# facebookresearch/gtn

Hardware: AMD Instinct MI355X
Metric: CTC forward+backward losses/sec (T=1000, C=256) (higher is better)
Workload: dtype f32; 1 GPU; BASELINE config C3: compose(ctc_target, emissions)+forwardScore CTC loss fwd+bwd, T=1000, C=256, U=100, batch=512 per GPU; global_batch=512, parallelism=dp1 (utterance sharding, all_gather of losses), rccl_ranks=0

## Files before the change

### gtn_amd/csrc/band.hip

```cpp
#include <hip/hip_runtime.h>

#include <algorithm>
#include <cstdlib>
#include <stdexcept>
#include <type_traits>

#include "kernels.h"

#ifdef GTNX_BAND_TIMING
__device__ long long g_band_timing[256];
#endif

namespace gtnx {
namespace {

constexpr float NEGF = -1.0e30f;
constexpr float DEADF = -1.0e29f;
constexpr float LOG2E = 1.44269504088896340736f;
constexpr double LN2 = 0.693147180559945309417;
constexpr int BW = 256;
constexpr int WG = 512;
constexpr int WGB = 768;
constexpr int NBE = 5;
constexpr int NBG = 7;
// ... 6 lines not shown
#endif
#ifndef GTNX_FWD_COPY_ROTATE
#define GTNX_FWD_COPY_ROTATE 1
#endif
#ifndef GTNX_FWD_DEPTH
#define GTNX_FWD_DEPTH 2
#endif

#ifdef GTNX_BAND_TIMING
#define GTNX_TM(slot)                 \
  do {                                \
    const long long now_ = clock64(); \
    tm_acc[slot] += now_ - tm_last;   \
    tm_last = now_;                   \
  } while (0)
#define GTNX_TM_INIT(base)                       \
  const int tm_base = base;                      \
  long long tm_acc[8] = {0, 0, 0, 0, 0, 0, 0, 0}; \
  long long tm_n = 0;                            \
  long long tm_last = clock64()
#define GTNX_TM_TICK() tm_n += 1
#define GTNX_TM_DUMP()                                                      \
  do {                                                                      \
    if (blockIdx.x == 0 && (threadIdx.x & 63) == 0) {                       \
      for (int i_ = 0; i_ < 7; ++i_) g_band_timing[tm_base + (threadIdx.x >> 6) * 7 + i_] += tm_acc[i_]; \
      if (threadIdx.x == 0) g_band_timing[tm_base + 127] += tm_n;           \
    }                                                                       \
  } while (0)
#else
#define GTNX_TM(slot) do { } while (0)
#define GTNX_TM_INIT(base) do { } while (0)
#define GTNX_TM_TICK() do { } while (0)
#define GTNX_TM_DUMP() do { } while (0)
#endif

__device__ __forceinline__ void lds_barrier() { asm volatile("s_waitcnt lgkmcnt(0)\n\ts_barrier" ::: "memory"); }
#ifdef GTNX_EXP_FAKE_MATH
__device__ __forceinline__ float ex2(float x) { return __builtin_fmaf(x, 0.001f, 1.0f); }
__device__ __forceinline__ float lg2(float x) { return __builtin_fmaf(x, 0.001f, -0.001f); }
#else
__device__ __forceinline__ float ex2(float x) { return __builtin_amdgcn_exp2f(x); }
__device__ __forceinline__ float lg2(float x) { return __builtin_amdgcn_logf(x); }
#endif

__device__ __forceinline__ void settle(float& x) { asm volatile("" : "+v"(x)); }
__device__ __forceinline__ void settle(int& x) { asm volatile("" : "+v"(x)); }
__device__ __forceinline__ float uniform(float x) {
  return __int_as_float(__builtin_amdgcn_readfirstlane(__float_as_int(x)));
}
__device__ __forceinline__ double uniform(double x) {
  const long long b = __double_as_longlong(x);
  const unsigned lo = __builtin_amdgcn_readfirstlane(unsigned(b)), hi = __builtin_amdgcn_readfirstlane(unsigned(b >> 32));
  return __longlong_as_double((long long)(((unsigned long long)hi << 32) | lo));
}

__device__ __forceinline__ float wave_shr1(float x, float fill) {
  return __int_as_float(__builtin_amdgcn_update_dpp(__float_as_int(fill), __float_as_int(x), 0x138, 0xf, 0xf, false));
}
__device__ __forceinline__ float wave_shl1(float x, float fill) {
  return __int_as_float(__builtin_amdgcn_update_dpp(__float_as_int(fill), __float_as_int(x), 0x130, 0xf, 0xf, false));
}
#define GTNX_DPP6(op)                                                         \
  "s_nop 1\n\t" op " %0, %0, %0 row_shr:1 row_mask:0xf bank_mask:0xf\n\t"     \
  "s_nop 1\n\t" op " %0, %0, %0 row_shr:2 row_mask:0xf bank_mask:0xf\n\t"     \
  "s_nop 1\n\t" op " %0, %0, %0 row_shr:4 row_mask:0xf bank_mask:0xf\n\t"     \
  "s_nop 1\n\t" op " %0, %0, %0 row_shr:8 row_mask:0xf bank_mask:0xf\n\t"     \
  "s_nop 1\n\t" op " %0, %0, %0 row_bcast:15 row_mask:0xa bank_mask:0xf\n\t"  \
  "s_nop 1\n\t" op " %0, %0, %0 row_bcast:31 row_mask:0xc bank_mask:0xf\n\t"  \
  "s_nop 1"
__device__ __forceinline__ float wave_max(float x) {
  asm volatile(GTNX_DPP6("v_max_f32_dpp") : "+v"(x));
  return __int_as_float(__builtin_amdgcn_readlane(__float_as_int(x), 63));
}
__device__ __forceinline__ float wave_sum63(float x) {
  asm volatile(GTNX_DPP6("v_add_f32_dpp") : "+v"(x));
  return x;
}
__device__ __forceinline__ float wave_sum(float x) {
  return __int_as_float(__builtin_amdgcn_readlane(__float_as_int(wave_sum63(x)), 63));
}
#define GTNX_DPP2(ctl)                                                  \
  "v_add_f32_dpp %0, %0, %0 " ctl "\n\tv_add_f32_dpp %1, %1, %1 " ctl "\n\ts_nop 0\n\t"
__device__ __forceinline__ void wave_sum63x2(float& a, float& b) {
  asm volatile("s_nop 1\n\t"
               GTNX_DPP2("row_shr:1 row_mask:0xf bank_mask:0xf")
               GTNX_DPP2("row_shr:2 row_mask:0xf bank_mask:0xf")
               GTNX_DPP2("row_shr:4 row_mask:0xf bank_mask:0xf")
               GTNX_DPP2("row_shr:8 row_mask:0xf bank_mask:0xf")
               GTNX_DPP2("row_bcast:15 row_mask:0xa bank_mask:0xf")
               GTNX_DPP2("row_bcast:31 row_mask:0xc bank_mask:0xf")
               : "+v"(a), "+v"(b));
}
__device__ __forceinline__ void row_sum15x2(float& a, float& b) {
  asm volatile("s_nop 1\n\t"
               GTNX_DPP2("row_shr:1 row_mask:0xf bank_mask:0xf")
               GTNX_DPP2("row_shr:2 row_mask:0xf bank_mask:0xf")
               GTNX_DPP2("row_shr:4 row_mask:0xf bank_mask:0xf")
               GTNX_DPP2("row_shr:8 row_mask:0xf bank_mask:0xf")
               : "+v"(a), "+v"(b));
}
#define GTNX_ROR4(op)                                                        \
  "s_nop 1\n\t" op " %0, %0, %0 row_ror:8 row_mask:0xf bank_mask:0xf\n\t"    \
  "s_nop 1\n\t" op " %0, %0, %0 row_ror:4 row_mask:0xf bank_mask:0xf\n\t"    \
  "s_nop 1\n\t" op " %0, %0, %0 row_ror:2 row_mask:0xf bank_mask:0xf\n\t"    \
  "s_nop 1\n\t" op " %0, %0, %0 row_ror:1 row_mask:0xf bank_mask:0xf\n\t"    \
  "s_nop 1"
__device__ __forceinline__ float row16_max(float x) {
  asm volatile(GTNX_ROR4("v_max_f32_dpp") : "+v"(x));
  return x;
}
__device__ __forceinline__ float row16_sum(float x) {
  asm volatile(GTNX_ROR4("v_add_f32_dpp") : "+v"(x));
  return x;
}
__device__ __forceinline__ float lse3(float x0, float x1, float x2) {
  const float mx = fmaxf(fmaxf(x0, x1), x2);
  const float md = __builtin_amdgcn_fmed3f(x0, x1, x2);
  const float mn = fminf(fminf(x0, x1), x2);
  return mx + lg2(1.0f + ex2(md - mx) + ex2(mn - mx));
}

template <int NPL>
struct NodeRegs {
  int lab[NPL];
  float wi[3][NPL];
  float wo[3][NPL];
  int ao[3][NPL];
  bool has_in[NPL];
  bool start[NPL], accept[NPL];
};
template <int NPL, bool WANT_OUT>
__device__ __forceinline__ void load_nodes(const BandPair& P, int m0, NodeRegs<NPL>& g) {
  const GTNX_G gtnx_i4* nodes = reinterpret_cast<const GTNX_G gtnx_i4*>(P.nodes);
#pragma unroll
  for (int j = 0; j < NPL; ++j) {
    const int m = m0 + j;
    g.lab[j] = 0;
    g.start[j] = g.accept[j] = g.has_in[j] = false;
#pragma unroll
    for (int k = 0; k < 3; ++k) {
      g.wi[k][j] = g.wo[k][j] = NEGF;
      g.ao[k][j] = -1;
    }
    if (m < P.N) {
      const gtnx_i4 q = nodes[m];
      g.lab[j] = q.x >= 0 ? q.x : 0;
      const uint8_t f = P.nflags[m];
      g.start[j] = (f & NF_START) != 0;
      g.accept[j] = (f & NF_ACCEPT) != 0;
      const int a[3] = {q.y, q.z, q.w};
#pragma unroll
      for (int k = 0; k < 3; ++k)
        if (a[k] >= 0) {
          g.has_in[j] = true;
          g.wi[k][j] = P.w ? fmaxf(P.w[a[k]] * LOG2E, NEGF) : 0.0f;
        }
    }
    if (WANT_OUT) {
#pragma unroll
      for (int k = 0; k < 3; ++k) {
        if (m + k < P.N) {
          const gtnx_i4 q = nodes[m + k];
          const int a = k == 0 ? q.y : (k == 1 ? q.z : q.w);
          if (a >= 0) {
            g.ao[k][j] = a;
            g.wo[k][j] = P.w ? fmaxf(P.w[a] * LOG2E, NEGF) : 0.0f;
          }
        }
      }
    }
  }
}

__device__ __forceinline__ float em2(float x) { return fmaxf(x * LOG2E, NEGF); }

__device__ __forceinline__ int row_of(int e, int W, float invW) {
  int r = int(float(e) * invW);
  if (r * W > e) --r;
  if ((r + 1) * W <= e) ++r;
  return r;
}

template <int NS, int LN = BW>
struct Stage {
  float v[NS];
  template <bool VEC>
  __device__ __forceinline__ void issue(const GTNX_G float* src, int cnt, int tid) {
    if (cnt <= 0) return;
#pragma unroll
    for (int i = 0; i < NS / 4; ++i) {
      if (i > 0 && 4 * i * LN >= cnt) break;
      const int e = min(4 * (i * LN + tid), cnt - 4);
      const gtnx_f4 q = *reinterpret_cast<const GTNX_G gtnx_f4*>(reinterpret_cast<const GTNX_G char*>(src) + unsigned(4 * e));
      v[4 * i] = q.x;
      v[4 * i + 1] = q.y;
      v[4 * i + 2] = q.z;
      v[4 * i + 3] = q.w;
    }
  }
  int off[NS / 4];
  __device__ __forceinline__ void init_offsets(int W, int stride, int K, int tid, bool reverse = true) {
    const float invW = 1.0f / float(W);
#pragma unroll
    for (int i = 0; i < NS / 4; ++i) {
      const int e = 4 * (i * LN + tid);
      const int r = row_of(min(e, 4096), W, invW);
      off[i] = (reverse ? K - 1 - r : r) * stride + (e - r * W);
    }
  }
  template <class F>
  __device__ __forceinline__ void each_vec(int cnt, int shift, int tid, F&& f) const {
#pragma unroll
    for (int i = 0; i < NS / 4; ++i) {
      if (i > 0 && 4 * i * LN >= cnt) break;
      if (4 * (i * LN + tid) < cnt) f(i, off[i] - shift, gtnx_f4{v[4 * i], v[4 * i + 1], v[4 * i + 2], v[4 * i + 3]});
    }
  }
  __device__ __forceinline__ void settle_all() {
#pragma unroll
    for (int i = 0; i < NS; ++i) asm volatile("" : "+v"(v[i]));
  }
  template <bool VEC, class F>
  __device__ __forceinline__ void each(int cnt, int W, int tid, F&& f) const {
    const float invW = 1.0f / float(W);
    if constexpr (VEC) {
#pragma unroll
      for (int i = 0; i < NS / 4; ++i) {
        if (i > 0 && 4 * i * LN >= cnt) break;
        const int e = 4 * (i * LN + tid);
        if (e < cnt) {
          const int r = row_of(e, W, invW);
          f(i, e, r, e - r * W, gtnx_f4{v[4 * i], v[4 * i + 1], v[4 * i + 2], v[4 * i + 3]});
        }
      }
    } else {
#pragma unroll
      for (int i = 0; i < NS / 4; ++i) {
        if (i > 0 && 4 * i * LN >= cnt) break;
        if (4 * (i * LN + tid) < cnt) {
          const int e = min(4 * (i * LN + tid), cnt - 4);
          const int r0 = row_of(e, W, invW), c0 = e - r0 * W;
#pragma unroll
          for (int k = 0; k < 4; ++k) {
            int r = r0, col = c0 + k;
            if (col >= W) {
              col -= W;
              ++r;
            }
            f(i, e + k, r, col, gtnx_f4{v[4 * i + k], 0.0f, 0.0f, 0.0f});
          }
        }
      }
    }
  }
};

struct BandLds {
  int CS;
  int o_ering, o_aring, o_oring, o_snode, o_misc, total;
};
__host__ __device__ inline BandLds band_lds(int C, int K, int NSmax, bool backward) {
  BandLds L;
  L.CS = C + 4;
  int o = 0;
  L.o_ering = o;
  o += (backward ? NBGE : NBE) * K * L.CS;
  o = (o + 3) & ~3;
  L.o_aring = o;
  o += backward ? NBE * K * NSmax : 0;
  o = (o + 3) & ~3;
  L.o_oring = o;
  o += backward ? max(NBG * K * NSmax, 2 * C) : 0;
  o = (o + 3) & ~3;
  L.o_snode = o;
  o += backward ? 512 : 0;
  L.o_misc = o;
  o += 160 + 32 + 8 + 2 * NBE * K * 4 + 40 * K + 8 + 512;
  L.total = o;
  return L;
}
struct BandMisc {
  double *offr, *red, *find, *aofr;
  float *bndr, *fin, *lsep;
};
template <int K>
__device__ __forceinline__ BandMisc band_misc(float* lds, const BandLds& L) {
  BandMisc m;
  m.offr = reinterpret_cast<double*>(lds + L.o_misc);
  m.red = m.offr + 80;
  m.find = m.red + 16;
  m.aofr = m.find + 4;
  m.bndr = lds + L.o_misc + 200 + 2 * NBE * K * 4;
  m.fin = m.bndr + 40 * K;
  m.lsep = m.fin + 8;
  return m;
}

__device__ __forceinline__ float wave_max_of(const float* v, int n) {
  float mx = v[0];
  for (int j = 1; j < n; ++j) mx = fmaxf(mx, v[j]);
  return wave_max(mx);
}

template <int NPL, bool UNIT, int K, bool VEC>
__global__ __launch_bounds__(WG) void band_forward_kernel(const BandPair* __restrict__ pairs, int NSmax) {
#define GTNX_BAND_PAIR pairs[blockIdx.x]
#include "band_forward_body.inc"
#undef GTNX_BAND_PAIR
}
template <int NPL, bool UNIT, int K, bool VEC>
__global__ __launch_bounds__(WG) void band_forward_one_kernel(BandPair one, int NSmax) {
#define GTNX_BAND_PAIR one
#include "band_forward_body.inc"
#undef GTNX_BAND_PAIR
}

__device__ __forceinline__ BandPair band_patched(BandPair P, const BandPatch& pt) {
  if (pt.on) {
    const int b = P.bidx;
    P.delta = pt.delta + b;
    P.delta_norm = pt.delta_norm ? pt.delta_norm + b : nullptr;
    P.rowlse = pt.rowlse ? pt.rowlse + int64_t(b) * pt.M : nullptr;
    P.norm = nullptr;
    P.em_copy = nullptr;
    P.grad_em = pt.grad_em ? pt.grad_em + int64_t(b) * pt.A : nullptr;
    P.grad_fixed = pt.grad_fixed ? pt.grad_fixed + P.goff : nullptr;
  }
  return P;
}
template <int NPL, bool UNIT, bool GRADG, int K, bool VEC, bool BIG>
__global__ __launch_bounds__(WGB, BIG ? 3 : 6) void band_backward_kernel(const BandPair* __restrict__ pairs, int NSmax, BandPatch patch) {
#define GTNX_BAND_PAIR band_patched(pairs[blockIdx.x], patch)
#include "band_backward_body.inc"
#undef GTNX_BAND_PAIR
}
template <int NPL, bool UNIT, bool GRADG, int K, bool VEC, bool BIG>
__global__ __launch_bounds__(WGB, BIG ? 3 : 6) void band_backward_one_kernel(BandPair one, int NSmax) {
#define GTNX_BAND_PAIR one
#include "band_backward_body.inc"
#undef GTNX_BAND_PAIR
}


__global__ __launch_bounds__(512) void ctc_targets_kernel(const CtcTargetArgs* __restrict__ args, int blank) {
  const CtcTargetArgs a = args[blockIdx.x];
  __shared__ __attribute__((aligned(16))) int tl[256 + 4];
  __shared__ __attribute__((aligned(16))) int tk[256 + 4];
  const int N = a.N, U = (N - 1) >> 1, m = threadIdx.x;
  if (m < 260) {
    const int v = m < U ? a.labels[m] : 0x7fffffff;
    tl[m] = v;
    tk[m] = (m > 0 && m < U && v != a.labels[m - 1]) ? 1 : 0;
  }
  __syncthreads();
  if (m >= N) return;
  const bool odd = (m & 1) != 0;
  const int my = odd ? tl[(m - 1) >> 1] : blank;
  const int skip = odd ? tk[(m - 1) >> 1] : 0;
  const int mi = (m - 1) >> 1;
  const int before = odd ? mi : (m >> 1);
  int rank = 0, skips = 0;
  for (int o = 0; o < U; o += 4) {
    const gtnx_i4 l4 = *reinterpret_cast<const gtnx_i4*>(tl + o), k4 = *reinterpret_cast<const gtnx_i4*>(tk + o);
    const int lo[4] = {l4.x, l4.y, l4.z, l4.w}, ko[4] = {k4.x, k4.y, k4.z, k4.w};
#pragma unroll
    for (int k = 0; k < 4; ++k) {
      const bool front = o + k < before;
      rank += (lo[k] < my || (lo[k] == my && front)) ? 1 : 0;
      skips += front ? ko[k] : 0;
    }
  }
  rank += blank < my ? U + 1 : (blank == my ? (m + 1) >> 1 : 0);
  const int base = (m > 0 ? 2 * m - 1 : 0) + skips;
  GTNX_G BandNode* nd = const_cast<GTNX_G BandNode*>(a.nodes);
  nd[m].lab = my;
  nd[m].aid[0] = base;
  nd[m].aid[1] = m > 0 ? base + 1 : -1;
  nd[m].aid[2] = skip ? base + 2 : -1;
  a.nflags[m] = uint8_t((m == 0 ? NF_START : 0) | (m + 2 >= N ? NF_ACCEPT : 0));
  a.snode[rank] = m;
  a.slab[rank] = my;
  if (m == N - 1 && a.n_arcs) a.n_arcs[0] = base + 1 + (m > 0 ? 1 : 0) + skip;
}

__global__ __launch_bounds__(512) void band_viterbi_kernel(const BandDecode* __restrict__ pairs) {
  const BandDecode P = pairs[blockIdx.x];
  const int T = P.T, C = P.C, N = P.N, NS = P.NS;
  extern __shared__ float lds[];
  const float NINF = -__builtin_inff();
  float* a0 = lds;
  float* a1 = lds + 516;
  float* stage = lds + 1032;
  const int m = threadIdx.x;
  const GTNX_G gtnx_i4* nodes = reinterpret_cast<const GTNX_G gtnx_i4*>(P.nodes);
  int lab = 0;
  float wi[3] = {NINF, NINF, NINF};
  bool accept = false, start = false;
  if (m < N) {
    const gtnx_i4 q = nodes[m];
    lab = q.x >= 0 ? q.x : 0;
    const int a[3] = {q.y, q.z, q.w};
#pragma unroll
    for (int k = 0; k < 3; ++k)
      if (a[k] >= 0) wi[k] = P.w ? P.w[a[k]] : 0.0f;
    const uint8_t f = P.nflags[m];
    start = (f & NF_START) != 0;
    accept = (f & NF_ACCEPT) != 0;
  }
  if (m < 2) a0[m] = a1[m] = NINF;
  a0[2 + m] = start ? 0.0f : NINF;
  a1[2 + m] = NINF;
  int tie = 0;
  const int R = max(1, min(64, P.stage_floats / C));
  float* cur = a0;
  float* nxt = a1;
  __syncthreads();
  for (int t0 = 0; t0 < T; t0 += R) {
    const int rows = min(R, T - t0);
    for (int e = threadIdx.x; e < rows * C; e += blockDim.x) stage[e] = P.em[int64_t(t0) * C + e];
    __syncthreads();
    for (int i = 0; i < rows; ++i) {
      const float e = stage[i * C + lab];
      const float c0 = cur[2 + m] + (wi[0] + e), c1 = cur[1 + m] + (wi[1] + e), c2 = cur[m] + (wi[2] + e);
      float best = c0;
      int k = 0;
      if (c1 > best) best = c1, k = 1;
      if (c2 > best) best = c2, k = 2;
      if (best > NINF && ((k != 0 && c0 == best) || (k != 1 && c1 == best) || (k != 2 && c2 == best))) tie = 1;
      if (m < NS) P.bp[int64_t(t0 + i) * NS + m] = uint8_t(best > NINF ? k : 3);
      nxt[2 + m] = m < N ? best : NINF;
      __syncthreads();
      float* sw = cur;
      cur = nxt;
      nxt = sw;
    }
  }
  __shared__ float red_v[8];
  __shared__ int red_m[8], s_best, s_tie;
  float v = accept ? cur[2 + m] : NINF;
  int bm = (m < N && accept && v > NINF) ? m : 1 << 30;
  const float wmx = wave_max(v);
  if (!(v == wmx)) bm = 1 << 30;
  int cnt = (bm != (1 << 30)) ? 1 : 0;
  for (int o = 32; o > 0; o >>= 1) {
    bm = min(bm, __shfl_xor(bm, o));
    cnt += __shfl_xor(cnt, o);
  }
  if ((threadIdx.x & 63) == 0) {
    red_v[threadIdx.x >> 6] = wmx;
    red_m[threadIdx.x >> 6] = bm;
  }
  if (cnt > 1) tie = 1;
  if (threadIdx.x == 0) s_tie = 0;
  __syncthreads();
  if (threadIdx.x == 0) {
    float bv = NINF;
    int bn = -1;
    for (int w = 0; w < 8; ++w) {
      if (red_m[w] == (1 << 30)) continue;
      if (red_v[w] > bv) bv = red_v[w], bn = red_m[w];
      else if (red_v[w] == bv && bv > NINF) s_tie = 1;
    }
    s_best = bn;
    P.score[0] = bv;
  }
  if (tie) atomicOr(&s_tie, 1);
  __syncthreads();
  const int best = s_best;
  if (threadIdx.x == 0) {
    P.tie[0] = s_tie;
    P.path_len[0] = best >= 0 ? T : -1;
  }
  if (best < 0 || T == 0) return;
  uint8_t* bst = reinterpret_cast<uint8_t*>(stage);
  const int RB = max(1, min(T, P.stage_floats * 4 / NS));
  __shared__ int s_node;
  if (threadIdx.x == 0) {
    s_node = best;
    P.pnode[T] = best;
  }
  for (int hi = T; hi > 0; hi -= RB) {
    const int lo = max(0, hi - RB);
    __syncthreads();
    for (int e = threadIdx.x; e < (hi - lo) * NS; e += blockDim.x) bst[e] = P.bp[int64_t(lo) * NS + e];
    __syncthreads();
    if (threadIdx.x == 0) {
      int node = s_node;
      for (int t = hi - 1; t >= lo; --t) {
        node -= bst[(t - lo) * NS + node] & 3;
        P.pnode[t] = node;
      }
      s_node = node;
    }
  }
  __threadfence_block();
  __syncthreads();
  for (int t = threadIdx.x; t < T; t += blockDim.x) {
    const int m1 = P.pnode[t + 1], k = m1 - P.pnode[t];
    const gtnx_i4 q = nodes[m1];
    const int arc = k == 0 ? q.y : (k == 1 ? q.z : q.w);
    P.path_arc[t] = arc;
    P.path_lab[t] = q.x;
    P.path_w[t] = (P.w ? P.w[arc] : 0.0f) + P.em[int64_t(t) * C + q.x];
  }
}

constexpr int VBLK = 2048;

template <int NPL, bool RANKED>
__global__ __launch_bounds__(64) void band_viterbi_wave_kernel(const BandDecode* __restrict__ pairs) {
  const BandDecode P = pairs[blockIdx.x];
  const int T = P.T, C = P.C, N = P.N;
  const int lane = threadIdx.x;
  constexpr int SPW = 16 / NPL;
  constexpr int NLD = VBLK / 256;
  __shared__ __attribute__((aligned(16))) float ring[3 * VBLK];
  const float NINF = -__builtin_inff();
  const GTNX_G gtnx_i4* nodes = reinterpret_cast<const GTNX_G gtnx_i4*>(P.nodes);
  int loff[NPL];
  float w0[NPL], w1[NPL], w2[NPL], alpha[NPL];
  bool acc[NPL];
#pragma unroll
  for (int j = 0; j < NPL; ++j) {
    const int m = lane * NPL + j;
    loff[j] = 0;
    w0[j] = w1[j] = w2[j] = NINF;
    alpha[j] = NINF;
    acc[j] = false;
    if (m < N) {
      const gtnx_i4 q = nodes[m];
      loff[j] = 4 * (q.x >= 0 ? q.x : 0);
      if (q.y >= 0) w0[j] = P.w ? P.w[q.y] : 0.0f;
      if (q.z >= 0) w1[j] = P.w ? P.w[q.z] : 0.0f;
      if (q.w >= 0) w2[j] = P.w ? P.w[q.w] : 0.0f;
      const uint8_t f = P.nflags[m];
      if (f & NF_START) alpha[j] = 0.0f;
      acc[j] = (f & NF_ACCEPT) != 0;
    }
  }
#pragma unroll
  for (int j = 0; j < NPL; ++j) {
    settle(w0[j]);
    settle(w1[j]);
    settle(w2[j]);
    settle(loff[j]);
  }
  int r0[NPL], r1[NPL], r2[NPL];
  if (RANKED) {
#pragma unroll
    for (int j = 0; j < NPL; ++j) {
      const int m = lane * NPL + j;
      r0[j] = m < N ? P.rank_in[m] : 0x7ffffffe;
      r1[j] = (m >= 1 && m - 1 < N) ? P.rank_in[m - 1] : 0x7ffffffe;
      r2[j] = (m >= 2 && m - 2 < N) ? P.rank_in[m - 2] : 0x7ffffffe;
    }
  }
  const int R = max(1, VBLK / C);
  const int NB = (T + R - 1) / R;
  const int64_t total = int64_t(T) * C;
  auto issue = [&](int b) {
    const int64_t f0 = int64_t(b) * R * C;
    float* dst = ring + (b % 3) * VBLK;
#pragma unroll
    for (int i = 0; i < NLD; ++i) {
      int64_t f = f0 + i * 256 + lane * 4;
      f = f + 4 <= total ? f : total - 4;
      __builtin_amdgcn_global_load_lds((const __attribute__((address_space(1))) void*)(P.em + f),
                                       (__attribute__((address_space(3))) void*)(dst + i * 256), 16, 0, 0);
    }
  };
  GTNX_G unsigned* bp32 = reinterpret_cast<GTNX_G unsigned*>(P.bp);
  unsigned word = 0;
  if (NB > 0) issue(0);
  if (NB > 1) issue(1);
#ifdef GTNX_VIT_NO_SWEEP
#define GTNX_VIT_ROWS 0
#else
#define GTNX_VIT_ROWS rows
#endif
  for (int b = 0; b < NB; ++b) {
    if (b + 2 < NB) {
      issue(b + 2);
      asm volatile("s_waitcnt vmcnt(16)" ::: "memory");
    } else if (b + 1 < NB) {
      asm volatile("s_waitcnt vmcnt(8)" ::: "memory");
    } else {
      asm volatile("s_waitcnt vmcnt(0)" ::: "memory");
    }
    const char* buf = reinterpret_cast<const char*>(ring + (b % 3) * VBLK);
    const int t0 = b * R, rows = min(R, T - t0);
    float e[NPL];
#pragma unroll
    for (int j = 0; j < NPL; ++j) e[j] = *reinterpret_cast<const float*>(buf + loff[j]);
    for (int i = 0; i < GTNX_VIT_ROWS; ++i) {
      const int t = t0 + i;
      const char* nrow = buf + (i + 1 < rows ? i + 1 : i) * (C * 4);
      float en[NPL];
#pragma unroll
      for (int j = 0; j < NPL; ++j) en[j] = *reinterpret_cast<const float*>(nrow + loff[j]);
      float s1, s2;
      if (NPL >= 2) {
        s1 = wave_shr1(alpha[NPL - 1], NINF);
        s2 = wave_shr1(alpha[NPL >= 2 ? NPL - 2 : 0], NINF);
      } else {
        s1 = wave_shr1(alpha[0], NINF);
        s2 = wave_shr1(s1, NINF);
      }
      float na[NPL];
      const int sh = (t % SPW) * 2 * NPL;
      unsigned codes = 0;
#pragma unroll
      for (int j = 0; j < NPL; ++j) {
        const float p1 = j > 0 ? alpha[j > 0 ? j - 1 : 0] : s1;
        const float p2 = j > 1 ? alpha[j > 1 ? j - 2 : 0] : (j == 1 ? s1 : s2);
        const float c0 = alpha[j] + (w0[j] + e[j]), c1 = p1 + (w1[j] + e[j]), c2 = p2 + (w2[j] + e[j]);
        const float best = fmaxf(fmaxf(c0, c1), c2);
        const float med = __builtin_amdgcn_fmed3f(c0, c1, c2);
        unsigned k;
        if (RANKED) {
          const int q0 = c0 == best ? r0[j] : 0x7fffffff, q1 = c1 == best ? r1[j] : 0x7fffffff,
                    q2 = c2 == best ? r2[j] : 0x7fffffff;
          k = (q0 <= q1 && q0 <= q2) ? 0u : (q1 <= q2 ? 1u : 2u);
          k = best == NINF ? 3u : k;
          (void)med;
        } else {
          k = c0 == best ? 0u : (c1 == best ? 1u : 2u);
          k = med == best ? 3u : k;
        }
        codes |= k << (2 * j);
        na[j] = best;
      }
      word |= codes << sh;
#pragma unroll
      for (int j = 0; j < NPL; ++j) {
        alpha[j] = na[j];
        e[j] = en[j];
      }
      if ((t % SPW) == SPW - 1 || t == T - 1) {
        bp32[int64_t(t / SPW) * 64 + lane] = word;
        word = 0;
      }
    }
  }
  float lv = NINF;
#pragma unroll
  for (int j = 0; j < NPL; ++j) lv = fmaxf(lv, acc[j] ? alpha[j] : NINF);
  const float wmx = wave_max(lv);
  int bm = 1 << 30, cnt = 0;
#pragma unroll
  for (int j = NPL - 1; j >= 0; --j)
    if (acc[j] && alpha[j] == wmx && wmx > NINF) {
      const int m = lane * NPL + j;
      bm = RANKED ? min(bm, (P.rank_acc[m] << 16) | m) : m;
      ++cnt;
    }
  for (int o = 32; o > 0; o >>= 1) {
    bm = min(bm, __shfl_xor(bm, o));
    cnt += __shfl_xor(cnt, o);
  }
  int tie = (cnt > 1 && !RANKED) ? 1 : 0;
  const int best = bm == (1 << 30) ? -1 : (RANKED ? (bm & 0xffff) : bm);
  if (lane == 0) {
    P.score[0] = best >= 0 ? wmx : NINF;
    P.path_len[0] = best >= 0 ? T : -1;
  }
  if (best < 0 || T == 0) {
    if (lane == 0) P.tie[0] = tie;
    return;
  }
#ifdef GTNX_VIT_NO_CHASE
  if (lane == 0) P.tie[0] = tie;
  return;
#endif
  __builtin_amdgcn_fence(__ATOMIC_SEQ_CST, "workgroup");
  unsigned node = unsigned(__builtin_amdgcn_readfirstlane(best));
  int* lpn = reinterpret_cast<int*>(ring);
  constexpr int LPN = 3 * VBLK;
  if (lane == 0) {
    P.pnode[T] = int(node);
    if (T < LPN) lpn[T] = int(node);
  }
  const int NW = (T + SPW - 1) / SPW;
  constexpr int RB = 16;
  unsigned cur[RB], nxt[RB];
  const int nbatch = (NW + RB - 1) / RB;
  auto fetch = [&](unsigned (&dst)[RB], int q) {
#pragma unroll
    for (int r = 0; r < RB; ++r) dst[r] = bp32[int64_t(min(q * RB + r, NW - 1)) * 64 + lane];
  };
  fetch(cur, nbatch - 1);
  int pn = 0;
  for (int q = nbatch - 1; q >= 0; --q) {
    if (q > 0) fetch(nxt, q - 1);
#pragma unroll
    for (int r = RB - 1; r >= 0; --r) {
      const int wi = q * RB + r;
      if (wi < NW) {
#pragma unroll
        for (int u = SPW - 1; u >= 0; --u) {
          const int t = wi * SPW + u;
          if (t < T) {
            const unsigned wv = unsigned(__builtin_amdgcn_readlane(int(cur[r]), int(node / NPL)));
            unsigned k = (wv >> (u * 2 * NPL + 2 * (node % NPL))) & 3u;
            if (k == 3u) {
              tie = 1;
              k = 0;
            }
            node -= min(k, node);
            if (lane == (t & 63)) pn = int(node);
            if ((t & 63) == 0) {
              if (t + lane < T) {
                P.pnode[t + lane] = pn;
                if (t + lane < LPN) lpn[t + lane] = pn;
              }
            }
          }
        }
      }
    }
#pragma unroll
    for (int r = 0; r < RB; ++r) cur[r] = nxt[r];
  }
  if (lane == 0) P.tie[0] = tie;
  if (T >= LPN) __builtin_amdgcn_fence(__ATOMIC_SEQ_CST, "workgroup");
  for (int t = lane; t < T; t += 64) {
    const int m1 = T < LPN ? lpn[t + 1] : P.pnode[t + 1], k = m1 - (T < LPN ? lpn[t] : P.pnode[t]);
    const gtnx_i4 q = nodes[m1];
    const int arc = k == 0 ? q.y : (k == 1 ? q.z : q.w);
    P.path_arc[t] = arc;
    P.path_lab[t] = q.x;
    P.path_w[t] = (arc >= 0 && P.w ? P.w[arc] : 0.0f) + P.em[int64_t(t) * C + (q.x >= 0 ? q.x : 0)];
  }
}

__global__ __launch_bounds__(512) void asg_fal_targets_kernel(const AsgFalArgs* __restrict__ args, int NL) {
  const AsgFalArgs a = args[blockIdx.x];
  __shared__ int lab[512];
  const int U = a.U, m = threadIdx.x;
  int my = -1;
  if (m >= 1 && m <= U) my = a.labels[m - 1];
  lab[m] = my;
  __syncthreads();
  if (m > U) return;
  GTNX_G BandNode* nd = const_cast<GTNX_G BandNode*>(a.nodes);
  nd[m].lab = my;
  nd[m].aid[0] = m >= 1 ? 2 * m - 1 : -1;
  nd[m].aid[1] = m >= 1 ? 2 * m - 2 : -1;
  nd[m].aid[2] = -1;
  a.nflags[m] = uint8_t((m == 0 ? NF_START : 0) | (m == U ? NF_ACCEPT : 0));
  if (m >= 1) {
    int rank = 0;
    for (int o = 1; o <= U; ++o) {
      const int lo = lab[o];
      rank += (lo < my || (lo == my && o < m)) ? 1 : 0;
    }
    a.snode[rank] = m;
    a.slab[rank] = my;
    const int step = m == 1 ? my : NL + my * NL + lab[m - 1];
    const int self = NL + my * NL + my;
    a.arc_map[2 * m - 2] = step;
    a.arc_map[2 * m - 1] = self;
    a.w[2 * m - 2] = a.trans_w[step];
    a.w[2 * m - 1] = a.trans_w[self];
  }
}
__global__ void asg_fal_scatter_kernel(const float* __restrict__ g, const int* __restrict__ maps,
                                       const int64_t* __restrict__ tab, float* __restrict__ trans_grad) {
  const int64_t* e = tab + int64_t(blockIdx.y) * 3;
  const int64_t n = e[2];
  const float* gb = g + e[0];
  const int* mb = maps + e[1];
  for (int64_t i = int64_t(blockIdx.x) * blockDim.x + threadIdx.x; i < n; i += int64_t(gridDim.x) * blockDim.x)
    if (mb[i] >= 0 && gb[i] != 0.0f) atomicAdd(trans_grad + mb[i], gb[i]);
}

template <class K>
void big_lds(K kern) {
  (void)hipFuncSetAttribute(reinterpret_cast<const void*>(kern), hipFuncAttributeMaxDynamicSharedMemorySize, 160 * 1024 - 512);
}

template <int NPL, int K, bool VEC>
void launch_fwd2(const BandPair* d, const BandPair* one, int n, int ns, size_t lds, bool unit, hipStream_t st) {
  static std::atomic<uint64_t> done{0};
  if (gtnx_first_on_device first{done}) {
    big_lds(band_forward_kernel<NPL, true, K, VEC>);
    big_lds(band_forward_kernel<NPL, false, K, VEC>);
    if constexpr (NPL == 1 && VEC) {
      big_lds(band_forward_one_kernel<NPL, true, K, VEC>);
      big_lds(band_forward_one_kernel<NPL, false, K, VEC>);
    }
  }
  if constexpr (NPL == 1 && VEC) {
    if (one) {
      if (unit) hipLaunchKernelGGL((band_forward_one_kernel<NPL, true, K, VEC>), dim3(1), dim3(WG), lds, st, *one, ns);
      else hipLaunchKernelGGL((band_forward_one_kernel<NPL, false, K, VEC>), dim3(1), dim3(WG), lds, st, *one, ns);
      return;
    }
  }
  if (unit) hipLaunchKernelGGL((band_forward_kernel<NPL, true, K, VEC>), dim3(n), dim3(WG), lds, st, d, ns);
  else hipLaunchKernelGGL((band_forward_kernel<NPL, false, K, VEC>), dim3(n), dim3(WG), lds, st, d, ns);
}
template <int NPL, int K>
void launch_fwd(const BandPair* d, const BandPair* one, int n, int ns, size_t lds, bool unit, bool vec, hipStream_t st) {
  if (vec) launch_fwd2<NPL, K, true>(d, one, n, ns, lds, unit, st);
  else launch_fwd2<NPL, K, false>(d, one, n, ns, lds, unit, st);
}
template <int NPL, int K, bool VEC, bool BIG>
void launch_bwd3(const BandPair* d, const BandPair* one, int n, int ns, size_t lds, bool unit, bool gradg, hipStream_t st,
                 const BandPatch& pt) {
  constexpr bool ONE = NPL == 1 && VEC && !BIG;
  static std::atomic<uint64_t> done{0};
  if (gtnx_first_on_device first{done}) {
    big_lds(band_backward_kernel<NPL, true, true, K, VEC, BIG>);
    big_lds(band_backward_kernel<NPL, true, false, K, VEC, BIG>);
    big_lds(band_backward_kernel<NPL, false, true, K, VEC, BIG>);
    big_lds(band_backward_kernel<NPL, false, false, K, VEC, BIG>);
    if constexpr (ONE) {
      big_lds(band_backward_one_kernel<NPL, true, true, K, VEC, BIG>);
      big_lds(band_backward_one_kernel<NPL, true, false, K, VEC, BIG>);
      big_lds(band_backward_one_kernel<NPL, false, true, K, VEC, BIG>);
      big_lds(band_backward_one_kernel<NPL, false, false, K, VEC, BIG>);
    }
  }
  if constexpr (ONE) {
    if (one) {
      if (unit) {
        if (gradg) hipLaunchKernelGGL((band_backward_one_kernel<NPL, true, true, K, VEC, BIG>), dim3(1), dim3(WGB), lds, st, *one, ns);
        else hipLaunchKernelGGL((band_backward_one_kernel<NPL, true, false, K, VEC, BIG>), dim3(1), dim3(WGB), lds, st, *one, ns);
      } else {
        if (gradg) hipLaunchKernelGGL((band_backward_one_kernel<NPL, false, true, K, VEC, BIG>), dim3(1), dim3(WGB), lds, st, *one, ns);
        else hipLaunchKernelGGL((band_backward_one_kernel<NPL, false, false, K, VEC, BIG>), dim3(1), dim3(WGB), lds, st, *one, ns);
      }
      return;
    }
  }
  if (unit) {
    if (gradg) hipLaunchKernelGGL((band_backward_kernel<NPL, true, true, K, VEC, BIG>), dim3(n), dim3(WGB), lds, st, d, ns, pt);
    else hipLaunchKernelGGL((band_backward_kernel<NPL, true, false, K, VEC, BIG>), dim3(n), dim3(WGB), lds, st, d, ns, pt);
  } else {
    if (gradg) hipLaunchKernelGGL((band_backward_kernel<NPL, false, true, K, VEC, BIG>), dim3(n), dim3(WGB), lds, st, d, ns, pt);
    else hipLaunchKernelGGL((band_backward_kernel<NPL, false, false, K, VEC, BIG>), dim3(n), dim3(WGB), lds, st, d, ns, pt);
  }
}
template <int NPL, int K>
void launch_bwd(const BandPair* d, const BandPair* one, int n, int ns, size_t lds, bool unit, bool gradg, bool vec, bool big,
                hipStream_t st, const BandPatch& pt) {
  if constexpr (K == 2) {
    if (big) {
      if (vec) launch_bwd3<NPL, K, true, true>(d, one, n, ns, lds, unit, gradg, st, pt);
      else launch_bwd3<NPL, K, false, true>(d, one, n, ns, lds, unit, gradg, st, pt);
      return;
    }
  }
  if (vec) launch_bwd3<NPL, K, true, false>(d, one, n, ns, lds, unit, gradg, st, pt);
  else launch_bwd3<NPL, K, false, false>(d, one, n, ns, lds, unit, gradg, st, pt);
}

constexpr size_t LDS_TWO = 78 * 1024;
constexpr size_t LDS_ONE = 156 * 1024;

}

int band_block_rows(int C, int max_NS, bool backward);
static int band_backward_lds_stride(int K, int max_NS) { return K == 4 ? (max_NS + 15) / 16 * 16 : max_NS; }
int band_max_nodes() { return 512; }
int band_max_labels() { return 1024; }
int band_min_labels() { return 4; }
int band_npl(int max_nodes) { return max_nodes <= 256 ? 1 : 2; }
int band_row_stride(int N, int) { return (N + 3) / 4 * 4; }
#ifndef GTNX_FWD_SHIFT_ROWS
#define GTNX_FWD_SHIFT_ROWS 4
#endif
int band_forward_lgrn(int C) {
  const int K = band_block_rows(C, 0, false);
  return K >= GTNX_FWD_SHIFT_ROWS ? (GTNX_FWD_SHIFT_ROWS == 8 ? 3 : 2) : (K >= 4 ? 2 : 1);
}
int band_block_rows(int C, int max_NS, bool backward) {
  for (int k = backward ? 4 : 8; k >= 2; k /= 2) {
    if (k * C > 2048 || k * max_NS > 2048) continue;
    if (backward && k > 2 && (k * C > 1024 || k * max_NS > 1024)) continue;
    const int ns_lds = backward ? band_backward_lds_stride(k, max_NS) : max_NS;
    if (4 * size_t(band_lds(C, k, ns_lds, backward).total) + 64 <= LDS_TWO) return k;
  }
  if (4 * size_t(band_lds(C, 2, max_NS, backward).total) + 64 <= LDS_ONE) return 2;
  return 0;
}

bool band_one_ok(int npl, int C, int max_NS, bool vec, bool backward) {
  if (npl != 1 || !vec) return false;
  if (!backward) return true;
  const int K = band_block_rows(C, max_NS, true);
  return !(K * C > 1024 || K * max_NS > 1024);
}
void launch_band_forward(const BandPair* d_pairs, int n, int npl, int C, int max_NS, bool unit, bool vec, hipStream_t st,
                         const BandPair* one) {
  if (n <= 0) return;
  if (one && (n != 1 || !band_one_ok(npl, C, max_NS, vec, false))) throw std::logic_error("band.hip: not a single-pair launch");
  const int K = band_block_rows(C, 0, false);
  const size_t lds = 4 * size_t(band_lds(C, K, max_NS, false).total) + 64;
  if (npl == 1) {
    if (K == 8) launch_fwd<1, 8>(d_pairs, one, n, max_NS, lds, unit, vec, st);
    else if (K == 4) launch_fwd<1, 4>(d_pairs, one, n, max_NS, lds, unit, vec, st);
    else launch_fwd<1, 2>(d_pairs, one, n, max_NS, lds, unit, vec, st);
  } else {
    if (K == 8) launch_fwd<2, 8>(d_pairs, one, n, max_NS, lds, unit, vec, st);
    else if (K == 4) launch_fwd<2, 4>(d_pairs, one, n, max_NS, lds, unit, vec, st);
    else launch_fwd<2, 2>(d_pairs, one, n, max_NS, lds, unit, vec, st);
  }
}

void launch_band_backward(const BandPair* d_pairs, int n, int npl, int C, int max_NS, bool unit, bool gradg, bool vec,
                          hipStream_t st, const BandPair* one, const BandPatch* patch) {
  if (n <= 0) return;
  if (one && patch) throw std::logic_error("band.hip: a patched launch reads a device table");
  BandPatch pt{};
  if (patch) pt = *patch;
  if (one && (n != 1 || !band_one_ok(npl, C, max_NS, vec, true))) throw std::logic_error("band.hip: not a single-pair launch");
  const int K = band_block_rows(C, max_NS, true);
  const bool big = K * C > 1024 || K * max_NS > 1024;
  const int ns_lds = band_backward_lds_stride(K, max_NS);
  const size_t lds = 4 * size_t(band_lds(C, K, ns_lds, true).total) + 64;
  if (npl == 1) {
    if (K == 4) launch_bwd<1, 4>(d_pairs, one, n, ns_lds, lds, unit, gradg, vec, big, st, pt);
    else launch_bwd<1, 2>(d_pairs, one, n, ns_lds, lds, unit, gradg, vec, big, st, pt);
  } else {
    if (K == 4) throw std::logic_error("band.hip: four rows per block with two nodes per lane");
    launch_bwd<2, 2>(d_pairs, one, n, ns_lds, lds, unit, gradg, vec, big, st, pt);
  }
}

template <int NPL>
static void launch_viterbi_wave(const BandDecode* d_pairs, int n, int ranked, hipStream_t st) {
  if (ranked) hipLaunchKernelGGL((band_viterbi_wave_kernel<NPL, true>), dim3(n), dim3(64), 0, st, d_pairs);
  else hipLaunchKernelGGL((band_viterbi_wave_kernel<NPL, false>), dim3(n), dim3(64), 0, st, d_pairs);
}
bool band_viterbi_wave_ok(int max_nodes, int max_labels, int vec) {
  static const bool force_wg = std::getenv("GTNX_VITERBI_WG") != nullptr;
  return !force_wg && vec && max_nodes <= 512 && max_labels <= VBLK;
}
void launch_band_viterbi(const BandDecode* d_pairs, int n, int stage_floats, int max_nodes, int max_labels, int vec,
                         hipStream_t st, int ranked) {
  if (n <= 0) return;
  if (band_viterbi_wave_ok(max_nodes, max_labels, vec)) {
    if (max_nodes <= 64) launch_viterbi_wave<1>(d_pairs, n, ranked, st);
    else if (max_nodes <= 128) launch_viterbi_wave<2>(d_pairs, n, ranked, st);
    else if (max_nodes <= 256) launch_viterbi_wave<4>(d_pairs, n, ranked, st);
    else launch_viterbi_wave<8>(d_pairs, n, ranked, st);
    return;
  }
  if (ranked) return;
  static std::atomic<uint64_t> done{0};
  if (gtnx_first_on_device first{done}) big_lds(band_viterbi_kernel);
  hipLaunchKernelGGL(band_viterbi_kernel, dim3(n), dim3(512), 4 * size_t(1032 + stage_floats) + 64, st, d_pairs);
}

void launch_asg_fal_targets(const AsgFalArgs* d_args, int n, int n_labels, hipStream_t st) {
  if (n > 0) hipLaunchKernelGGL(asg_fal_targets_kernel, dim3(n), dim3(512), 0, st, d_args, n_labels);
}
void launch_asg_fal_scatter(const float* g, const int* maps, const int64_t* tab, int n_seq, int64_t longest, float* trans_grad,
                            hipStream_t st) {
  if (n_seq > 0 && longest > 0)
    hipLaunchKernelGGL(asg_fal_scatter_kernel, dim3(unsigned(std::min<int64_t>((longest + 255) / 256, 64)), unsigned(n_seq)),
                       dim3(256), 0, st, g, maps, tab, trans_grad);
}
void launch_ctc_targets(const CtcTargetArgs* d_args, int n, int blank, hipStream_t st) {
  if (n > 0) hipLaunchKernelGGL(ctc_targets_kernel, dim3(n), dim3(512), 0, st, d_args, blank);
}

}
```

### gtn_amd/csrc/band_backward_body.inc

```
  constexpr int RNk = K >= 4 ? 4 : K;
  constexpr int NP = K / RNk;
  const BandPair P = GTNX_BAND_PAIR;
  const int T = P.T, C = P.C, NS = P.NS;
  extern __shared__ float lds[];
  const BandLds L = band_lds(C, K, NSmax, true);
  float* ering = lds + L.o_ering;
  float* aring = lds + L.o_aring;
  float* oring = lds + L.o_oring;
  int* snode = reinterpret_cast<int*>(lds + L.o_snode);
  const BandMisc M = band_misc<K>(lds, L);
  float* lser = M.lsep;
  const int CS = L.CS;
  const int wv = __builtin_amdgcn_readfirstlane(threadIdx.x >> 6);
  const bool sweeper = wv < 4;
  const int l = threadIdx.x & 63;
  const int nblocks = (T + K - 1) / K;
  const int nticks = nblocks + 5;
  const GTNX_G double* ao = P.aoff;
  const double z2 = uniform(ao[0]);
  const bool dead = !(z2 > double(DEADF));
  const float ds = uniform(P.delta[0]);
  const bool want_em = P.grad_em != nullptr;
  GTNX_TM_INIT(128);
  constexpr bool SPLIT = !BIG && K >= 2 && GTNX_BWD_SPLIT;
  const float dn_k = P.delta_norm ? uniform(P.delta_norm[0]) : 0.0f;
  float* const rnorm_k = lser + NBG * K;
  auto rows_of_k = [&](int c) { return c < nblocks ? min(K, T - c * K) : 0; };
  auto ring_start = [](int c, int M) { return ((c % M) + M) % M; };
  static_assert((NBGE & (NBGE - 1)) == 0, "the emission ring's position is a mask");
  auto ge_of = [](int c) { return int(unsigned(c) & unsigned(NBGE - 1)); };
  auto ring_step = [](int& v, int M) { v = v + 1 == M ? 0 : v + 1; };
  struct RowSumRegs {
    float in[NPL];
    gtnx_f4 hot[NPL];
  };
  auto rowsum_init = [&](RowSumRegs& R) {
#pragma unroll
    for (int q = 0; q < NPL; ++q) {
      const int mb = 256 * q + 4 * l;
      R.in[q] = mb < NSmax ? 1.0f : 0.0f;
      float hm[4];
#pragma unroll
      for (int k = 0; k < 4; ++k) {
        const int m = mb + k;
        int lab = -1;
        if (m < P.N) lab = P.nodes[m].lab;
        settle(lab);
        hm[k] = (P.hot >= 0 && lab == P.hot) ? 1.0f : 0.0f;
      }
      R.hot[q] = gtnx_f4{hm[0], hm[1], hm[2], hm[3]};
    }
  };
  auto rowsum_do = [&](const RowSumRegs& R, int c, int cg , int r, auto steady_tag) -> float {
    constexpr bool STEADY = decltype(steady_tag)::value;
    if (!want_em || (K < 4 && r >= K)) return 0.0f;
    if constexpr (!STEADY) {
      if (r >= rows_of_k(c)) return 0.0f;
    }
    const bool dead_r = STEADY ? false : dead;
    const float* ob = oring + (cg * K + r) * NSmax;
    gtnx_f4 v[NPL];
#pragma unroll
    for (int q = 0; q < NPL; ++q) v[q] = *reinterpret_cast<const gtnx_f4*>(ob + min(256 * q + 4 * l, NSmax - 4));
    const float em_hot = ering[(ge_of(c) * K + r) * CS + max(P.hot, 0)];
    const float ls_hot = lser[cg * K + r];
    float all = (v[0].x * R.in[0] + v[0].y * R.in[0]) + (v[0].z * R.in[0] + v[0].w * R.in[0]);
    float hotp = (v[0].x * R.hot[0].x + v[0].y * R.hot[0].y) + (v[0].z * R.hot[0].z + v[0].w * R.hot[0].w);
#pragma unroll
    for (int q = 1; q < NPL; ++q) {
      all += (v[q].x * R.in[q] + v[q].y * R.in[q]) + (v[q].z * R.in[q] + v[q].w * R.in[q]);
      hotp += (v[q].x * R.hot[q].x + v[q].y * R.hot[q].y) + (v[q].z * R.hot[q].z + v[q].w * R.hot[q].w);
    }
    if (dead_r) all = hotp = 0.0f;
    wave_sum63x2(all, hotp);
    all = __int_as_float(__builtin_amdgcn_readlane(__float_as_int(all), 63));
    const bool have = all != 0.0f && !dead_r;
    const float f = have ? ds * __builtin_amdgcn_rcpf(all) : 1.0f;
    if (l == 63 && P.hot >= 0) {
      const float sm = dn_k * ex2(em_hot - ls_hot);
      P.grad_em[int64_t(T - 1 - c * K - r) * C + P.hot] = (dead_r ? 0.0f : hotp * f) + sm;
    }
    if (l == 0) rnorm_k[cg * K + r] = f;
    return have ? f : 0.0f;
  };
#ifndef GTNX_BWD_ROWSUM4
#define GTNX_BWD_ROWSUM4 1
#endif
  constexpr bool RS4 = !BIG && !SPLIT && K == 4 && NPL == 1 && GTNX_BWD_ROWSUM4;
  struct RowSum4Regs {
    float in;
    gtnx_f4 hot[4];
    int po;
    int eo, go;
  };
  auto rowsum4_init = [&](RowSum4Regs& R) {
    const int r = l >> 4, nb = 16 * (l & 15);
    R.in = nb < NSmax ? 1.0f : 0.0f;
    R.po = r * NSmax + min(nb, NSmax - 16);
#pragma unroll
    for (int k = 0; k < 4; ++k) {
      float hm[4];
#pragma unroll
      for (int e = 0; e < 4; ++e) {
        const int m = nb + 4 * k + e;
        int lab = -1;
        if (m < P.N) lab = P.nodes[m].lab;
        settle(lab);
        hm[e] = (P.hot >= 0 && lab == P.hot) ? 1.0f : 0.0f;
      }
      R.hot[k] = gtnx_f4{hm[0], hm[1], hm[2], hm[3]};
    }
    R.eo = r * CS + max(P.hot, 0);
    R.go = (K - 1 - r) * C + max(P.hot, 0);
  };
  auto rowsum4_do = [&](const RowSum4Regs& R, int c, int cg , auto steady_tag) {
    constexpr bool STEADY = decltype(steady_tag)::value;
    const int rows = STEADY ? K : rows_of_k(c);
    if (!want_em || rows <= 0) return;
    const bool dead_r = STEADY ? false : dead;
    typedef float f2v __attribute__((ext_vector_type(2)));
    const float* ob = oring + cg * K * NSmax + R.po;
    gtnx_f4 v[4];
#pragma unroll
    for (int k = 0; k < 4; ++k) v[k] = *reinterpret_cast<const gtnx_f4*>(ob + 4 * k);
    const float em_hot = ering[ge_of(c) * K * CS + R.eo];
    const float ls_hot = lser[cg * K + (l >> 4)];
    f2v a2 = f2v{v[0].x, v[0].y} + f2v{v[0].z, v[0].w};
    f2v h2 = f2v{v[0].x, v[0].y} * f2v{R.hot[0].x, R.hot[0].y};
    h2 = __builtin_elementwise_fma(f2v{v[0].z, v[0].w}, f2v{R.hot[0].z, R.hot[0].w}, h2);
#pragma unroll
    for (int k = 1; k < 4; ++k) {
      a2 += f2v{v[k].x, v[k].y} + f2v{v[k].z, v[k].w};
      h2 = __builtin_elementwise_fma(f2v{v[k].x, v[k].y}, f2v{R.hot[k].x, R.hot[k].y}, h2);
      h2 = __builtin_elementwise_fma(f2v{v[k].z, v[k].w}, f2v{R.hot[k].z, R.hot[k].w}, h2);
    }
    float all = (a2.x + a2.y) * R.in, hotp = h2.x + h2.y;
    if (dead_r) all = hotp = 0.0f;
    row_sum15x2(all, hotp);
    const bool have = all != 0.0f && !dead_r;
    const float f = have ? ds * __builtin_amdgcn_rcpf(all) : 1.0f;
    if ((l & 15) == 15 && (STEADY || (l >> 4) < rows)) {
      if (P.hot >= 0) {
        const float sm = dn_k * ex2(em_hot - ls_hot);
        const GTNX_G char* gb = reinterpret_cast<const GTNX_G char*>(P.grad_em + int64_t(T - c * K - K) * C);
        *reinterpret_cast<GTNX_G float*>(const_cast<GTNX_G char*>(gb) + unsigned(4 * R.go)) = (dead_r ? 0.0f : hotp * f) + sm;
      }
      rnorm_k[cg * K + (l >> 4)] = f;
    }
  };
  constexpr int NCS = 8 / K;
  struct DrainRegs {
    int s[NCS], e[NCS], n0[NCS], n1[NCS];
    float m0[NCS], m1[NCS];
    bool more_any;
  };
  auto drain_init = [&](DrainRegs& D, int hid) {
    const int* cls = reinterpret_cast<const int*>(oring);
#pragma unroll
    for (int q = 0; q < NCS; ++q) {
      const int cc = hid + q * BW;
      D.s[q] = D.e[q] = 0;
      if (cc < C && cc != P.hot) {
        D.s[q] = cls[cc];
        D.e[q] = cls[C + cc];
      }
      const int cnt = D.e[q] - D.s[q];
      D.n0[q] = cnt > 0 ? snode[D.s[q]] : 0;
      D.n1[q] = cnt > 1 ? snode[D.s[q] + 1] : 0;
      D.m0[q] = cnt > 0 ? 1.0f : 0.0f;
      D.m1[q] = cnt > 1 ? 1.0f : 0.0f;
    }
    D.more_any = false;
#pragma unroll
    for (int q = 0; q < NCS; ++q) D.more_any = D.more_any || __builtin_amdgcn_ballot_w64(D.e[q] - D.s[q] > 2) != 0;
  };
  auto drain_rows = [&](const DrainRegs& D, int hid, int c, int cg , auto full_tag, auto dead_tag, auto r0_tag, auto r1_tag) {
    constexpr bool FULL = decltype(full_tag)::value;
    constexpr bool DEADU = decltype(dead_tag)::value;
    constexpr int R0 = decltype(r0_tag)::value, R1 = decltype(r1_tag)::value;
    const int rows = FULL ? K : rows_of_k(c);
    const float* ob = oring + cg * K * NSmax;
    const float* eb = ering + ge_of(c) * K * CS;
    const float* lb = lser + cg * K;
    const float* fb = rnorm_k + cg * K;
    GTNX_G float* dst = P.grad_em + int64_t(T - 1 - c * K) * C;
#pragma unroll
    for (int q = 0; q < NCS; ++q) {
      if (q > 0 && q * BW >= C) break;
      const int cc = hid + q * BW;
      const bool mine = cc < C && cc != P.hot;
      float p0[K], p1[K], e[K], ls[K], f[K];
#pragma unroll
      for (int r = R0; r < R1; ++r) {
        if constexpr (!DEADU) {
          p0[r] = ob[r * NSmax + D.n0[q]];
          p1[r] = ob[r * NSmax + D.n1[q]];
        }
        e[r] = eb[r * CS + min(cc, C - 1)];
      }
      if constexpr (K == 4) {
        const gtnx_f4 l4 = *reinterpret_cast<const gtnx_f4*>(lb), f4 = *reinterpret_cast<const gtnx_f4*>(fb);
        ls[0] = l4.x, ls[1] = l4.y, ls[2] = l4.z, ls[3] = l4.w;
        f[0] = f4.x, f[1] = f4.y, f[2] = f4.z, f[3] = f4.w;
      } else {
#pragma unroll
        for (int r = R0; r < R1; ++r) {
          ls[r] = lb[r];
          f[r] = fb[r];
        }
      }
      float sum[K];
      if constexpr (!DEADU) {
#pragma unroll
      for (int r = R0; r < R1; ++r) sum[r] = p0[r] * D.m0[q] + p1[r] * D.m1[q];
      }
      if (!DEADU && D.more_any) {
        for (int i = D.s[q] + 2; i < D.e[q]; ++i) {
          const float* o = ob + snode[i];
#pragma unroll
          for (int r = R0; r < R1; ++r) sum[r] += o[r * NSmax];
        }
      }
      float val[K];
#pragma unroll
      for (int r = R0; r < R1; ++r) {
        const float sm = dn_k * ex2(e[r] - ls[r]);
        val[r] = DEADU ? sm : sum[r] * f[r] + sm;
      }
      if (mine) {
#pragma unroll
        for (int r = R0; r < R1; ++r) {
          if (FULL || r < rows) {
            GTNX_G float* row = dst - int64_t(r) * C;
            row[cc] = val[r];
          }
        }
      }
    }
  };
  auto drain_block = [&](const DrainRegs& D, int hid, int c, int cg, auto r0_tag, auto r1_tag) {
    if (!want_em || c >= nblocks) return;
    if (dead) drain_rows(D, hid, c, cg, std::false_type{}, std::true_type{}, r0_tag, r1_tag);
    else if (c * K + K <= T) drain_rows(D, hid, c, cg, std::true_type{}, std::false_type{}, r0_tag, r1_tag);
    else drain_rows(D, hid, c, cg, std::false_type{}, std::false_type{}, r0_tag, r1_tag);
  };
  constexpr int KH = SPLIT ? K / 2 : K;

  if (sweeper) {
#ifndef GTNX_BWD_SWEEP_PRIO
#define GTNX_BWD_SWEEP_PRIO 1
#endif
    __builtin_amdgcn_s_setprio(GTNX_BWD_SWEEP_PRIO);
    const int w = wv;
    const int lag = 3 - w;
    const int m0 = threadIdx.x * NPL;
    NodeRegs<NPL> g;
    load_nodes<NPL, true>(P, m0, g);
    float b[NPL], post[NPL], acc[3][NPL];
    const double Ahi = uniform(ao[1 + (T >> P.lgrn) * 4 + w]);
    double bsum = 0.0;
#pragma unroll
    for (int j = 0; j < NPL; ++j) {
      b[j] = g.accept[j] ? 0.0f : NEGF;
      float ahi = m0 < NS ? P.alpha[int64_t(T) * NS + m0 + j] : NEGF;
      settle(ahi);
      post[j] = dead ? 0.0f : ex2(ahi + b[j] + float(Ahi - z2));
      acc[0][j] = acc[1][j] = acc[2][j] = 0.0f;
      settle(g.lab[j]);
#pragma unroll
      for (int k = 0; k < 3; ++k) {
        settle(g.wo[k][j]);
        settle(g.ao[k][j]);
      }
    }
    float* bnd_own = M.bndr + (4 - w) * 4 * K * 2;
    const float* bnd_prev = M.bndr + (3 - w) * 4 * K * 2;
    double* off_own = M.offr + (4 - w) * 16;
    const double* off_prev = M.offr + (3 - w) * 16;
    if (threadIdx.x < 8 * K) M.bndr[threadIdx.x] = NEGF;
    if (threadIdx.x < 16) M.offr[threadIdx.x] = 0.0;
    if (l == 0) off_own[0] = 0.0;
    lds_barrier();
    lds_barrier();
    RowSumRegs rsr;
    if constexpr (!SPLIT && !RS4) rowsum_init(rsr);
    float gscale = ds;
    int bm5 = ring_start(-lag, NBE), bm7 = ring_start(-lag, NBG), rm7 = ring_start(RS4 ? -5 : -4, NBG);
    lds_barrier();
    auto tick = [&](int tau, auto steady_tag) {
      constexpr bool STEADY = decltype(steady_tag)::value;
      GTNX_TM(0);
      if constexpr (RS4) {
#ifndef GTNX_EXP_NO_GSCALE
        if (GRADG && want_em && (STEADY || (tau >= 5 && (tau - 5) * K + K <= T))) gscale = rnorm_k[rm7 * K + w];
#endif
      } else if constexpr (!SPLIT) {
#ifndef GTNX_EXP_NO_ROWSUM
        if (STEADY || tau >= 4) {
          const float fr = rowsum_do(rsr, tau - 4, rm7, w, steady_tag);
#ifndef GTNX_EXP_NO_GSCALE
          if (fr != 0.0f) gscale = fr;
#endif
        }
#endif
      }
      GTNX_TM(3);
      const int beta = tau - lag;
      auto block = [&](auto full_tag) {
        constexpr bool FULL = decltype(full_tag)::value;
        const int v0 = beta * K, rows = FULL ? K : min(K, T - v0);
        const float* eb = ering + ge_of(beta) * K * CS;
        const float* ab = aring + bm5 * K * NSmax;
        const double* Ab = M.aofr + (bm5 * K) * 4 + w;
        float* ob = oring + bm7 * K * NSmax + m0;
        float ev[K][NPL], alov[K][NPL], bq1[K], bq2[K];
        double Acur[K], offp[NP + 1];
#pragma unroll
        for (int i = 0; i < K; ++i) {
#pragma unroll
          for (int j = 0; j < NPL; ++j) {
            ev[i][j] = eb[i * CS + g.lab[j]];
            alov[i][j] = ab[i * NSmax + min(m0 + j, NS - 1)];
          }
          Acur[i] = Ab[i * 4];
        }
#pragma unroll
        for (int q = 0; q <= NP; ++q) offp[q] = off_prev[(beta * NP + q) & 15];
        {
// ... 400 lines not shown
```

### gtn_amd/csrc/band_forward_body.inc

```
#ifndef GTNX_FWD_SHIFT_ROWS
#define GTNX_FWD_SHIFT_ROWS 4
#endif
  constexpr int RNk = K >= GTNX_FWD_SHIFT_ROWS ? GTNX_FWD_SHIFT_ROWS : (K >= 4 ? 4 : K);
  constexpr int NP = K / RNk;
  constexpr int D = 8 / K > GTNX_FWD_DEPTH ? 8 / K : GTNX_FWD_DEPTH;
  const BandPair P = GTNX_BAND_PAIR;
  const int T = P.T, C = P.C, NS = P.NS;
  extern __shared__ float lds[];
  const BandLds L = band_lds(C, K, NSmax, false);
  float* ering = lds + L.o_ering;
  const BandMisc M = band_misc<K>(lds, L);
  const int CS = L.CS;
  const int wv = __builtin_amdgcn_readfirstlane(threadIdx.x >> 6);
  const bool sweeper = wv < 4;
  const int l = threadIdx.x & 63;
  const int nblocks = (T + K - 1) / K;
  const int nticks = nblocks + 3;
  GTNX_TM_INIT(0);

  if (sweeper) {
    __builtin_amdgcn_s_setprio(1);
    const int w = wv;
    const int m0 = threadIdx.x * NPL;
    NodeRegs<NPL> g;
    load_nodes<NPL, false>(P, m0, g);
    const bool writer = m0 < NS;
    float a[NPL];
#pragma unroll
    for (int j = 0; j < NPL; ++j) a[j] = g.start[j] ? 0.0f : NEGF;
    double off = 0.0;
    const GTNX_G char* arow = reinterpret_cast<const GTNX_G char*>(P.alpha);
    const unsigned aoffb = unsigned(m0) * 4u;
    auto store_row = [&](const float* v) {
#pragma unroll
      for (int j = 0; j < NPL; ++j) *reinterpret_cast<GTNX_G float*>(const_cast<GTNX_G char*>(arow) + (aoffb + 4u * j)) = v[j];
    };
    if (writer) store_row(a);
    float* bnd_own = M.bndr + (w + 1) * 4 * K * 2;
    const float* bnd_prev = M.bndr + w * 4 * K * 2;
    double* off_own = M.offr + (w + 1) * 16;
    const double* off_prev = M.offr + w * 16;
    if (threadIdx.x < 8 * K) M.bndr[threadIdx.x] = NEGF;
    if (threadIdx.x < 16) M.offr[threadIdx.x] = 0.0;
    if (l == 0) {
      P.aoff[1 + w] = 0.0;
      off_own[0] = 0.0;
    }
    if (NPL == 1) {
      if (l >= 62) bnd_own[63 - l] = a[0];
    } else if (l == 63) {
      bnd_own[0] = a[NPL - 1];
      bnd_own[1] = a[0];
    }
    lds_barrier();
    int bm5 = ((-w % NBE) + NBE) % NBE;
    for (int tau = 0; tau < nticks; ++tau, bm5 = bm5 + 1 == NBE ? 0 : bm5 + 1) {
      GTNX_TM(0);
      const int beta = tau - w;
      auto block = [&](auto full_tag) {
        constexpr bool FULL = decltype(full_tag)::value;
        const int t0 = beta * K, rows = FULL ? K : min(K, T - t0);
        const float* eb = ering + bm5 * K * CS;
        float ev[K][NPL], bv1[K], bv2[K];
        double offp[NP + 1];
#pragma unroll
        for (int i = 0; i < K; ++i) {
#pragma unroll
#ifdef GTNX_EXP_NOCONFLICT
          for (int j = 0; j < NPL; ++j) ev[i][j] = eb[i * CS + l * NPL + j];
#else
          for (int j = 0; j < NPL; ++j) ev[i][j] = eb[i * CS + g.lab[j]];
#endif
        }
        {
          const float* bp = bnd_prev + (beta & 3) * K * 2;
          if constexpr (K % 2 == 0) {
#pragma unroll
            for (int i = 0; i < K; i += 2) {
              const gtnx_f4 q4 = *reinterpret_cast<const gtnx_f4*>(bp + 2 * i);
              bv1[i] = q4.x, bv2[i] = q4.y, bv1[i + 1] = q4.z, bv2[i + 1] = q4.w;
            }
          } else {
#pragma unroll
            for (int i = 0; i < K; ++i) bv1[i] = bp[2 * i], bv2[i] = bp[2 * i + 1];
          }
        }
#pragma unroll
        for (int q = 0; q <= NP; ++q) offp[q] = off_prev[(beta * NP + q) & 15];
        float hist[K][NPL];
#pragma unroll
        for (int i = 0; i < K; ++i) {
          if (FULL || i < rows) {
            if (i % RNk == 0) {
              typedef float f2v __attribute__((ext_vector_type(2)));
              const float dconv = float(offp[i / RNk] - off);
              const f2v d2 = {dconv, dconv};
#pragma unroll
              for (int r = i; r < i + RNk && r < K; ++r) {
                const f2v c = f2v{bv1[r], bv2[r]} + d2;
                bv1[r] = c.x, bv2[r] = c.y;
              }
            }
            const float b1 = bv1[i], b2 = bv2[i];
            const float p1 = wave_shr1(a[NPL - 1], b1);
            const float p2 = NPL == 2 ? wave_shr1(a[0], b2) : wave_shr1(p1, b2);
            float nw[NPL];
#pragma unroll
            for (int j = 0; j < NPL; ++j) {
              const float s1 = j == 0 ? p1 : a[0];
              const float s2 = j == 0 ? p2 : p1;
              float x0, x1, x2;
              if (UNIT) {
                x0 = a[j];
                x1 = s1;
                x2 = s2 + g.wi[2][j];
              } else {
                x0 = a[j] + g.wi[0][j];
                x1 = s1 + g.wi[1][j];
                x2 = s2 + g.wi[2][j];
              }
              nw[j] = lse3(x0, x1, x2) + ev[i][j];
            }
            if ((i + 1) % RNk == 0) {
              const float mx = wave_max_of(nw, NPL);
              if (mx > DEADF) {
#pragma unroll
                for (int j = 0; j < NPL; ++j) nw[j] -= mx;
                off += double(mx);
              } else if (w > 0) {
                off = offp[(i + 1) / RNk];
              }
              if (l == 0) {
                const int p = (t0 + i + 1) / RNk;
                off_own[p & 15] = off;
                P.aoff[1 + p * 4 + w] = off;
              }
            }
#pragma unroll
            for (int j = 0; j < NPL; ++j) hist[i][j] = a[j] = nw[j];
          }
        }
        {
          const GTNX_G char* const brow = arow;
          arow += int64_t(NS) * 4 * rows;
#ifdef GTNX_EXP_NO_ALPHA_STORE
          if (writer && beta < 0) {
#else
          if (writer) {
#endif
#pragma unroll
            for (int i = 0; i < K; ++i)
              if (FULL || i < rows) {
                const GTNX_G char* ri = brow + int64_t(NS) * 4 * (i + 1);
#pragma unroll
                for (int j = 0; j < NPL; ++j) *reinterpret_cast<GTNX_G float*>(const_cast<GTNX_G char*>(ri) + (aoffb + 4u * j)) = hist[i][j];
              }
          }
        }
        if (NPL == 1 ? l >= 62 : l == 63) {
#pragma unroll
          for (int i = 0; i < K; ++i)
            if (FULL || i < rows) {
              float* bp = bnd_own + ((((beta & 3) * K + i + 1) & (4 * K - 1))) * 2;
              if (NPL == 1) {
                bp[63 - l] = hist[i][0];
              } else {
                bp[0] = hist[i][NPL - 1];
                bp[1] = hist[i][0];
              }
            }
        }
      };
      if (beta >= 0 && beta < nblocks) {
        if (beta * K + K <= T) block(std::true_type{});
        else block(std::false_type{});
      }
      GTNX_TM(5);
      lds_barrier();
      GTNX_TM(6);
      GTNX_TM_TICK();
    }
    float f = NEGF;
#pragma unroll
    for (int j = 0; j < NPL; ++j) f = fmaxf(f, g.accept[j] ? a[j] : NEGF);
    const float mx = wave_max(f);
    float s = 0.0f;
#pragma unroll
    for (int j = 0; j < NPL; ++j) s += g.accept[j] ? ex2(a[j] - mx) : 0.0f;
    s = wave_sum(s);
    if (l == 0) {
      M.fin[2 * w] = mx;
      M.fin[2 * w + 1] = s;
      M.find[w] = off;
    }
  } else {
    const int hid = threadIdx.x - BW;
    constexpr bool vec = VEC;
    const bool want_lse = P.norm != nullptr || P.rowlse != nullptr;
    Stage<8> st[D];
    auto rows_of = [&](int c) { return c < nblocks ? min(K, T - c * K) : 0; };
    auto issue = [&](Stage<8>& s, int c) { s.template issue<VEC>(P.em + int64_t(c) * K * C, rows_of(c) * C, hid); };
    GTNX_G float* const em_copy = P.em_copy;
    auto land = [&](const Stage<8>& s, int c, int c5 , auto copy_tag) {
      constexpr bool COPY = decltype(copy_tag)::value;
      float* base = ering + c5 * K * CS;
      GTNX_G float* cdst = em_copy + int64_t(c) * K * C;
      s.template each<VEC>(rows_of(c) * C, C, hid, [&](int, int e, int r, int col, gtnx_f4 q) {
        float* d = base + r * CS + col;
        if (vec) *reinterpret_cast<gtnx_f4*>(d) = gtnx_f4{em2(q.x), em2(q.y), em2(q.z), em2(q.w)};
        else d[0] = em2(q.x);
        if (COPY) {
          if (vec) __builtin_nontemporal_store(q, reinterpret_cast<GTNX_G gtnx_f4*>(cdst + e));
          else __builtin_nontemporal_store(q.x, cdst + e);
        }
      });
    };
    constexpr int LPR = BW / K, G16 = LPR / 16;
    const int EPL = (C + LPR - 1) / LPR;
    double normacc = 0.0;
    auto lse_a_n = [&](int c, int c5 , auto nconst) {
      constexpr int NE = decltype(nconst)::value;
      const int rows = rows_of(c), rr = hid / LPR, sub = hid - rr * LPR;
      if (rows <= 0) return;
      const float* e = ering + (c5 * K + min(rr, rows - 1)) * CS + sub * EPL;
      float x[NE];
      float m = NEGF;
      if (VEC && (EPL & 3) == 0) {
#pragma unroll
        for (int i = 0; i < NE; i += 4) {
          const bool in = i < EPL && sub * EPL + i < C;
          const gtnx_f4 q = in ? *reinterpret_cast<const gtnx_f4*>(e + i) : gtnx_f4{NEGF, NEGF, NEGF, NEGF};
          x[i] = q.x, x[i + 1] = q.y, x[i + 2] = q.z, x[i + 3] = q.w;
          m = fmaxf(fmaxf(m, fmaxf(q.x, q.y)), fmaxf(q.z, q.w));
        }
      } else {
#pragma unroll
        for (int i = 0; i < NE; ++i) {
          x[i] = (i < EPL && sub * EPL + i < C) ? e[i] : NEGF;
          m = fmaxf(m, x[i]);
        }
      }
      m = row16_max(m);
      float sum = 0.0f;
#pragma unroll
      for (int i = 0; i < NE; ++i) sum += (i < EPL) ? ex2(x[i] - m) : 0.0f;
      sum = row16_sum(sum);
      if ((hid & 15) == 0 && rr < rows) {
        float* p = M.lsep + (c & 1) * 256 + (rr * 8 + (sub >> 4)) * 2;
        p[0] = m;
        p[1] = sum;
      }
    };
    auto lse_a = [&](int c, int c5) {
      if (EPL <= 4) lse_a_n(c, c5, std::integral_constant<int, 4>{});
      else if (EPL <= 8) lse_a_n(c, c5, std::integral_constant<int, 8>{});
      else lse_a_n(c, c5, std::integral_constant<int, 16>{});
    };
    auto lse_b = [&](int c) {
      const int rows = rows_of(c);
      if (hid < rows) {
        const float* p = M.lsep + (c & 1) * 256 + hid * 16;
        float Mx = p[0];
#pragma unroll
        for (int k = 1; k < G16; ++k) Mx = fmaxf(Mx, p[2 * k]);
        float S = 0.0f;
#pragma unroll
        for (int k = 0; k < G16; ++k) S += p[2 * k + 1] * ex2(p[2 * k] - Mx);
        const float l2 = Mx + lg2(S);
        if (P.rowlse) P.rowlse[c * K + hid] = l2;
        normacc += double(l2);
      }
    };
    auto run = [&](auto copy_tag) {
      issue(st[0], 0);
      land(st[0], 0, 0, copy_tag);
#pragma unroll
      for (int c = 1; c <= D; ++c) issue(st[c % D], c);
      lds_barrier();
      int t5 = 0;
      for (int tau0 = 0; tau0 < nticks; tau0 += D) {
#pragma unroll
        for (int d = 0; d < D; ++d) {
          const int tau = tau0 + d;
          if (tau >= nticks) break;
          GTNX_TM(0);
          const int n5 = t5 + 1 == NBE ? 0 : t5 + 1;
          land(st[(d + 1) % D], tau + 1, n5, copy_tag);
          GTNX_TM(1);
          issue(st[(d + 1) % D], tau + 1 + D);
          GTNX_TM(2);
          if (want_lse) {
            if (tau >= 1 && tau - 1 < nblocks) lse_b(tau - 1);
            if (tau < nblocks) lse_a(tau, t5);
          }
          t5 = n5;
          GTNX_TM(4);
          lds_barrier();
          GTNX_TM(6);
          GTNX_TM_TICK();
        }
      }
    };
    auto run_copy = [&]() {
      constexpr int DC = GTNX_FWD_COPY_DEPTH < 8 / K ? 8 / K : GTNX_FWD_COPY_DEPTH;
      constexpr int R = DC + 1;
      Stage<8> sc[R];
      issue(sc[0], 0);
      land(sc[0], 0, 0, std::true_type{});
#pragma unroll
      for (int c = 1; c <= DC; ++c) issue(sc[c % R], c);
      lds_barrier();
      int t5 = 0;
      for (int tau0 = 0; tau0 < nticks; tau0 += R) {
#pragma unroll
        for (int d = 0; d < R; ++d) {
          const int tau = tau0 + d;
          if (tau >= nticks) break;
          GTNX_TM(0);
          const int n5 = t5 + 1 == NBE ? 0 : t5 + 1;
          sc[(d + 1) % R].settle_all();
          issue(sc[d % R], tau + 1 + DC);
          GTNX_TM(2);
          land(sc[(d + 1) % R], tau + 1, n5, std::true_type{});
          GTNX_TM(1);
          if (want_lse) {
            if (tau >= 1 && tau - 1 < nblocks) lse_b(tau - 1);
            if (tau < nblocks) lse_a(tau, t5);
// ... 37 lines not shown
```

### gtn_amd/csrc/batch.cpp

```cpp
#include "batch.h"

#include <algorithm>
#include <atomic>
#include <unordered_map>
#include <unordered_set>

namespace gtnx {

namespace {

std::atomic<uint64_t> g_batch_seq{1};

struct CompMode {
  int old;
  CompMode() : old(compose_mode_hint(2)) {}
  ~CompMode() { compose_mode_hint(old); }
};

BatchP make_batch(Batch::Kind k, int n, bool cg) {
  auto b = std::make_shared<Batch>();
  b->kind = k;
  b->n = n;
  b->calc_grad = cg;
  return b;
}

BatchP result(Batch::Kind k, int n, std::shared_ptr<BatchOp> op) {
  bool cg = false;
  for (auto& i : op->inputs) cg |= i->calc_grad;
  BatchP r = make_batch(k, n, cg);
  op->seq = g_batch_seq.fetch_add(1);
  r->op = std::move(op);
  return r;
}

bool native(const Batch& b, Batch::Kind k) { return b.kind == k; }

void alloc_grad(Batch& b, bool zero) {
  Runtime& rt = Runtime::get();
  b.g_off.resize(size_t(b.n) + 1);
  b.g_off[0] = 0;
  for (int i = 0; i < b.n; ++i) b.g_off[size_t(i) + 1] = b.g_off[size_t(i)] + b.elem_size(i);
  const size_t bytes = sizeof(float) * size_t(b.g_off[size_t(b.n)]);
  if (b.dest) {
    b.g_mem = b.dest_mem;
    b.g_dev = b.dest;
    b.dest = nullptr;
    if (zero && bytes) HIP_CHECK(hipMemsetAsync(b.g_dev, 0, bytes, rt.stream()));
  } else {
    b.g_mem = zero ? rt.alloc_zero(bytes ? bytes : 4) : rt.alloc(bytes ? bytes : 4);
    b.g_dev = b.g_mem->as<float>();
  }
}

struct GradTarget {
  float* ptr = nullptr;
  DevMemP scratch;
};
GradTarget grad_target(Batch& b, bool zero) {
  GradTarget t;
  if (!b.g_dev) {
    alloc_grad(b, zero);
    t.ptr = b.g_dev;
    return t;
  }
  Runtime& rt = Runtime::get();
  const size_t bytes = sizeof(float) * size_t(b.g_off[size_t(b.n)]);
  t.scratch = zero ? rt.alloc_zero(bytes ? bytes : 4) : rt.alloc(bytes ? bytes : 4);
  t.ptr = t.scratch->as<float>();
  return t;
}
void add_scratch(Batch& b, const GradTarget& t) {
  if (!t.scratch) return;
  launch_vec_axpby(b.g_dev, t.ptr, nullptr, size_t(b.g_off[size_t(b.n)]), 1.0f, 0.0f, 1, Runtime::get().stream());
}

struct BScalarOp : BatchOp {
  ScalarKind kind;
  void backward(Batch& out) override {
    Runtime& rt = Runtime::get();
    for (size_t i = 0; i < inputs.size(); ++i) {
      Batch& in = *inputs[i];
      if (!in.calc_grad) continue;
      const float s = (kind == SK_NEGATE || (kind == SK_SUBTRACT && i == 1)) ? -1.0f : 1.0f;
      const bool have = in.g_dev != nullptr;
      if (!have) alloc_grad(in, false);
      launch_vec_axpby(in.g_dev, out.g_dev, nullptr, size_t(in.n), s, 0.0f, have ? 1 : 0, rt.stream());
    }
  }
};

struct BackwardPlan {
  std::unordered_map<Batch*, Batch*> lin;
  std::unordered_set<Batch*> fused;
};
thread_local BackwardPlan* t_plan = nullptr;
thread_local bool t_batch_retain = false;

struct BFsLinearOp : BatchOp {
  void backward(Batch& out) override {
    Batch& e = *inputs[0];
    if (!e.calc_grad) return;
    if (t_plan && e.nc_rowlse && !t_plan->lin.count(&e)) {
      t_plan->lin[&e] = &out;
      return;
    }
    run(out);
  }
  void run(Batch& out) {
    Batch& e = *inputs[0];
    Runtime& rt = Runtime::get();
    if (e.w_pend) e.w_pend->settle();
    const bool have = e.g_dev != nullptr;
    if (!have) alloc_grad(e, false);
    std::vector<LinArgs> args;
    args.resize(size_t(e.n));
    const size_t A = size_t(e.M) * size_t(e.C);
    for (int b = 0; b < e.n; ++b) {
      LinArgs& a = args[size_t(b)];
      a.w = e.w_dev + size_t(b) * A;
      a.M = e.M;
      a.C = e.C;
      a.out_score = nullptr;
      a.partial = nullptr;
      a.delta = out.g_dev + b;
      a.grad = e.g_dev + size_t(b) * A;
      a.accumulate = have ? 1 : 0;
    }
    DevMemP d = upload_vec(args);
    const bool vec_rows = e.C % 4 == 0 && e.C <= 1024 && (reinterpret_cast<uintptr_t>(e.w_dev) & 15) == 0 &&
                          (reinterpret_cast<uintptr_t>(e.g_dev) & 15) == 0;
    GTNX_PROF("linear_forward_grad", (have ? 12.0 : 8.0) * double(A) * e.n);
    launch_linear_backward(d->as<LinArgs>(), e.n, 0, vec_rows ? 1 : 0, rt.stream());
  }
};

struct BFsBandOp : BatchOp {
  std::vector<BandPair> pairs;
  DevMemP arena;
  DevMemP fwd_table;
  DevMemP through_acc;
  void backward(Batch& out) override {
    Batch& prod = *inputs[0];
    Batch& fx = *prod.fixed;
    Batch& ch = *prod.chain;
    Runtime& rt = Runtime::get();
    const float* delta = out.g_dev;
    if (through_acc || t_batch_retain) {
      const size_t n = size_t(prod.n);
      if (!through_acc) through_acc = rt.alloc_zero(sizeof(float) * (n ? n : 1));
      launch_vec_axpby(through_acc->as<float>(), out.g_dev, nullptr, n, 1.0f, 0.0f, 1, rt.stream());
      delta = through_acc->as<float>();
    }
    GradTarget ge, gf;
    if (ch.calc_grad) ge = grad_target(ch, false);
    if (fx.calc_grad) gf = grad_target(fx, fx.fal);
    Batch* lin_out = nullptr;
    if (t_plan && ch.calc_grad && !ge.scratch) {
      auto it = t_plan->lin.find(&ch);
      if (it != t_plan->lin.end() && !t_plan->fused.count(&ch)) {
        lin_out = it->second;
        t_plan->fused.insert(&ch);
      }
    }
    std::vector<std::pair<BandLaunchKey, BandPair>> tab;
    tab.reserve(pairs.size());
    double bytes = 0;
    const size_t A = size_t(ch.M) * size_t(ch.C);
    bool one_key = true;
    int max_ns = 0;
    for (int b = 0; b < prod.n; ++b) {
      BandPair p = pairs[size_t(b)];
      p.delta = delta + b;
      p.delta_norm = lin_out ? lin_out->g_dev + b : nullptr;
      p.rowlse = lin_out ? ch.nc_rowlse + size_t(b) * size_t(ch.M) : nullptr;
      p.norm = nullptr;
      p.grad_em = ge.ptr ? ge.ptr + size_t(b) * A : nullptr;
      p.grad_fixed = gf.ptr ? gf.ptr + fx.g_off[size_t(b)] : nullptr;
      tab.push_back({BandLaunchKey{p.C, band_npl(p.N), fx.fal ? 0 : 1, p.grad_fixed ? 1 : 0, band_vec_ok(p)}, p});
      one_key = one_key && tab.back().first == tab.front().first;
      max_ns = std::max(max_ns, p.NS);
      bytes += 4.0 * p.T * p.C * (p.grad_em ? 2 : 1) + 4.0 * double(p.T + 1) * p.NS +
               (p.grad_fixed ? 4.0 * double(fx.elem_size(b)) : 0.0);
    }
    static const bool no_patch = std::getenv("GTNX_NO_BAND_PATCH") != nullptr;
    if (fwd_table && one_key && prod.n > 1 && !no_patch) {
      BandPatch pt{};
      pt.on = 1;
      pt.M = ch.M;
      pt.delta = delta;
      pt.delta_norm = lin_out ? lin_out->g_dev : nullptr;
      pt.rowlse = lin_out ? ch.nc_rowlse : nullptr;
      pt.grad_em = ge.ptr;
      pt.grad_fixed = gf.ptr;
      pt.A = int64_t(A);
      band_launch_patched(fwd_table, prod.n, tab.front().first, max_ns, pt, "band_forward_score_grad", bytes);
    } else {
      band_launch(tab, true, "band_forward_score_grad", bytes);
    }
    if (ch.calc_grad) add_scratch(ch, ge);
    if (fx.calc_grad) add_scratch(fx, gf);
    (void)rt;
  }
};


struct BFalOp : BatchOp {
  void backward(Batch& out) override {
    Graph& tr = out.trans;
    if (!tr.calc_grad() || !out.g_dev) return;
    Runtime& rt = Runtime::get();
    const int64_t A = tr.num_arcs();
    DevMemP gm = rt.alloc_zero(sizeof(float) * size_t(A ? A : 1));
    std::vector<int64_t> tab(size_t(out.n) * 3);
    int64_t longest = 0;
    for (int b = 0; b < out.n; ++b) {
      const int64_t len = out.g_off[size_t(b) + 1] - out.g_off[size_t(b)];
      tab[size_t(b) * 3 + 0] = out.g_off[size_t(b)];
      tab[size_t(b) * 3 + 1] = int64_t(out.map_off[size_t(b)] / sizeof(int));
      tab[size_t(b) * 3 + 2] = len;
      longest = std::max(longest, len);
    }
    DevMemP dt = upload_vec(tab);
    launch_asg_fal_scatter(out.g_dev, out.rec_mem->as<int>(), dt->as<int64_t>(), out.n, longest, gm->as<float>(), rt.stream());
    tr.add_grad_device(gm, gm->as<float>(), true);
  }
};

struct BFromGraphsOp : BatchOp {
  DevMemP passed;
  void backward(Batch& out) override {
    Batch& src = *inputs[0];
    Runtime& rt = Runtime::get();
    const size_t n = size_t(src.n);
    DevMemP delta = rt.alloc(sizeof(float) * (n ? n : 1));
    if (passed)
      launch_vec_axpby(delta->as<float>(), out.g_dev, passed->as<float>(), n, 1.0f, -1.0f, 0, rt.stream());
    else
      rt.d2d(delta->ptr, out.g_dev, sizeof(float) * n);
    if (retain) {
      if (!passed) passed = rt.alloc(sizeof(float) * (n ? n : 1));
      rt.d2d(passed->ptr, out.g_dev, sizeof(float) * n);
    }
    std::vector<Graph> roots;
    for (int b = 0; b < src.n; ++b) {
      Graph& r = src.graphs[size_t(b)];
      if (!r.calc_grad()) continue;
      r.add_grad_device(delta, delta->as<float>() + b, true);
      roots.push_back(r);
    }
    if (!roots.empty()) op_backward(roots, nullptr, retain, false);
  }
  bool retain = false;
};

}

Batch::~Batch() {
  if (host_ev) (void)hipEventDestroy(static_cast<hipEvent_t>(host_ev));
  if (give_back && !origins.empty()) {
    for (const Origin& o : origins) {
      auto* part = new std::vector<Graph>();
      part->reserve(o.end - o.begin);
      for (size_t i = o.begin; i < o.end && i < graphs.size(); ++i) part->push_back(std::move(graphs[i]));
      give_back(o.home, part);
    }
    graphs.clear();
    return;
  }
  if (graphs.size() < 64 || !Runtime::initialized()) return;
  Runtime& rt = Runtime::get();
  for (size_t i = 0; i < graphs.size(); i += 32) {
    auto* part = new std::vector<Graph>();
    const size_t e = std::min(graphs.size(), i + 32);
    part->reserve(e - i);
    for (size_t k = i; k < e; ++k) part->push_back(std::move(graphs[k]));
    rt.defer_delete(part, [](void* q) { delete static_cast<std::vector<Graph>*>(q); }, e - i);
  }
  graphs.clear();
}

int64_t Batch::elem_size(int b) const {
  switch (kind) {
    case SCALAR: return 1;
    case LINEAR: return int64_t(M) * C;
    case CTC_TARGETS:
      if (fal) return 2 * int64_t(lab_off[size_t(b) + 1] - lab_off[size_t(b)]);
      return 3 * int64_t(2 * (lab_off[size_t(b) + 1] - lab_off[size_t(b)]) + 1);
    default: return 0;
  }
}

BatchP batch_from_graphs(std::vector<Graph> gs) {
  bool cg = false;
  for (auto& g : gs) cg |= g.calc_grad();
  BatchP b = make_batch(Batch::GRAPHS, int(gs.size()), cg);
  b->graphs = std::move(gs);
  b->materialised = true;
  return b;
}

namespace {
Graph ctc_target_graph_host(const int* t, int U, int blank, bool cg) {
  const int L = 2 * U + 1;
  std::vector<uint8_t> st(size_t(L), 0), ac(size_t(L), 0);
  std::vector<int> src, dst, lab;
  src.reserve(size_t(3 * L));
  dst.reserve(size_t(3 * L));
  lab.reserve(size_t(3 * L));
  for (int l = 0; l < L; ++l) {
    const int idx = (l - 1) / 2;
    st[size_t(l)] = l == 0;
    ac[size_t(l)] = l == L - 1 || l + 2 == L;
    const int label = l % 2 ? t[idx] : blank;
    src.push_back(l), dst.push_back(l), lab.push_back(label);
    if (l > 0) src.push_back(l - 1), dst.push_back(l), lab.push_back(label);
    if (l % 2 && l > 1 && label != t[idx - 1]) src.push_back(l - 2), dst.push_back(l), lab.push_back(label);
  }
  Graph g(cg);
  g.add_nodes(L, st.data(), ac.data());
  g.add_arcs(int(src.size()), src.data(), dst.data(), lab.data(), lab.data(), nullptr);
  g.arc_sort(false);
  return g;
}
}

BatchP batch_ctc_targets(const int* labels, const int* lengths, int n, int blank, bool calc_grad) {
  GTNX_HOST_T("batch.ctc_targets");
  if (n < 0) throw_invalid("[gtnx_batch_ctc_targets] negative batch size");
  BatchP b = make_batch(Batch::CTC_TARGETS, n, calc_grad);
  b->blank = blank;
  b->lab_off.resize(size_t(n) + 1);
  b->lab_off[0] = 0;
  for (int i = 0; i < n; ++i) {
    if (lengths[i] < 0) throw_invalid("[gtnx_batch_ctc_targets] negative length");
    b->lab_off[size_t(i) + 1] = b->lab_off[size_t(i)] + lengths[i];
    b->max_nodes = std::max(b->max_nodes, 2 * lengths[i] + 1);
  }
  const size_t total = size_t(b->lab_off[size_t(n)]);
  b->labels.assign(labels, labels + total);
  int mn = blank;
  b->max_label = blank;
  for (size_t i = 0; i < total; ++i) {
    b->max_label = std::max(b->max_label, labels[i]);
    mn = std::min(mn, labels[i]);
  }
  if (mn < 0 || b->max_nodes > band_max_nodes() || n == 0) {
    std::vector<Graph> gs;
    gs.reserve(size_t(n));
    for (int i = 0; i < n; ++i)
      gs.push_back(ctc_target_graph_host(labels + b->lab_off[size_t(i)], lengths[i], blank, calc_grad));
    return batch_from_graphs(std::move(gs));
  }
  Runtime& rt = Runtime::get();
  const size_t lab_bytes = align_up(sizeof(int) * (total ? total : 1), 256);
  const size_t arg_bytes = align_up(sizeof(CtcTargetArgs) * size_t(n), 256);
  size_t bytes = lab_bytes + arg_bytes;
  b->rec_off.resize(size_t(n));
  for (int i = 0; i < n; ++i) {
    const size_t N = size_t(2 * lengths[i] + 1);
    b->rec_off[size_t(i)] = bytes;
    bytes += align_up(sizeof(BandNode) * N, 64) + align_up(N, 64) + 2 * align_up(4 * N, 64) + 64;
  }
  b->rec_mem = rt.alloc(bytes);
  PinnedMemP pin = rt.alloc_pinned(lab_bytes + arg_bytes);
  std::memcpy(pin->ptr, labels, sizeof(int) * total);
  CtcTargetArgs* args = reinterpret_cast<CtcTargetArgs*>(static_cast<char*>(pin->ptr) + lab_bytes);
  for (int i = 0; i < n; ++i) {
    const size_t N = size_t(2 * lengths[i] + 1);
    char* base = b->rec_mem->as<char>(b->rec_off[size_t(i)]);
    CtcTargetArgs& a = args[size_t(i)];
    a.labels = b->rec_mem->as<int>() + b->lab_off[size_t(i)];
    a.nodes = reinterpret_cast<BandNode*>(base);
    base += align_up(sizeof(BandNode) * N, 64);
    a.nflags = reinterpret_cast<uint8_t*>(base);
    base += align_up(N, 64);
    a.snode = reinterpret_cast<int*>(base);
    base += align_up(4 * N, 64);
    a.slab = reinterpret_cast<int*>(base);
    base += align_up(4 * N, 64);
    a.n_arcs = reinterpret_cast<int*>(base);
    a.N = int(N);
    a.pad = 0;
  }
  rt.h2d_pinned(b->rec_mem->ptr, pin->ptr, lab_bytes + arg_bytes);
  launch_ctc_targets(reinterpret_cast<const CtcTargetArgs*>(b->rec_mem->as<char>(lab_bytes)), n, blank, rt.stream());
  return b;
}


BatchP batch_asg_force_align(const int* labels, const int* lengths, int n, Graph& transitions, int n_labels) {
  if (n < 0) throw_invalid("[gtnx_batch_asg_force_align] negative batch size");
  if (transitions.num_nodes() != int64_t(n_labels) + 1 || transitions.num_arcs() != int64_t(n_labels) * (n_labels + 1))
    throw_invalid("[gtnx_batch_asg_force_align] the transitions graph must have the asgTransitions(N) layout");
  BatchP b = make_batch(Batch::CTC_TARGETS, n, transitions.calc_grad());
  b->fal = true;
  b->trans = transitions;
  b->trans_labels = n_labels;
  b->lab_off.resize(size_t(n) + 1);
  b->lab_off[0] = 0;
  int max_u = 0;
  for (int i = 0; i < n; ++i) {
    if (lengths[i] < 0) throw_invalid("[gtnx_batch_asg_force_align] negative length");
    b->lab_off[size_t(i) + 1] = b->lab_off[size_t(i)] + lengths[i];
    max_u = std::max(max_u, lengths[i]);
  }
  b->max_nodes = max_u + 1;
  const size_t total = size_t(b->lab_off[size_t(n)]);
  b->labels.assign(labels, labels + total);
  int mn = 0;
  for (size_t i = 0; i < total; ++i) {
    b->max_label = std::max(b->max_label, labels[i]);
    mn = std::min(mn, labels[i]);
  }
  if (mn < 0 || b->max_label >= n_labels || b->max_nodes > band_max_nodes() || n == 0) {
    b->kind = Batch::GRAPHS;
    batch_materialise(*b);
    return b;
  }
  Runtime& rt = Runtime::get();
  std::vector<Weights*> ws{transitions.w.get()};
  ensure_weights_device_batch(ws);
  size_t bytes = align_up(sizeof(int) * (total ? total : 1), 256);
  b->rec_off.resize(size_t(n));
  b->w_off.resize(size_t(n));
  b->map_off.resize(size_t(n));
  for (int i = 0; i < n; ++i) {
    const size_t N = size_t(lengths[i]) + 1, A = 2 * size_t(lengths[i]);
    b->rec_off[size_t(i)] = bytes;
    bytes += align_up(sizeof(BandNode) * N, 64) + align_up(N, 64) + 2 * align_up(4 * N, 64);
    b->w_off[size_t(i)] = bytes;
    bytes += align_up(4 * (A ? A : 1), 64);
    b->map_off[size_t(i)] = bytes;
    bytes += align_up(4 * (A ? A : 1), 64);
  }
  b->rec_mem = rt.alloc(bytes);
  {
    PinnedMemP pin = rt.alloc_pinned(sizeof(int) * (total ? total : 1));
    std::memcpy(pin->ptr, labels, sizeof(int) * total);
    rt.h2d_pinned(b->rec_mem->ptr, pin->ptr, sizeof(int) * total);
  }
  std::vector<AsgFalArgs> args;
  args.resize(size_t(n));
  for (int i = 0; i < n; ++i) {
    const size_t N = size_t(lengths[i]) + 1;
    char* base = b->rec_mem->as<char>(b->rec_off[size_t(i)]);
    AsgFalArgs& a = args[size_t(i)];
    a.labels = b->rec_mem->as<int>() + b->lab_off[size_t(i)];
    a.trans_w = transitions.w->dev;
    a.nodes = reinterpret_cast<BandNode*>(base);
    base += align_up(sizeof(BandNode) * N, 64);
    a.nflags = reinterpret_cast<uint8_t*>(base);
    base += align_up(N, 64);
    a.snode = reinterpret_cast<int*>(base);
    base += align_up(4 * N, 64);
    a.slab = reinterpret_cast<int*>(base);
    a.w = b->rec_mem->as<float>(b->w_off[size_t(i)]);
    a.arc_map = b->rec_mem->as<int>(b->map_off[size_t(i)]);
    a.U = lengths[i];
    a.pad = 0;
  }
  DevMemP d = upload_vec(args);
  launch_asg_fal_targets(d->as<AsgFalArgs>(), n, n_labels, rt.stream());
  auto op = std::make_shared<BFalOp>();
  op->seq = g_batch_seq.fetch_add(1);
  b->op = op;
  return b;
}

BatchP batch_linear(int n, int M, int C, bool calc_grad, const void* dev, bool borrow) {
  if (n < 0 || M < 0 || C < 0) throw_invalid("[gtnx_batch_linear] negative size");
  Runtime& rt = Runtime::get();
  BatchP b = make_batch(Batch::LINEAR, n, calc_grad);
  b->M = M;
  b->C = C;
  const size_t bytes = sizeof(float) * size_t(n) * size_t(M) * size_t(C);
  if (borrow && dev) {
    b->w_mem = std::make_shared<DevMem>();
    b->w_mem->ptr = const_cast<void*>(dev);
    b->w_mem->bytes = bytes;
    b->w_mem->borrowed = true;
  } else {
    b->w_mem = dev ? rt.alloc(bytes ? bytes : 4) : rt.alloc_zero(bytes ? bytes : 4);
    if (dev && bytes) rt.d2d(b->w_mem->ptr, dev, bytes);
  }
  b->w_dev = b->w_mem->as<float>();
  return b;
}

BatchP batch_ctc_targets_from_graphs(const std::vector<Graph>& gs) {
  GTNX_HOST_T("batch.ctc_targets_from_graphs");
  const int n = int(gs.size());
  if (n == 0) return nullptr;
  detect_ctc_shape(*gs[0].s);
  const Structure& s0 = *gs[0].s;
  if (!s0.ctc_labels) return nullptr;
  const bool cg = gs[0].calc_grad();
  std::vector<int> flat, len;
  len.reserve(size_t(n));
  flat.reserve(size_t(n) * s0.ctc_labels->size());
  for (auto& g : gs) {
    detect_ctc_shape(*g.s);
    const Structure& s = *g.s;
    if (!s.ctc_labels || s.ctc_blank != s0.ctc_blank || g.calc_grad() != cg || s.N > band_max_nodes() ||
        !g.w->is_all_zero())
      return nullptr;
    flat.insert(flat.end(), s.ctc_labels->begin(), s.ctc_labels->end());
    len.push_back(int(s.ctc_labels->size()));
  }
  BatchP b = batch_ctc_targets(flat.data(), len.data(), n, s0.ctc_blank, cg);
  if (b->kind != Batch::CTC_TARGETS) return nullptr;
  b->graphs = gs;
  b->leaf = true;
  for (auto& g : gs) g.s->leaf_batch = b;
  return b;
}

BatchP batch_linear_from_graphs(const std::vector<Graph>& gs) {
  GTNX_HOST_T("batch.linear_from_graphs");
  const int n = int(gs.size());
  if (n == 0) return nullptr;
  const Structure& s0 = *gs[0].s;
  if (s0.kind != KIND_LINEAR || s0.M < 1 || s0.C < 1) return nullptr;
  const bool cg = gs[0].calc_grad();
  std::vector<Weights*> ws;
  ws.reserve(size_t(n));
  std::unordered_set<Weights*> distinct;
  for (auto& g : gs) {
    const Structure& s = *g.s;
    if (s.kind != KIND_LINEAR || s.M != s0.M || s.C != s0.C || g.calc_grad() != cg || g.w->host_escaped ||
        !distinct.insert(g.w.get()).second)
      return nullptr;
    ws.push_back(g.w.get());
  }
  ensure_weights_device_batch(ws);
  Runtime& rt = Runtime::get();
  const size_t A = size_t(s0.M) * size_t(s0.C);
  BatchP b = make_batch(Batch::LINEAR, n, cg);
  b->M = s0.M;
  b->C = s0.C;
  bool contiguous = true;
  for (int i = 0; i < n && contiguous; ++i)
    contiguous = ws[size_t(i)]->dev == ws[0]->dev + size_t(i) * A && ws[size_t(i)]->dev_mem == ws[0]->dev_mem;
  if (contiguous) {
    b->w_mem = ws[0]->dev_mem;
    b->w_dev = ws[0]->dev;
  } else {
    b->w_mem = rt.alloc(sizeof(float) * A * size_t(n));
    b->w_dev = b->w_mem->as<float>();
    std::vector<CopySeg> segs;
    segs.resize(size_t(n));
    for (int i = 0; i < n; ++i) segs[size_t(i)] = {b->w_dev + size_t(i) * A, ws[size_t(i)]->dev, int64_t(4 * A)};
    DevMemP d = upload_vec(segs);
    launch_copy_segments(d->as<CopySeg>(), n, int64_t(4 * A), rt.stream());
    for (int i = 0; i < n; ++i) {
      ws[size_t(i)]->dev_mem = b->w_mem;
      ws[size_t(i)]->dev = b->w_dev + size_t(i) * A;
    }
  }
  b->graphs = gs;
  b->leaf = true;
  for (auto& g : gs) {
    g.w->leaf_batch = b;
    g.w->leaf_version = g.w->version;
  }
  if (cg && gs[0].g->grad_dest && !gs[0].is_grad_available()) {
    bool block = true;
    for (int i = 0; i < n && block; ++i)
      block = gs[size_t(i)].g->grad_dest == gs[0].g->grad_dest + size_t(i) * A && !gs[size_t(i)].is_grad_available();
    if (block) {
      b->dest_mem = gs[0].g->grad_dest_mem;
      b->dest = gs[0].g->grad_dest;
    }
  }
  return b;
}

namespace {
void push_grads_to_graphs(Batch& x) {
  if (!x.g_dev) return;
  GTNX_HOST_T("batch.push_grads_to_graphs");
  GradSink sink;
  const size_t n = size_t(x.n);
  for (size_t i = 0; i < n; ++i) {
    if (i + 6 < n) __builtin_prefetch(x.graphs[i + 6].g.get(), 1);
    if (i + 3 < n) __builtin_prefetch(x.graphs[i + 3].s.get(), 1);
    Graph& g = x.graphs[i];
    if (!g.calc_grad()) continue;
    float* ptr = x.g_dev + x.g_off[i];
    if (!g.s->deferred) {
      std::lock_guard<std::mutex> lk(g.s->grad_lock);
      if (!g.is_grad_available()) {
        g.g->lazy_owner = x.g_mem;
        g.g->lazy_ptr = ptr;
        continue;
      }
    }
    sink.add(g, x.g_mem, ptr);
  }
  sink.flush();
  x.g_dev = nullptr;
  x.g_mem.reset();
}
}

void batch_materialise(Batch& x) {
  if (x.materialised) return;
  if (x.leaf) {
    x.materialised = true;
    push_grads_to_graphs(x);
    return;
  }
  GraphSlabScope slab_scope(size_t(x.n > 0 ? x.n : 0));
  std::vector<Graph> gs;
  switch (x.fal && x.kind == Batch::GRAPHS ? Batch::CTC_TARGETS : x.kind) {
    case Batch::GRAPHS: break;
    case Batch::CTC_TARGETS:
      gs.reserve(size_t(x.n));
      if (x.fal) {
        std::vector<Graph> fals;
        for (int i = 0; i < x.n; ++i) {
          const int* t = x.labels.data() + x.lab_off[size_t(i)];
          const int U = x.lab_off[size_t(i) + 1] - x.lab_off[size_t(i)];
          Graph f(false);
          f.add_node(true, U == 0);
          for (int l = 1; l <= U; ++l) {
            f.add_node(false, l == U);
            f.add_arc(l - 1, l, t[l - 1], t[l - 1], 0.0f);
            f.add_arc(l, l, t[l - 1], t[l - 1], 0.0f);
          }
          fals.push_back(std::move(f));
        }
        std::vector<Graph> tr{x.trans};
        gs = op_compose(fals, tr, false);
        break;
      }
      for (int i = 0; i < x.n; ++i)
        gs.push_back(ctc_target_graph_host(x.labels.data() + x.lab_off[size_t(i)],
                                           x.lab_off[size_t(i) + 1] - x.lab_off[size_t(i)], x.blank, x.calc_grad));
      break;
    case Batch::LINEAR: {
      gs.reserve(size_t(x.n));
      const int64_t A = int64_t(x.M) * x.C;
      for (int i = 0; i < x.n; ++i) {
        Graph g = Graph::make_result(x.calc_grad);
        Structure& s = *g.s;
        s.kind = KIND_LINEAR;
        s.M = x.M;
        s.C = x.C;
        s.N = int64_t(x.M) + 1;
        s.A = A;
        s.ilabel_sorted = s.olabel_sorted = true;
        Weights& w = *g.w;
        w.n = A;
        if (x.w_pend) x.w_pend->settle();
        w.dev_mem = x.w_mem;
        w.dev = x.w_dev + size_t(i) * size_t(A);
        w.dev_valid = true;
        w.host_valid = false;
        w.version++;
        gs.push_back(std::move(g));
      }
      break;
    }
    case Batch::PRODUCT: {
      batch_materialise(*x.fixed);
      batch_materialise(*x.chain);
      CompMode symbolic;
      gs = x.chain_first ? op_compose(x.chain->graphs, x.fixed->graphs, x.intersect)
                         : op_compose(x.fixed->graphs, x.chain->graphs, x.intersect);
      break;
    }
    case Batch::SCALAR: {
      if (!x.v_mem && x.v_dev) {
        Runtime& rt = Runtime::get();
        x.v_mem = rt.alloc(sizeof(float) * size_t(x.n ? x.n : 1));
        rt.d2d(x.v_mem->ptr, x.v_dev, sizeof(float) * size_t(x.n));
        x.v_dev = x.v_mem->as<float>();
      }
      if (!x.op) {
        gs.reserve(size_t(x.n));
        for (int i = 0; i < x.n; ++i) {
          Graph g(false);
          Structure& s = *g.s;
          s.kind = KIND_LINEAR;
          s.M = s.C = 1;
          s.N = 2;
          s.A = 1;
          Weights& w = *g.w;
          w.n = 1;
          w.dev_mem = x.v_mem;
          w.dev = x.v_dev + i;
          w.dev_valid = true;
          w.host_valid = false;
          w.version++;
          gs.push_back(std::move(g));
        }
        break;
      }
      for (auto& in : x.op->inputs) batch_materialise(*in);
      if (auto* so = dynamic_cast<BScalarOp*>(x.op.get())) {
        std::vector<Graph> none;
        gs = op_scalar(so->kind, so->inputs[0]->graphs, so->inputs.size() > 1 ? so->inputs[1]->graphs : none);
      } else {
        gs = op_shortest_distance(x.op->inputs[0]->graphs, false);
      }
      break;
    }
  }
  if (x.kind != Batch::GRAPHS || x.fal) x.graphs = std::move(gs);
  x.materialised = true;
  if (x.g_dev && ((x.kind == Batch::CTC_TARGETS && !x.fal) || x.kind == Batch::LINEAR)) {
    for (int i = 0; i < x.n; ++i) x.graphs[size_t(i)].add_grad_device(x.g_mem, x.g_dev + x.g_off[size_t(i)], true);
    x.g_dev = nullptr;
    x.g_mem.reset();
  }
}

Graph batch_get(const BatchP& x, int i) {
  if (i < 0 || i >= x->n) throw_range("[gtnx_batch_get] element index out of range");
  batch_materialise(*x);
  return x->graphs[size_t(i)];
}

BatchP batch_compose(const BatchP& a, const BatchP& b, bool intersect) {
  const Batch *fx = nullptr, *ch = nullptr;
  bool chain_first = false;
  if (native(*a, Batch::CTC_TARGETS) && native(*b, Batch::LINEAR)) fx = a.get(), ch = b.get();
  if (native(*a, Batch::LINEAR) && native(*b, Batch::CTC_TARGETS)) fx = b.get(), ch = a.get(), chain_first = true;
  if (fx && a->n == b->n && ch->C >= band_min_labels() && ch->C <= band_max_labels() && fx->max_label < ch->C && ch->M <= (1 << 20)) {
    struct Op : BatchOp {
      void backward(Batch&) override {}
    };
    auto op = std::make_shared<Op>();
    op->inputs = {a, b};
    BatchP r = result(Batch::PRODUCT, a->n, op);
    r->fixed = chain_first ? b : a;
    r->chain = chain_first ? a : b;
    r->chain_first = chain_first;
    r->intersect = intersect;
    return r;
  }
  batch_materialise(*a);
  batch_materialise(*b);
  return batch_from_graphs(op_compose(a->graphs, b->graphs, intersect));
}

BatchP batch_shortest_distance(const BatchP& x, bool tropical) {
  GTNX_HOST_T("batch.shortest_distance");
  Runtime& rt = Runtime::get();
  if (!tropical && native(*x, Batch::PRODUCT) && !x->materialised) {
    Batch& fx = *x->fixed;
    Batch& ch = *x->chain;
    const int n = x->n, T = ch.M, C = ch.C;
    auto op = std::make_shared<BFsBandOp>();
    op->inputs = {x};
    const bool want_norm = ch.nc_norm == nullptr;
    size_t bytes = align_up(4 * size_t(n), 256);
    const size_t o_norm = bytes;
    bytes = align_up(bytes + 4 * size_t(n), 256);
    const size_t o_lse = bytes;
    bytes = align_up(bytes + 4 * size_t(n) * size_t(T > 0 ? T : 1), 256);
    std::vector<size_t> oo, ao;
    oo.resize(size_t(n));
    ao.resize(size_t(n));
    for (int b = 0; b < n; ++b) {
      const int Ub = fx.lab_off[size_t(b) + 1] - fx.lab_off[size_t(b)];
      const int N = fx.fal ? Ub + 1 : 2 * Ub + 1;
      const int ns = band_row_stride(N, band_npl(N));
      oo[size_t(b)] = bytes;
      bytes = align_up(bytes + 8 * (4 * size_t(T) + 16), 256);
      ao[size_t(b)] = bytes;
      bytes = align_up(bytes + 4 * size_t(T + 1) * size_t(ns), 256);
    }
    op->arena = rt.alloc(bytes);
    op->pairs.resize(size_t(n));
    std::vector<std::pair<BandLaunchKey, BandPair>> tab;
    tab.reserve(size_t(n));
    double abytes = 0;
    std::shared_ptr<PendingCopy> pend = ch.w_pend;
    std::unique_lock<std::mutex> pend_lock;
    bool fuse_copy = false;
    if (pend && !pend->done.load(std::memory_order_acquire)) {
      pend_lock = std::unique_lock<std::mutex>(pend->mu);
      fuse_copy = !pend->done.load(std::memory_order_relaxed) && pend->device == rt.device();
      const size_t A = size_t(T) * size_t(C);
      for (int b = 0; b < n && fuse_copy; ++b) fuse_copy = pend->src_of(ch.w_dev + size_t(b) * A) != nullptr;
      fuse_copy = fuse_copy && pend->segs.size() == size_t(n);
      if (!fuse_copy) {
        pend_lock.unlock();
        pend->settle();
      }
    }
    int64_t goff_run = 0;
    for (int b = 0; b < n; ++b) {
      BandPair& p = op->pairs[size_t(b)];
      p = BandPair{};
      const int U = fx.lab_off[size_t(b) + 1] - fx.lab_off[size_t(b)];
      const size_t N = fx.fal ? size_t(U) + 1 : size_t(2 * U + 1);
      char* base = fx.rec_mem->as<char>(fx.rec_off[size_t(b)]);
      p.nodes = reinterpret_cast<BandNode*>(base);
      base += align_up(sizeof(BandNode) * N, 64);
      p.nflags = reinterpret_cast<uint8_t*>(base);
      base += align_up(N, 64);
      p.snode = reinterpret_cast<int*>(base);
      base += align_up(4 * N, 64);
      p.slab = reinterpret_cast<int*>(base);
      p.n_lab = fx.fal ? U : int(N);
      p.w = fx.fal ? fx.rec_mem->as<float>(fx.w_off[size_t(b)]) : nullptr;
      p.em = ch.w_dev + size_t(b) * size_t(T) * size_t(C);
      p.N = int(N);
      p.T = T;
      p.C = C;
      p.NS = band_row_stride(p.N, band_npl(p.N));
      p.alpha = op->arena->as<float>(ao[size_t(b)]);
      p.aoff = op->arena->as<double>(oo[size_t(b)]);
      p.score = op->arena->as<float>(4 * size_t(b));
      if (want_norm) {
        p.norm = op->arena->as<float>(o_norm + 4 * size_t(b));
        p.rowlse = op->arena->as<float>(o_lse + 4 * size_t(b) * size_t(T));
      }
      p.hot = (!fx.fal && U + 1 >= 8) ? fx.blank : -1;
      p.lgrn = band_forward_lgrn(C);
      p.bidx = b;
      p.goff = goff_run;
      goff_run += int64_t(fx.elem_size(b));
      BandPair q = p;
      if (fuse_copy) {
        q.em = static_cast<const float*>(pend->src_of(p.em));
        q.em_copy = const_cast<float*>(p.em);
      }
      tab.push_back({BandLaunchKey{C, band_npl(q.N), fx.fal ? 0 : 1, 0, band_vec_ok(q)}, q});
      abytes += 4.0 * T * C + 4.0 * double(T + 1) * p.NS + (fuse_copy ? 4.0 * T * C : 0.0);
    }
    band_launch(tab, false, "band_forward_score", abytes, fuse_copy ? nullptr : &op->fwd_table);
    if (fuse_copy) pend->done.store(true, std::memory_order_release);
    if (want_norm) {
      ch.nc_mem = op->arena;
      ch.nc_norm = op->arena->as<float>(o_norm);
      ch.nc_rowlse = op->arena->as<float>(o_lse);
    }
    DevMemP arena = op->arena;
    BatchP r = result(Batch::SCALAR, n, op);
    r->v_mem = arena;
    r->v_dev = arena->as<float>();
    return r;
  }
  if (!tropical && native(*x, Batch::LINEAR) && !x->materialised && x->nc_norm) {
    auto op = std::make_shared<BFsLinearOp>();
    op->inputs = {x};
    BatchP r = result(Batch::SCALAR, x->n, op);
    r->v_mem = x->nc_mem;
    r->v_dev = x->nc_norm;
    return r;
  }
  if (!tropical && native(*x, Batch::LINEAR) && !x->materialised && x->n > 0 && x->M > 0) {
    if (x->w_pend) x->w_pend->settle();
    auto op = std::make_shared<BFsLinearOp>();
    op->inputs = {x};
    const int n = x->n;
    DevMemP res = rt.alloc(sizeof(float) * size_t(n) * 9);
    float* scal = res->as<float>();
    float* partial = scal + n;
    std::vector<LinArgs> args;
    args.resize(size_t(n));
    const size_t A = size_t(x->M) * size_t(x->C);
    for (int b = 0; b < n; ++b) {
      LinArgs& a = args[size_t(b)];
      a.w = x->w_dev + size_t(b) * A;
      a.M = x->M;
      a.C = x->C;
      a.out_score = scal + b;
      a.partial = partial + size_t(b) * 8;
      a.delta = nullptr;
      a.grad = nullptr;
      a.accumulate = 0;
    }
    DevMemP d = upload_vec(args);
    const bool vec_rows = x->C % 4 == 0 && x->C <= 1024 && (reinterpret_cast<uintptr_t>(x->w_dev) & 15) == 0 && (A % 4) == 0;
    {
      GTNX_PROF("linear_forward", 4.0 * double(A) * n);
      launch_linear_forward(d->as<LinArgs>(), n, 0, vec_rows ? 1 : 0, rt.stream());
    }
    BatchP r = result(Batch::SCALAR, n, op);
    r->v_mem = res;
    r->v_dev = scal;
    return r;
  }
  batch_materialise(*x);
  return batch_from_graphs(op_shortest_distance(x->graphs, tropical));
}

BatchP batch_viterbi_path(const BatchP& x) {
  batch_materialise(*x);
  return batch_from_graphs(op_viterbi_path(x->graphs));
}


namespace {
BatchP scalars_from_graphs(const BatchP& gsb) {
  Runtime& rt = Runtime::get();
  for (auto& g : gsb->graphs)
    if (g.num_arcs() != 1) return nullptr;
  auto op = std::make_shared<BFromGraphsOp>();
  op->inputs = {gsb};
  BatchP r = result(Batch::SCALAR, gsb->n, op);
  r->v_mem = rt.alloc(sizeof(float) * size_t(gsb->n ? gsb->n : 1));
  r->v_dev = r->v_mem->as<float>();
  items_device(gsb->graphs, r->v_dev);
  return r;
}
}

BatchP batch_scalar(ScalarKind k, const BatchP& a0, const BatchP& b0, void* items_dev) {
  BatchP a = a0, b = b0;
  const bool binary = k != SK_NEGATE;
  if (binary && a->n == b->n) {
    const bool an = a->kind == Batch::SCALAR && !a->materialised, bn = b->kind == Batch::SCALAR && !b->materialised;
    if (an && !bn && b->kind == Batch::GRAPHS) {
      if (BatchP w = scalars_from_graphs(b)) b = w;
    } else if (bn && !an && a->kind == Batch::GRAPHS) {
      if (BatchP w = scalars_from_graphs(a)) a = w;
    }
  }

  if (native(*a, Batch::SCALAR) && !a->materialised &&
      (!binary || (native(*b, Batch::SCALAR) && !b->materialised && b->n == a->n))) {
    Runtime& rt = Runtime::get();
    auto op = std::make_shared<BScalarOp>();
    op->kind = k;
    op->inputs = binary ? std::vector<BatchP>{a, b} : std::vector<BatchP>{a};
    BatchP r = result(Batch::SCALAR, a->n, op);
    if (items_dev) {
      r->v_dev = static_cast<float*>(items_dev);
    } else {
      r->v_mem = rt.alloc(sizeof(float) * size_t(a->n ? a->n : 1));
      r->v_dev = r->v_mem->as<float>();
    }
    launch_vec_axpby(r->v_dev, a->v_dev, binary ? b->v_dev : nullptr, size_t(a->n), k == SK_NEGATE ? -1.0f : 1.0f,
                     k == SK_SUBTRACT ? -1.0f : 1.0f, 0, rt.stream());
    return r;
  }
  batch_materialise(*a);
  std::vector<Graph> none;
  if (binary) batch_materialise(*b);
  BatchP r = batch_from_graphs(op_scalar(k, a->graphs, binary ? b->graphs : none));
  if (items_dev) batch_items_device(r, items_dev);
  return r;
}

void batch_backward(const BatchP& root, bool retain) {
  GTNX_HOST_T("batch.backward");
  if (root->tape_cleared)
    throw_invalid("[autograd::backward] Cannot Backward twice without retaining the graph.");
  if (root->materialised || !root->op || root->kind != Batch::SCALAR) {
    batch_materialise(*root);
    op_backward(root->graphs, nullptr, retain);
    return;
  }
  Runtime& rt = Runtime::get();
  std::vector<Batch*> order;
  std::unordered_set<Batch*> seen;
  std::vector<BatchP> hold;
  std::vector<BatchP> stack{root};
  while (!stack.empty()) {
    BatchP b = stack.back();
    stack.pop_back();
    if (!b->calc_grad || !seen.insert(b.get()).second) continue;
    hold.push_back(b);
    if (b->op) {
      order.push_back(b.get());
      for (auto& in : b->op->inputs) stack.push_back(in);
    }
  }
  std::sort(order.begin(), order.end(), [](Batch* a, Batch* b) { return a->op->seq > b->op->seq; });
  bool root_done = false;
  if (!root->g_dev) {
    alloc_grad(*root, false);
    auto* sop = dynamic_cast<BScalarOp*>(root->op.get());
    bool plain = sop != nullptr && !sop->inputs.empty() && sop->inputs.size() <= 2;
    if (plain)
      for (auto& in : sop->inputs) plain = plain && in->kind == Batch::SCALAR && !in->materialised && in->n == root->n;
    if (plain && sop->inputs.size() == 2 && sop->inputs[0].get() == sop->inputs[1].get()) plain = false;
    if (plain) {
      float* g[2] = {nullptr, nullptr};
      float sc[2] = {0.0f, 0.0f};
      int acc[2] = {0, 0};
      for (size_t i = 0; i < sop->inputs.size(); ++i) {
        Batch& in = *sop->inputs[i];
        if (!in.calc_grad) continue;
        sc[i] = (sop->kind == SK_NEGATE || (sop->kind == SK_SUBTRACT && i == 1)) ? -1.0f : 1.0f;
        acc[i] = in.g_dev != nullptr;
        if (!in.g_dev) alloc_grad(in, false);
        g[i] = in.g_dev;
      }
      launch_scalar_seed(root->g_dev, g[0], sc[0], acc[0], g[1], sc[1], acc[1], size_t(root->n), rt.stream());
      root_done = true;
    } else {
      launch_fill_f32(root->g_dev, 1.0f, size_t(root->n), rt.stream());
    }
  } else {
    DevMemP ones = rt.alloc(sizeof(float) * size_t(root->n ? root->n : 1));
    launch_fill_f32(ones->as<float>(), 1.0f, size_t(root->n), rt.stream());
    launch_vec_axpby(root->g_dev, ones->as<float>(), nullptr, size_t(root->n), 1.0f, 0.0f, 1, rt.stream());
  }
  std::vector<Batch*> from_graphs;
  BackwardPlan plan;
  t_plan = &plan;
  struct RetainScope {
    bool prev;
    explicit RetainScope(bool r) : prev(t_batch_retain) { t_batch_retain = r; }
    ~RetainScope() { t_batch_retain = prev; }
  } retain_scope(retain);
  try {
    for (Batch* b : order) {
      if (!b->g_dev) continue;
      if (root_done && b == root.get()) continue;
      if (auto* f = dynamic_cast<BFromGraphsOp*>(b->op.get())) {
        f->retain = retain;
        from_graphs.push_back(b);
        continue;
      }
      b->op->backward(*b);
    }
    for (auto& kv : plan.lin)
      if (!plan.fused.count(kv.first)) static_cast<BFsLinearOp*>(kv.second->op.get())->run(*kv.second);
  } catch (...) {
    t_plan = nullptr;
    throw;
  }
  t_plan = nullptr;
  for (Batch* b : seen)
    if ((b->materialised || b->leaf) && b->g_dev && !b->op) push_grads_to_graphs(*b);
  for (Batch* b : from_graphs) b->op->backward(*b);
  if (!retain)
    for (Batch* b : order) {
      if (b != root.get()) {
        b->g_dev = nullptr;
        b->g_mem.reset();
      }
      b->op.reset();
      b->tape_cleared = true;
    }
}

void batch_items_device(const BatchP& x, void* dev_out) {
  if (x->kind == Batch::SCALAR && !x->materialised) {
    if (static_cast<const void*>(x->v_dev) == dev_out) return;
    Runtime::get().d2d(dev_out, x->v_dev, sizeof(float) * size_t(x->n));
    return;
  }
  batch_materialise(*x);
  items_device(x->graphs, dev_out);
}
float batch_item_host(const BatchP& x, int i) {
  if (i < 0 || i >= x->n) throw_range("[gtnx_batch_get] element index out of range");
  if (!x->host_vals_valid) {
    x->host_vals.resize(size_t(x->n));
    if (x->host_ev) {
      Runtime::get().drain_until(x->host_ev);
      std::memcpy(x->host_vals.data(), x->host_pin->ptr, sizeof(float) * size_t(x->n));
      (void)hipEventDestroy(static_cast<hipEvent_t>(x->host_ev));
      x->host_ev = nullptr;
      x->host_pin.reset();
    } else {
      Runtime::get().d2h_sync(x->host_vals.data(), x->v_dev, sizeof(float) * size_t(x->n));
    }
    x->host_vals_valid = true;
  }
  return x->host_vals[size_t(i)];
}
void batch_prefetch_items(const BatchP& x) {
  if (!x || x->kind != Batch::SCALAR || x->materialised || x->host_vals_valid || x->host_ev || x->n <= 0 || !x->v_dev) return;
  Runtime& rt = Runtime::get();
  hipEvent_t ev;
  if (hipEventCreateWithFlags(&ev, hipEventDisableTiming) != hipSuccess) {
    (void)hipGetLastError();
    return;
  }
  x->host_pin = rt.alloc_pinned(sizeof(float) * size_t(x->n));
  rt.d2h_pinned_async(x->host_pin->ptr, x->v_dev, sizeof(float) * size_t(x->n));
  HIP_CHECK(hipEventRecord(ev, rt.stream()));
  x->host_ev = ev;
}
void batch_items_host(const BatchP& x, float* out) {
  if (x->kind == Batch::SCALAR && !x->materialised) {
    Runtime::get().d2h_sync(out, x->v_dev, sizeof(float) * size_t(x->n));
    return;
  }
  batch_materialise(*x);
  items_host(x->graphs, out);
}
void batch_grads_bind(const BatchP& x, void* dev_out, const int64_t* offsets) {
  if (x->materialised) {
    grads_bind_device(x->graphs, dev_out, offsets);
    return;
  }
  if (x->kind != Batch::LINEAR && x->kind != Batch::SCALAR) return;
  int64_t o = 0;
  for (int i = 0; i < x->n; ++i) {
    if (offsets[i] != offsets[0] + o) return;
    o += x->elem_size(i);
  }
  if (x->n == 0) return;
  x->dest_mem = std::make_shared<DevMem>();
  x->dest_mem->ptr = dev_out;
  x->dest_mem->borrowed = true;
  x->dest = static_cast<float*>(dev_out) + offsets[0];
}
void batch_grads_device(const BatchP& x, void* dev_out, const int64_t* offsets) {
  if (x->kind == Batch::CTC_TARGETS) batch_materialise(*x);
  if (x->materialised) {
    grads_device(x->graphs, dev_out, offsets);
    return;
  }
  if (!x->g_dev) throw_logic("[gtn::Graph::grad] Gradient not calculated yet.");
  Runtime& rt = Runtime::get();
  std::vector<AxpyArgs> ax;
  int64_t maxn = 0;
  for (int i = 0; i < x->n; ++i) {
    float* dst = static_cast<float*>(dev_out) + offsets[i];
    float* src = x->g_dev + x->g_off[size_t(i)];
    if (dst == src) continue;
    const int64_t len = x->g_off[size_t(i) + 1] - x->g_off[size_t(i)];
    ax.push_back({dst, src, len, 1.0f});
    maxn = std::max(maxn, len);
  }
  if (ax.empty()) return;
  DevMemP d = upload_vec(ax);
  launch_axpy_batch(d->as<AxpyArgs>(), int(ax.size()), maxn,  2, rt.stream());
}

}
```

### gtn_amd/csrc/batch.h

```cpp
#pragma once

#include <memory>
#include <vector>

#include "ops.h"

namespace gtnx {

struct Batch;
using BatchP = std::shared_ptr<Batch>;

struct BatchOp {
  uint64_t seq = 0;
  std::vector<BatchP> inputs;
  virtual void backward(Batch& out) = 0;
  virtual ~BatchOp() {}
};

struct Batch {
  enum Kind { GRAPHS, CTC_TARGETS, LINEAR, PRODUCT, SCALAR };
  Kind kind = GRAPHS;
  int n = 0;
  bool calc_grad = false;

  bool materialised = false;
  std::vector<Graph> graphs;
  bool leaf = false;
  struct Origin {
    std::shared_ptr<void> home;
    size_t begin, end;
  };
  std::vector<Origin> origins;
  void (*give_back)(const std::shared_ptr<void>& home, std::vector<Graph>* part) = nullptr;
  std::vector<float> host_vals;
  bool host_vals_valid = false;
  PinnedMemP host_pin;
  void* host_ev = nullptr;

  std::vector<int> labels, lab_off;
  int blank = 0;
  int max_label = -1, max_nodes = 0;
  DevMemP rec_mem;
  std::vector<size_t> rec_off;
  bool fal = false;
  Graph trans;
  int trans_labels = 0;
  std::vector<size_t> w_off, map_off;
  int M = 0, C = 0;
  DevMemP w_mem;
  float* w_dev = nullptr;
  std::shared_ptr<PendingCopy> w_pend;
  DevMemP nc_mem;
  float* nc_norm = nullptr;
  float* nc_rowlse = nullptr;
  BatchP fixed, chain;
  bool chain_first = false, intersect = false;
  DevMemP v_mem;
  float* v_dev = nullptr;

  std::shared_ptr<BatchOp> op;
  bool tape_cleared = false;
  DevMemP g_mem;
  float* g_dev = nullptr;
  std::vector<int64_t> g_off;
  DevMemP dest_mem;
  float* dest = nullptr;

  int64_t elem_size(int b) const;
  ~Batch();
};

BatchP batch_from_graphs(std::vector<Graph> gs);
BatchP batch_ctc_targets(const int* labels, const int* lengths, int n, int blank, bool calc_grad);
BatchP batch_asg_force_align(const int* labels, const int* lengths, int n, Graph& transitions, int n_labels);
BatchP batch_linear(int n, int M, int C, bool calc_grad, const void* dev, bool borrow);
BatchP batch_compose(const BatchP& a, const BatchP& b, bool intersect);
BatchP batch_shortest_distance(const BatchP& x, bool tropical);
BatchP batch_viterbi_path(const BatchP& x);
BatchP batch_scalar(ScalarKind k, const BatchP& a, const BatchP& b, void* items_dev = nullptr);
void batch_backward(const BatchP& root, bool retain);
void batch_items_host(const BatchP& x, float* out);
void batch_items_device(const BatchP& x, void* dev_out);
void batch_grads_device(const BatchP& x, void* dev_out, const int64_t* offsets);
void batch_grads_bind(const BatchP& x, void* dev_out, const int64_t* offsets);
Graph batch_get(const BatchP& x, int i);
float batch_item_host(const BatchP& x, int i);
void batch_prefetch_items(const BatchP& x);
BatchP batch_ctc_targets_from_graphs(const std::vector<Graph>& gs);
BatchP batch_linear_from_graphs(const std::vector<Graph>& gs);
void batch_materialise(Batch& x);

}
```

### gtn_amd/csrc/capi.cpp

```cpp
#include <atomic>
#include <chrono>
#include <condition_variable>
#include <cstdlib>
#include <cstring>
#include <mutex>
#include <string>
#include <vector>

#include "batch.h"
#include "ops.h"
#include "ops_internal.h"
#include "region.h"

#define GTNX_API extern "C" __attribute__((visibility("default")))

using namespace gtnx;

namespace {
thread_local std::string g_err;

gtnx_status_t fail(gtnx_status_t s, const std::string& m) {
  g_err = m;
  return s;
}

template <class F>
gtnx_status_t guard(F&& f) {
  try {
    f();
    return GTNX_OK;
  } catch (const Error& e) {
    return fail(e.status, e.what());
  } catch (const std::bad_alloc&) {
    return fail(GTNX_RUNTIME_ERROR, "out of host memory");
  } catch (const std::exception& e) {
    return fail(GTNX_RUNTIME_ERROR, e.what());
  }
}

inline Graph& RAW(gtnx_graph_t h) {
  if (!h) throw_invalid("null graph handle");
  return *reinterpret_cast<Graph*>(h);
}
inline Graph& GL(gtnx_graph_t h) {
  Graph& g = RAW(h);
  if (g.s->pending) return region_value(g);
  if (g.s->device >= 0 && g.s->device != Runtime::current_device()) {
    const bool host_only = !g.s->dev_valid && !g.s->lazy && !g.s->deferred && (!g.w || (!g.w->dev_valid && !g.w->staged)) &&
                           (!g.g || !g.is_grad_available());
    if (host_only) {
      g.s->device = Runtime::current_device();
      return g;
    }
    throw_invalid("[gtn_amd] this graph lives on device " + std::to_string(g.s->device) + ", the calling thread is on device " +
                  std::to_string(Runtime::current_device()) + " (gtnx_set_device)");
  }
  return g;
}
inline Graph& G(gtnx_graph_t h) {
  Graph& g = GL(h);
  if (g.s->lazy) realize(g);
  if (g.s->deferred) g.s->resolve_sizes();
  return g;
}
struct HandleSlab {
  std::atomic<int> live;
};
struct HandleEntry {
  Graph g;
  HandleSlab* slab;
};
HandleEntry* new_handles(size_t n) {
  const size_t head = (sizeof(HandleSlab) + alignof(HandleEntry) - 1) / alignof(HandleEntry) * alignof(HandleEntry);
  char* raw = static_cast<char*>(::operator new(head + sizeof(HandleEntry) * (n ? n : 1)));
  HandleSlab* s = new (raw) HandleSlab();
  s->live.store(int(n), std::memory_order_relaxed);
  HandleEntry* e = reinterpret_cast<HandleEntry*>(raw + head);
  for (size_t i = 0; i < n; ++i) {
    new (&e[i].g) Graph(Graph::Empty{});
    e[i].slab = s;
  }
  return e;
}
inline gtnx_graph_t H(Graph g) {
  HandleEntry* e = new_handles(1);
  e->g = std::move(g);
  return reinterpret_cast<gtnx_graph_t>(&e->g);
}

std::vector<Graph> vec(const gtnx_graph_t* a, int n, bool lazy_ok = false) {
  std::vector<Graph> v;
  v.reserve(n > 0 ? n : 0);
  for (int i = 0; i < n; ++i) v.push_back(lazy_ok ? GL(a[i]) : G(a[i]));
  return v;
}
void put(std::vector<Graph>& r, gtnx_graph_t* out) {
  if (r.empty()) return;
  HandleEntry* e = new_handles(r.size());
  for (size_t i = 0; i < r.size(); ++i) {
    e[i].g = std::move(r[i]);
    out[i] = reinterpret_cast<gtnx_graph_t>(&e[i].g);
  }
}
bool is_device_pointer(const void* p) {
  static const bool have_gpu = Runtime::device_count() > 0;
  if (!have_gpu || !p) return false;
  hipPointerAttribute_t attr;
  if (hipPointerGetAttributes(&attr, p) != hipSuccess) {
    (void)hipGetLastError();
    return false;
  }
  return attr.type == hipMemoryTypeDevice;
}
void check_node(Graph& g, int n) {
  if (n < 0 || n >= g.num_nodes()) throw_range("node index out of range");
}
void check_arc(Graph& g, int a) {
  if (a < 0 || a >= g.num_arcs()) throw_range("arc index out of range");
}
}

namespace gtnx {
void destroy_handle(Graph* g) {
  HandleEntry* e = reinterpret_cast<HandleEntry*>(g);
  HandleSlab* s = e->slab;
  e->g.~Graph();
  if (s->live.fetch_sub(1, std::memory_order_acq_rel) == 1) {
    s->~HandleSlab();
    ::operator delete(static_cast<void*>(s));
  }
}
}

GTNX_API gtnx_status_t gtnx_parallel_enter(void) {
  return guard([&] { region_enter(); });
}
GTNX_API gtnx_status_t gtnx_parallel_leave(void) {
  return guard([&] { region_leave(); });
}
GTNX_API gtnx_status_t gtnx_parallel_flush(void) {
  return guard([&] { region_flush(); });
}

GTNX_API const char* gtnx_last_error(void) { return g_err.c_str(); }
namespace gtnx {
void set_last_error(const std::string& m) { g_err = m; }
}
GTNX_API const char* gtnx_version(void) { return "0.1.0"; }
GTNX_API const char* gtnx_backend(void) { return "hip:gfx950"; }
GTNX_API int gtnx_device_count(void) { return Runtime::device_count(); }
GTNX_API gtnx_status_t gtnx_set_device(int d) {
  return guard([&] { Runtime::set_current_device(d); });
}
GTNX_API gtnx_status_t gtnx_get_device(int* d) {
  return guard([&] { *d = Runtime::current_device(); });
}
GTNX_API gtnx_status_t gtnx_compose_mode(int mode, int* previous) {
  return guard([&] {
    if (mode < -1 || mode > 2) throw_invalid("[gtnx_compose_mode] mode must be -1, 0, 1 or 2");
    const int old = compose_mode_hint(mode);
    if (previous) *previous = old;
  });
}
GTNX_API gtnx_status_t gtnx_set_stream(void* s) {
  return guard([&] { Runtime::get().set_stream(static_cast<hipStream_t>(s)); });
}
GTNX_API gtnx_status_t gtnx_synchronize(void) {
  return guard([&] {
    if (Runtime::initialized()) {
      Runtime::get().sync();
      deferred_resolve_all();
    }
  });
}
GTNX_API gtnx_status_t gtnx_memory_stats(uint64_t* r, uint64_t* u) {
  return guard([&] {
    if (r) *r = 0;
    if (u) *u = 0;
    if (Runtime::initialized()) Runtime::get().stats(r, u);
  });
}
GTNX_API gtnx_status_t gtnx_reclaim(void) {
  return guard([&] {
    region_reclaim_thread();
  });
}
GTNX_API gtnx_status_t gtnx_debug_viterbi_ties(int64_t* seen, int64_t* unresolved) {
  return guard([&] {
    if (seen) *seen = g_viterbi_ties_seen.load();
    if (unresolved) *unresolved = g_viterbi_ties_unresolved.load();
  });
}
GTNX_API gtnx_status_t gtnx_debug_tie_ranks(gtnx_graph_t g, int* queue_rank, int* creation_rank, int* applies) {
  return guard([&] {
    Graph& x = GL(g);
    const std::vector<int>*k = nullptr, *c = nullptr;
    const bool ok = x.s->kind == KIND_EXPLICIT && !x.s->lazy && ctc_tie_ranks(*x.s, true, &k, &c);
    if (applies) *applies = ok ? 1 : 0;
    if (!ok) return;
    if (queue_rank) std::copy(k->begin(), k->end(), queue_rank);
    if (creation_rank) std::copy(c->begin(), c->end(), creation_rank);
  });
}
GTNX_API gtnx_status_t gtnx_empty_cache(void) {
  return guard([&] {
    if (Runtime::initialized()) Runtime::get().empty_cache();
  });
}

GTNX_API gtnx_status_t gtnx_graph_create(int calc_grad, gtnx_graph_t* out) {
  return guard([&] { *out = H(Graph(calc_grad != 0)); });
}
GTNX_API gtnx_status_t gtnx_graph_copy(gtnx_graph_t g, gtnx_graph_t* out) {
  return guard([&] { *out = H(RAW(g)); });
}
GTNX_API gtnx_status_t gtnx_graph_deep_copy(gtnx_graph_t g, gtnx_graph_t* out) {
  return guard([&] { *out = H(Graph::deep_copy(G(g))); });
}
GTNX_API gtnx_status_t gtnx_graph_destroy(gtnx_graph_t g) {
  return guard([&] {
    Graph* p = reinterpret_cast<Graph*>(g);
    if (!p) return;
    if (region_active())
      region_trash(p);
    else if (p->s && p->s->pending)
      destroy_handle(p);
    else if (Runtime::initialized())
      Runtime::send(p->s && p->s->home ? p->s->home : Runtime::home(), p, [](void* q) { destroy_handle(static_cast<Graph*>(q)); });
    else
      destroy_handle(p);
  });
}
GTNX_API gtnx_status_t gtnx_graph_add_node(gtnx_graph_t g, int s, int a, int* id) {
  return guard([&] {
    Graph& gr = G(g);
    region_before_mutation(gr);
    int i = gr.add_node(s != 0, a != 0);
    if (id) *id = i;
  });
}
GTNX_API gtnx_status_t gtnx_graph_add_arc(gtnx_graph_t g, int src, int dst, int il, int ol, float w, int* id) {
  return guard([&] {
    Graph& gr = G(g);
    region_before_mutation(gr);
    int i = gr.add_arc(src, dst, il, ol, w);
    if (id) *id = i;
  });
}
GTNX_API gtnx_status_t gtnx_graph_add_nodes(gtnx_graph_t g, int n, const uint8_t* s, const uint8_t* a) {
  return guard([&] {
    Graph& gr = G(g);
    region_before_mutation(gr);
    gr.add_nodes(n, s, a);
  });
}
GTNX_API gtnx_status_t gtnx_graph_add_arcs(gtnx_graph_t g, int n, const int* src, const int* dst, const int* il,
                                           const int* ol, const float* w) {
  return guard([&] {
    Graph& gr = G(g);
    region_before_mutation(gr);
    gr.add_arcs(n, src, dst, il, ol, w);
  });
}
GTNX_API gtnx_status_t gtnx_graph_num_nodes(gtnx_graph_t g, int64_t* out) {
  return guard([&] { *out = G(g).num_nodes(); });
}
GTNX_API gtnx_status_t gtnx_graph_num_arcs(gtnx_graph_t g, int64_t* out) {
  return guard([&] { *out = G(g).num_arcs(); });
}
GTNX_API gtnx_status_t gtnx_graph_num_start(gtnx_graph_t g, int64_t* out) {
  return guard([&] { *out = G(g).num_start(); });
}
GTNX_API gtnx_status_t gtnx_graph_num_accept(gtnx_graph_t g, int64_t* out) {
  return guard([&] { *out = G(g).num_accept(); });
}
GTNX_API gtnx_status_t gtnx_graph_num_inputs(gtnx_graph_t g, int64_t* out) {
  return guard([&] { *out = int64_t(GL(g).g->inputs.size()); });
}
GTNX_API gtnx_status_t gtnx_graph_item(gtnx_graph_t g, float* out) {
  return guard([&] {
    Graph& raw = RAW(g);
    if (raw.s->pending && region_item(raw, out)) return;
    *out = G(g).item();
  });
}
GTNX_API gtnx_status_t gtnx_graph_arc_sort(gtnx_graph_t g, int ol) {
  return guard([&] {
    Graph& gr = G(g);
    region_before_mutation(gr);
    gr.arc_sort(ol != 0);
  });
}
GTNX_API gtnx_status_t gtnx_graph_mark_arc_sorted(gtnx_graph_t g, int ol) {
  return guard([&] {
    region_before_mutation(G(g));
    Structure& s = *G(g).s;
    bool& flag = ol ? s.olabel_sorted : s.ilabel_sorted;
    if (!flag) {
      flag = true;
      s.dev_valid = s.kind == KIND_LINEAR ? s.dev_valid : false;
    }
  });
}
GTNX_API gtnx_status_t gtnx_graph_ilabel_sorted(gtnx_graph_t g, int* out) {
  return guard([&] { *out = G(g).s->ilabel_sorted; });
}
GTNX_API gtnx_status_t gtnx_graph_olabel_sorted(gtnx_graph_t g, int* out) {
  return guard([&] { *out = G(g).s->olabel_sorted; });
}
GTNX_API gtnx_status_t gtnx_graph_weights(gtnx_graph_t g, int mut, float** out) {
  return guard([&] {
    Graph& gr = G(g);
    if (mut) region_before_mutation(gr);
    *out = const_cast<float*>(gr.weights_host(mut != 0));
  });
}
GTNX_API gtnx_status_t gtnx_graph_get_weights(gtnx_graph_t g, float* out) {
  return guard([&] {
    Graph& gr = G(g);
    const float* p = gr.weights_host(false);
    std::memcpy(out, p, sizeof(float) * size_t(gr.num_arcs()));
  });
}
GTNX_API gtnx_status_t gtnx_graph_set_weights(gtnx_graph_t g, const float* w) {
  return guard([&] {
    Graph& gr = G(g);
    region_before_mutation(gr);
    const bool dev = is_device_pointer(w);
    if (region_stage_weights(gr, w, dev)) return;
    if (dev)
      gr.set_weights_device(w);
    else
      gr.set_weights_host(w);
  });
}
GTNX_API gtnx_status_t gtnx_graph_set_weights_device(gtnx_graph_t g, const void* w) {
  return guard([&] {
    Graph& gr = G(g);
    region_before_mutation(gr);
    if (region_stage_weights(gr, static_cast<const float*>(w), true)) return;
    gr.set_weights_device(w);
  });
}
GTNX_API gtnx_status_t gtnx_graph_weights_device(gtnx_graph_t g, void** out) {
  return guard([&] {
    Graph& gr = G(g);
    std::vector<Weights*> v{gr.w.get()};
    ensure_weights_device_batch(v);
    *out = gr.w->dev;
  });
}
GTNX_API gtnx_status_t gtnx_graph_labels_to_array(gtnx_graph_t g, int* out, int il) {
  return guard([&] {
    Structure& s = *G(g).s;
    if (s.kind == KIND_LINEAR) {
      for (int64_t a = 0; a < s.A; ++a) out[a] = int(a % s.C);
      return;
    }
    s.ensure_host();
    std::memcpy(out, (il ? s.il : s.ol).data(), sizeof(int) * size_t(s.A));
  });
}
GTNX_API gtnx_status_t gtnx_graph_get_start(gtnx_graph_t g, int* out) {
  return guard([&] {
    Structure& s = *G(g).s;
    if (s.kind == KIND_LINEAR) {
      out[0] = 0;
      return;
    }
    s.ensure_host();
    std::memcpy(out, s.start.data(), sizeof(int) * s.start.size());
  });
}
GTNX_API gtnx_status_t gtnx_graph_get_accept(gtnx_graph_t g, int* out) {
  return guard([&] {
    Structure& s = *G(g).s;
    if (s.kind == KIND_LINEAR) {
      if (s.M > 0) out[0] = s.M;
      return;
    }
    s.ensure_host();
    std::memcpy(out, s.accept.data(), sizeof(int) * s.accept.size());
  });
}
GTNX_API gtnx_status_t gtnx_graph_is_start(gtnx_graph_t g, int n, int* out) {
  return guard([&] {
    Graph& gr = G(g);
    check_node(gr, n);
    Structure& s = *gr.s;
    if (s.kind == KIND_LINEAR) {
      *out = n == 0;
      return;
    }
    s.ensure_host();
    *out = (s.nflags[n] & NF_START) != 0;
  });
}
GTNX_API gtnx_status_t gtnx_graph_is_accept(gtnx_graph_t g, int n, int* out) {
  return guard([&] {
    Graph& gr = G(g);
    check_node(gr, n);
    Structure& s = *gr.s;
    if (s.kind == KIND_LINEAR) {
      *out = s.M > 0 && n == s.M;
      return;
    }
    s.ensure_host();
    *out = (s.nflags[n] & NF_ACCEPT) != 0;
  });
}
GTNX_API gtnx_status_t gtnx_graph_make_accept(gtnx_graph_t g, int n) {
  return guard([&] {
    Graph& gr = G(g);
    check_node(gr, n);
    region_before_mutation(gr);
    Structure& s = *gr.s;
    s.materialize();
    s.ensure_host();
    if (!(s.nflags[n] & NF_ACCEPT)) {
      s.accept.push_back(n);
      s.nflags[n] |= NF_ACCEPT;
      s.dev_valid = false;
      s.dev_mem.reset();
      s.rec_mem.reset();
      s.sched.reset();
      s.ctc_labels.reset();
      s.ctc_checked = false;
      s.leaf_batch.reset();
      s.band[0].reset();
      s.band[1].reset();
      s.dense[0].reset();
      s.dense[1].reset();
    }
  });
}
GTNX_API gtnx_status_t gtnx_graph_num_out(gtnx_graph_t g, int n, int64_t* out) {
  return guard([&] {
    check_node(G(g), n);
    *out = G(g).s->num_out(n);
  });
}
GTNX_API gtnx_status_t gtnx_graph_num_in(gtnx_graph_t g, int n, int64_t* out) {
  return guard([&] {
    check_node(G(g), n);
    *out = G(g).s->num_in(n);
  });
}
GTNX_API gtnx_status_t gtnx_graph_get_out(gtnx_graph_t g, int n, int* out) {
  return guard([&] {
    check_node(G(g), n);
    Structure& s = *G(g).s;
    if (s.kind == KIND_LINEAR) {
      if (n < s.M)
        for (int c = 0; c < s.C; ++c) out[c] = n * s.C + c;
      return;
    }
    s.ensure_csr();
    std::memcpy(out, s.out_list.data() + s.out_off[n], sizeof(int) * size_t(s.out_off[n + 1] - s.out_off[n]));
  });
}
GTNX_API gtnx_status_t gtnx_graph_get_in(gtnx_graph_t g, int n, int* out) {
  return guard([&] {
    check_node(G(g), n);
    Structure& s = *G(g).s;
    if (s.kind == KIND_LINEAR) {
      if (n > 0)
        for (int c = 0; c < s.C; ++c) out[c] = (n - 1) * s.C + c;
      return;
    }
    s.ensure_csr();
    std::memcpy(out, s.in_list.data() + s.in_off[n], sizeof(int) * size_t(s.in_off[n + 1] - s.in_off[n]));
  });
// ... 449 lines not shown
```

### gtn_amd/csrc/kernels.h

```cpp
#pragma once

#include <hip/hip_runtime.h>

#include <cstdint>

#include <atomic>
#include <cstdint>
struct gtnx_first_on_device {
  std::atomic<uint64_t>& done;
  uint64_t bit;
  bool first;
  explicit gtnx_first_on_device(std::atomic<uint64_t>& d) : done(d) {
    int dev = 0;
    (void)hipGetDevice(&dev);
    bit = uint64_t(1) << (dev & 63);
    first = !(done.load(std::memory_order_acquire) & bit);
  }
  gtnx_first_on_device(const gtnx_first_on_device&) = delete;
  ~gtnx_first_on_device() {
    if (first) done.fetch_or(bit, std::memory_order_acq_rel);
  }
  explicit operator bool() const { return first; }
};

// ... 53 lines not shown
enum : int { SCHED_TIE_BY_ARC = 1, SCHED_OUT_IDENTITY = 2 };

struct LevelizeOut {
  int* level_off;
  int* row_off;
  int* in_srcpos;
  int* in_arc;
  uint8_t* pflags;
  int* acc_pos;
  int* out_off;
  int* out_dstpos;
  int* out_arc;
};
enum : int { LV_P = 0, LV_L, LV_N_IN, LV_N_OUT, LV_ERROR, LV_MAX_WIDTH, LV_MAX_LEVEL_ARCS, LV_MAX_REACH, LV_INFO_INTS };
size_t levelize_scratch_bytes(int N, int A);
void device_levelize(const DGraph& g, const LevelizeOut& out, void* scratch, int* info_host , hipStream_t st);

struct SdResult {
  float score;
  float max_final;
  int argmax_final;
  int pad;
};

struct SdArgs {
  DSched s;
  const GTNX_G float* w;
  GTNX_G float* scores;
  GTNX_G int* argmax;
  GTNX_G SdResult* result;
  GTNX_G float* out_score;
  const GTNX_G float* delta;
  GTNX_G float* node_grad;
  GTNX_G float* arc_grad;
  int chunk_levels;
  const GTNX_G struct ComposeOut* dyn_out;
  const GTNX_G int* dyn_counts;
  const GTNX_G int* gi_fixed;
  const GTNX_G int* gi_chain;
  GTNX_G float* grad_fixed;
  GTNX_G float* grad_chain;
  int chain_C, fixed_A, chain_A;
  int chain_accumulate;
};

enum : int { SD_LOG = 0, SD_TROPICAL = 1, SD_PATH = 2 };

int sd_narrow_ring();
int sd_narrow_tmp_cap();
int sd_narrow_node_cap();
void launch_sd_forward(const SdArgs* d_args, int n, int mode, int narrow,
                       int avg_in_degree_x16, hipStream_t st);
int sd_deep_node_cap();
void launch_sd_forward_deep(const SdArgs* d_args, int n, int maxP, hipStream_t st);
void launch_sd_backward_deep(const SdArgs* d_args, int n, int maxP, hipStream_t st);
int sd_narrow_ring_backward();
void launch_sd_backward(const SdArgs* d_args, int n, int mode, int narrow, int avg_out_degree_x16, hipStream_t st,
                        int fuse_lds_bytes = 0);
void sd_narrow_fuse_caps(int* cap_fixed, int* cap_chain);

struct PathArgs {
  DSched s;
  DGraph g;
  const GTNX_G int* argmax;
  const GTNX_G SdResult* result;
  GTNX_G int* path_arcs;
  GTNX_G int* path_il;
  GTNX_G int* path_ol;
  GTNX_G float* path_w;
  GTNX_G int* path_len;
  int cap;
  const GTNX_G float* scores;
  const GTNX_G float* w;
  GTNX_G int* path_pos;
  GTNX_G int* pred;
  GTNX_G int* tmp;
};
void launch_path_chase(const PathArgs* d_args, int n, int max_cap, int max_P, hipStream_t st);

struct LinArgs {
  const GTNX_G float* w;
  int M, C;
  GTNX_G float* out_score;
  GTNX_G float* partial;
  const GTNX_G float* delta;
  GTNX_G float* grad;
  int accumulate;
};
void launch_linear_forward(const LinArgs* d_args, int n, int tropical, int vec_rows, hipStream_t st);
void launch_linear_backward(const LinArgs* d_args, int n, int tropical, int vec_rows, hipStream_t st);

enum : int { MATCH_UNSORTED = 0, MATCH_SINGLY_G1 = 1, MATCH_SINGLY_G2 = 2, MATCH_DOUBLY = 3 };

struct ComposeOut {
  int N, A, L;
  int layered;
  int overflow;
  int max_width;
  int max_level_arcs;
  int csr_built;
  int rep_levels;
  int skipped;
  int t_b, t_f, t_rep;
  int wr_L, wr_K, wr_lo, wr_W, wr_na, wr_Aw;
};

constexpr int GF_EPS_FREE = 4;
constexpr int GF_ACCEPTOR = 8;

struct ComposeArgs {
  DGraph g1, g2;
  int matcher;
  int lds_state;
  int skip;
  int chain_bits;
  int rep_grid;
  int Ncap, Acap;
  GTNX_G int* state;
  GTNX_G int* queue;
  GTNX_G int* src;
  GTNX_G int* dst;
  GTNX_G int* il;
  GTNX_G int* ol;
  GTNX_G float* w;
  GTNX_G int* gi1;
  GTNX_G int* gi2;
  GTNX_G uint8_t* nflags;
  GTNX_G int* pair_of;
  GTNX_G int* out_off;
  GTNX_G int* level_off;
  GTNX_G int* in_off;
  GTNX_G int* in_cursor;
  GTNX_G int* in_list;
  GTNX_G int* in_src;
  GTNX_G float* in_w;
  GTNX_G int* start_list;
  GTNX_G int* accept_list;
  GTNX_G int* counts;
  GTNX_G ComposeOut* out;
  int trim_fwd_first;
  const GTNX_G gtnx_i4* s1_out;
  const GTNX_G gtnx_i4* s1_in;
  const GTNX_G gtnx_i4* s2_out;
  const GTNX_G gtnx_i4* s2_in;
};
int compose_max_bitmap_bytes();
size_t compose_chain_bitmap_bytes(int No, int slices);
size_t compose_g1_cache_bytes(int N1, int A1);
int compose_lds_budget(int wide);
void launch_compose(const ComposeArgs* d_args, int n, int matcher, int lin1, int lin2, int dyn_lds_bytes,
                    int fast, int cache1, int wide, hipStream_t st);
void launch_compose_replicate(const ComposeArgs* d_args, int n, int lin2, int max_acap, hipStream_t st);
int compose_wide_node_cap();
void launch_compose_wide(const ComposeArgs* d_args, int n, int lin2, int max_acap, hipStream_t st);
void launch_compose_pairs(const ComposeArgs* d_args, int n, int matcher, hipStream_t st);
void launch_sorted_view(const DGraph& g, int key_olabel, void* out_view , void* in_view, hipStream_t st);
struct ComposeFillArgs {
  int N, A;
  const GTNX_G int* out_off;
  const GTNX_G int* dst;
  const GTNX_G float* w;
  const GTNX_G int* gi1;
  const GTNX_G int* gi2;
  const GTNX_G int* lab1;
  const GTNX_G int* lab2;
  int C1, C2;
  GTNX_G int* src;
  GTNX_G int* il;
  GTNX_G int* ol;
  GTNX_G int* in_cursor;
  GTNX_G int* in_list;
  GTNX_G int* in_src;
  GTNX_G float* in_w;
};
void launch_compose_fill(const ComposeFillArgs& a, hipStream_t st);
size_t compose_transpose_scratch_bytes(int n, int maxNcap);
void launch_compose_transpose(const ComposeArgs* d_args, int n, int maxAcap, int maxNcap, void* scratch,
                              hipStream_t st);

void launch_build_records(const DGraph& g, void* out_rec, void* in_rec, hipStream_t st);

struct ComposeGradArgs {
  const GTNX_G float* delta;
  const GTNX_G int* gi1;
  const GTNX_G int* gi2;
  int A;
  int A1, A2;
  GTNX_G float* grad1;
  GTNX_G float* grad2;
};
void launch_compose_grad(const ComposeGradArgs* d_args, int n, int maxA, hipStream_t st);

struct LazyGroup {
  DGraph g;
  int chain_first;
  int T, C, N, nb;
  int Npad, Cpad;
  const gtnx_i4* lrec_in;
  const gtnx_i4* lrec_out;
  const float* const* em;
  const float* em_base;
  int64_t em_stride;
  float* alpha;
  float* beta;
  int* bp;
  float* score;
  int* best;
  const float* const* delta;
  float* const* grad_em;
  float* grad_fixed;
  const float* E;
  const float* cmax;
  const int* nlab;
  int lab_unique;
  int tie_by_node;
  float* amax;
  float* bmax;
  float* amaxp;
  float* bmaxp;
  int ntp;
  float* R;
  const float* zt;
  float* xt[2];
  const float* Ep;
  const float* ETp;
  int Kpad, Npad2, nbpad;
  int rot;
  int rel;
  const float* mp_Wq;
  const int* mp_colidx;
  const int* mp_colnode;
  const int* mp_dead;
  int mp_ncol, mp_ndead;
};
size_t lazy_step_lds_bytes(const LazyGroup& g);
int lazy_tile_nodes();
int lazy_tile_batch();
void launch_lazy_pack(const LazyGroup& g, gtnx_i4* lrec_in, gtnx_i4* lrec_out, hipStream_t st);
void launch_lazy_init(const LazyGroup& g, int which, hipStream_t st);
void launch_lazy_step(const LazyGroup& g, int t, int mode, int backward, hipStream_t st);
void launch_lazy_final(const LazyGroup& g, int mode, hipStream_t st);
void launch_lazy_path(const LazyGroup& g, int* path_arc, int* path_il, int* path_ol, float* path_w, int* path_len,
                      hipStream_t st);
void launch_lazy_local_z(const LazyGroup& g, float* zt, hipStream_t st);
void launch_lazy_chain_grad(const LazyGroup& g, const int* node_label, hipStream_t st);
bool lazy_z_chain_grad_ok(const LazyGroup& g);
void launch_lazy_z_chain_grad(const LazyGroup& g, const int* node_label, float* zt, hipStream_t st);
void launch_lazy_fixed_grad(const LazyGroup& g, int max_in_deg, hipStream_t st);
struct LazyPathGrad {
  const float* delta;
  int delta_stride;
  const int* path_arc;
  const int* il;
  const int* ol;
  int len, C, chain_first;
  float* grad_chain;
  float* grad_fixed;
};
void launch_lazy_path_grad(const LazyPathGrad& a, hipStream_t st);
struct LazyPair {
  DGraph g;
  const GTNX_G float* em;
  GTNX_G float* alpha;
  GTNX_G float* score;
  const GTNX_G float* delta;
  GTNX_G float* grad_em;
  GTNX_G float* grad_fixed;
  int T, C, chain_first, pad;
};
int lazy_pair_max_nodes();
int lazy_pair_max_degree();
int lazy_pair_block(int max_nodes);
int lazy_pair_max_labels(int block);
void launch_lazy_pair_forward(const LazyPair* d_pairs, int n, int block, int C, int cus, hipStream_t st);
void launch_lazy_pair_backward(const LazyPair* d_pairs, int n, int block, int C, int cus, hipStream_t st);
struct BandNode {
  int lab;
  int aid[3];
};
struct BandPair {
  const GTNX_G BandNode* nodes;
  const GTNX_G uint8_t* nflags;
  const GTNX_G int* snode;
  const GTNX_G int* slab;
  const GTNX_G float* w;
  const GTNX_G float* em;
  GTNX_G float* em_copy;
  GTNX_G float* alpha;
  GTNX_G double* aoff;
  GTNX_G float* score;
  GTNX_G float* norm;
  GTNX_G float* rowlse;
  const GTNX_G float* delta;
  const GTNX_G float* delta_norm;
  GTNX_G float* grad_em;
  GTNX_G float* grad_fixed;
  int N, T, C, NS;
  int hot;
  int lgrn;
  int n_lab;
  int bidx;
  int64_t goff;
};
struct BandPatch {
  int on;
  int M;
  const GTNX_G float* delta;
  const GTNX_G float* delta_norm;
  GTNX_G float* rowlse;
  GTNX_G float* grad_em;
  GTNX_G float* grad_fixed;
  int64_t A;
};
struct BandDecode {
  const GTNX_G BandNode* nodes;
  const GTNX_G uint8_t* nflags;
  const GTNX_G float* w;
  const GTNX_G float* em;
  GTNX_G uint8_t* bp;
  GTNX_G int* pnode;
  GTNX_G int* path_arc;
  GTNX_G int* path_lab;
  GTNX_G float* path_w;
  GTNX_G int* path_len;
  GTNX_G float* score;
  GTNX_G int* tie;
  const GTNX_G int* rank_in;
  const GTNX_G int* rank_acc;
  int N, T, C, NS;
  int stage_floats, pad;
};
void launch_band_viterbi(const BandDecode* d_pairs, int n, int stage_floats, int max_nodes, int max_labels, int vec,
                         hipStream_t st, int ranked = 0);
bool band_viterbi_wave_ok(int max_nodes, int max_labels, int vec);
struct RationalSeg {
  DGraph g;
  int node_off, arc_off;
  int conn_off;
  int keep_start, keep_accept;
  int pad;
};
struct RationalOut {
  int N, A;
  GTNX_G int* src;
  GTNX_G int* dst;
  GTNX_G int* il;
  GTNX_G int* ol;
  GTNX_G float* w;
  GTNX_G uint8_t* nflags;
  GTNX_G int* start_list;
  GTNX_G int* accept_list;
  GTNX_G int* out_off;
  GTNX_G int* out_list;
  GTNX_G int* in_off;
  GTNX_G int* in_list;
};
size_t rational_csr_temp_bytes(int N, int A);
void launch_rational_build(const RationalSeg* d_segs, int nseg, int max_A, int max_N, int max_conn, const RationalOut& out,
                           int projection, int closure, void* temp, hipStream_t st);
void launch_rational_adjacency(const RationalOut& out, void* temp, hipStream_t st);
struct RemoveArgs {
  DGraph g;
  int ilabel, olabel;
  const GTNX_G int* new_id;
  const GTNX_G int* roots;
  int K, root0, rows;
  GTNX_G int* stamp;
  GTNX_G int* queue;
  GTNX_G int* arc_cnt;
  const GTNX_G int* arc_off;
  RationalOut out;
};
void launch_remove_keep(const DGraph& g, int ilabel, int olabel, int* keep, hipStream_t st);
void launch_remove_roots(const int* keep, const int* new_id, int N, int* roots, hipStream_t st);
void launch_remove_walk(const RemoveArgs& a, bool emit, hipStream_t st);
size_t scan_temp_bytes(int n);
void launch_exclusive_scan(const int* in, int* out, int n, void* temp, size_t temp_bytes, hipStream_t st);
void launch_rational_load(const void* rows, const float* w, const uint8_t* flags, const RationalOut& out, void* temp,
                          hipStream_t st);
struct CtcTargetArgs {
  const GTNX_G int* labels;
  GTNX_G BandNode* nodes;
  GTNX_G uint8_t* nflags;
  GTNX_G int* snode;
  GTNX_G int* slab;
  GTNX_G int* n_arcs;
  int N, pad;
};
void launch_ctc_targets(const CtcTargetArgs* d_args, int n, int blank, hipStream_t st);
struct AsgFalArgs {
  const GTNX_G int* labels;
  const GTNX_G float* trans_w;
  GTNX_G BandNode* nodes;
  GTNX_G uint8_t* nflags;
  GTNX_G int* snode;
  GTNX_G int* slab;
  GTNX_G float* w;
  GTNX_G int* arc_map;
  int U, pad;
};
void launch_asg_fal_targets(const AsgFalArgs* d_args, int n, int n_labels, hipStream_t st);
void launch_asg_fal_scatter(const float* g, const int* maps, const int64_t* tab , int n_seq, int64_t longest,
                            float* trans_grad, hipStream_t st);
int band_max_nodes();
int band_max_labels();
int band_min_labels();
int band_npl(int max_nodes);
int band_row_stride(int N, int npl);
int band_forward_lgrn(int C);
bool band_one_ok(int npl, int C, int max_NS, bool vec, bool backward);
void launch_band_forward(const BandPair* d_pairs, int n, int npl, int C, int max_NS, bool unit, bool vec, hipStream_t st,
                         const BandPair* one = nullptr);
void launch_band_backward(const BandPair* d_pairs, int n, int npl, int C, int max_NS, bool unit, bool gradg, bool vec,
                          hipStream_t st, const BandPair* one = nullptr, const BandPatch* patch = nullptr);
void launch_lazy_dense_prep(const LazyGroup& g, float* E, float* cmax, hipStream_t st);
void launch_lazy_dense_step(const LazyGroup& g, int t, int backward, hipStream_t st, const float* vin = nullptr,
                            float* vout = nullptr);
void launch_lazy_dense_fixed_grad(const LazyGroup& g, hipStream_t st);
size_t maxplus_w_floats(const LazyGroup& g);
void launch_maxplus_prep(const LazyGroup& g, hipStream_t st);
void launch_maxplus_step(const LazyGroup& g, int t, hipStream_t st);
void launch_maxplus_path(const LazyGroup& g, int* path_arc, int* path_il, int* path_ol, float* path_w, int* path_len,
                         hipStream_t st);
void launch_lazy_mfma_prep(const LazyGroup& g, hipStream_t st);
void launch_lazy_mfma_init(const LazyGroup& g, int which, hipStream_t st);
void launch_lazy_mfma_step(const LazyGroup& g, int t, int backward, hipStream_t st);
size_t lazy_mfma_chain_sync_ints(const LazyGroup& g);
bool launch_lazy_mfma_chain(const LazyGroup& g, int backward, int* zeroed_sync, int cus, hipStream_t st);
void launch_lazy_mfma_keys(float* keys, int64_t n, hipStream_t st);
void launch_lazy_mfma_rowmax(const LazyGroup& g, int which, hipStream_t st);
void launch_lazy_mfma_score(const LazyGroup& g, hipStream_t st);
size_t lazy_mfma_fixed_grad_scratch_bytes(const LazyGroup& g);
void launch_lazy_mfma_fixed_grad(const LazyGroup& g, void* pair_consts , hipStream_t st, void* partials = nullptr,
                                 size_t partials_bytes = 0);

void launch_fill_i32(int* p, int v, size_t n, hipStream_t st);
void launch_fill_f32(float* p, float v, size_t n, hipStream_t st);
void launch_scalar_seed(float* root, float* g0, float s0, int acc0, float* g1, float s1, int acc1, size_t n, hipStream_t st);
struct ScalarArgs {
  const GTNX_G float* a;
  const GTNX_G float* b;
  GTNX_G float* out;
  GTNX_G float* mirror;
};
void launch_scalar_combine(const ScalarArgs* d_args, int n, float sa, float sb, hipStream_t st);
void launch_copy_small(void* dst, const void* src, size_t bytes, hipStream_t st);
void launch_scalar_combine_one(const ScalarArgs& a, float sa, float sb, hipStream_t st);
struct ScalarFanArgs {
  const GTNX_G float* d;
  GTNX_G float* seed;
  GTNX_G float* o0;
  GTNX_G float* o1;
};
void launch_scalar_fan(const ScalarFanArgs* d_args, int n, float s0, float s1, hipStream_t st);
void launch_scalar_fan_one(const ScalarFanArgs& a, float s0, float s1, hipStream_t st);
struct AxpyArgs {
  GTNX_G float* dst;
  const GTNX_G float* src;
  int64_t n;
  float scale;
};
void launch_axpy_batch(const AxpyArgs* d_args, int n, int64_t maxn, int atomic, hipStream_t st);
struct CopySeg {
  void* dst;
  const void* src;
  int64_t bytes;
};
void launch_copy_segments(const CopySeg* d_segs, int n, int64_t max_bytes, hipStream_t st);
void launch_gather_scalars(const float* const* d_ptrs, float* out, int n, hipStream_t st);
void launch_vec_axpby(float* out, const float* a, const float* b, size_t n, float sa, float sb, int accumulate, hipStream_t st);
struct ScatterArgs {
  const GTNX_G int* idx;
  const GTNX_G float* delta;
  GTNX_G float* grad;
  int n;
};
void launch_scatter_add(const ScatterArgs* d_args, int n, int maxn, hipStream_t st);
void launch_linear_materialize(int M, int C, int* src, int* dst, int* il, int* ol, hipStream_t st);

}
```

### gtn_amd/csrc/ops.h

```cpp
#pragma once

#include <cstring>
#include <tuple>
#include <vector>

#include "graph.h"

namespace gtnx {

struct Member {
  int idx;
  Graph out;
};

struct OpRecord {
  uint64_t seq = 0;
  virtual void backward(std::vector<Member>& members) = 0;
  virtual bool joins_chain_plan() const { return false; }
  virtual ~OpRecord() {}
};

struct GradSink {
  struct Item {
    Graph g;
    DevMemP owner;
    float* ptr;
  };
  std::vector<Item> items;
  void add(const Graph& g, const DevMemP& owner, float* ptr) {
    if (g.calc_grad()) items.push_back({g, owner, ptr});
  }
  void flush();
};

struct BandLaunchKey {
  int C, npl, unit, gradg, vec;
  bool operator<(const BandLaunchKey& o) const {
    return std::tie(C, npl, unit, gradg, vec) < std::tie(o.C, o.npl, o.unit, o.gradg, o.vec);
  }
  bool operator==(const BandLaunchKey& o) const { return !(*this < o) && !(o < *this); }
};
int band_vec_ok(const BandPair& p);
void band_launch(std::vector<std::pair<BandLaunchKey, BandPair>>& tab, bool backward, const char* prof_name = nullptr,
                 double prof_bytes = 0.0, DevMemP* table_out = nullptr);
void band_launch_patched(const DevMemP& table, int n, const BandLaunchKey& key, int max_ns, const BandPatch& patch,
                         const char* prof_name, double prof_bytes);

enum ScalarKind { SK_NEGATE = 0, SK_ADD = 1, SK_SUBTRACT = 2 };

std::vector<Graph> op_scalar(ScalarKind k, std::vector<Graph>& a, std::vector<Graph>& b);
std::vector<Graph> op_shortest_distance(std::vector<Graph>& gs, bool tropical);
std::vector<Graph> op_viterbi_path(std::vector<Graph>& gs);
std::vector<Graph> op_compose(std::vector<Graph>& a, std::vector<Graph>& b, bool intersect);
enum RationalKind { RAT_CLONE = 0, RAT_CONCAT = 1, RAT_CLOSURE = 2, RAT_UNION = 3 };
Graph op_rational(int kind, std::vector<Graph>& inputs, int projection);
Graph op_remove(Graph& g, int ilabel, int olabel);
Graph op_load_buffer(const void* data, size_t bytes);
void op_backward(std::vector<Graph>& roots, Graph* grad, bool retain, bool seed = true);
void backward_validate(Graph& root);
int compose_mode_hint(int mode);
void realize(Graph& g);

Graph make_scalar_graph(float v, bool calc_grad);
Graph make_linear_graph(int M, int N, bool calc_grad);
std::vector<Graph> make_linear_graphs_device(int B, int M, int N, bool calc_grad, const void* dev, bool borrow = false);
Graph make_user_op(std::vector<Graph>& inputs, gtnx_grad_fn fn, void* ctx, void (*ctx_free)(void*));
void set_user_grad_fn(Graph& g, gtnx_grad_fn fn, void* ctx, void (*ctx_free)(void*));

void items_host(std::vector<Graph>& gs, float* out);
void items_device(std::vector<Graph>& gs, void* dev_out);
void grads_device(std::vector<Graph>& gs, void* dev_out, const int64_t* offsets);
void grads_bind_device(std::vector<Graph>& gs, void* dev_out, const int64_t* offsets);

inline bool upload_in_place(size_t bytes) {
  static const size_t lim = [] {
    const char* e = std::getenv("GTNX_ARGS_IN_PLACE");
    return e ? size_t(std::atol(e)) : size_t(0);
  }();
  return bytes <= lim;
}
template <class T>
DevMemP upload_vec(const std::vector<T>& v) {
  Runtime& rt = Runtime::get();
  size_t bytes = sizeof(T) * v.size();
  if (bytes && upload_in_place(bytes)) {
    PinnedMemP p = rt.alloc_pinned(bytes);
    std::memcpy(p->ptr, v.data(), bytes);
    DevMemP d = std::make_shared<DevMem>();
    d->ptr = p->ptr;
    d->bytes = bytes;
    d->borrowed = true;
    d->keep = p;
    return d;
  }
  DevMemP d = rt.alloc(bytes ? bytes : 1);
  if (bytes) {
    PinnedMemP p = rt.alloc_pinned(bytes);
    std::memcpy(p->ptr, v.data(), bytes);
    rt.h2d_pinned(d->ptr, p->ptr, bytes);
  }
  return d;
}

}
```

### gtn_amd/csrc/ops_band.cpp

```cpp
#include "ops_internal.h"

#include <memory>

namespace gtnx {

int band_vec_ok(const BandPair& p) { return p.C % 4 == 0 && (reinterpret_cast<uintptr_t>(p.em) & 15) == 0; }
void band_launch_patched(const DevMemP& table, int n, const BandLaunchKey& k, int max_ns, const BandPatch& patch,
                         const char* prof_name, double prof_bytes) {
  Runtime& rt = Runtime::get();
  std::unique_ptr<Runtime::Scope> prof(prof_name ? new Runtime::Scope(&rt, prof_name, prof_bytes) : nullptr);
  launch_band_backward(table->as<BandPair>(), n, k.npl, k.C, max_ns, k.unit != 0, k.gradg != 0, k.vec != 0, rt.stream(), nullptr,
                       &patch);
}
void band_launch(std::vector<std::pair<BandLaunchKey, BandPair>>& tab, bool backward, const char* prof_name, double prof_bytes,
                 DevMemP* table_out) {
  Runtime& rt = Runtime::get();
  if (table_out) table_out->reset();
  if (tab.empty()) return;
  bool one_key = true;
  for (size_t i = 1; i < tab.size() && one_key; ++i) one_key = tab[i].first == tab[0].first;
  if (!one_key) std::stable_sort(tab.begin(), tab.end(), [](const auto& x, const auto& y) { return x.first < y.first; });
  if (tab.size() == 1) {
    const BandLaunchKey& k = tab[0].first;
    const BandPair& p = tab[0].second;
    if (band_one_ok(k.npl, k.C, p.NS, k.vec != 0, backward)) {
      std::unique_ptr<Runtime::Scope> prof(prof_name ? new Runtime::Scope(&rt, prof_name, prof_bytes) : nullptr);
      if (backward) launch_band_backward(nullptr, 1, k.npl, k.C, p.NS, k.unit != 0, k.gradg != 0, true, rt.stream(), &p);
      else launch_band_forward(nullptr, 1, k.npl, k.C, p.NS, k.unit != 0, true, rt.stream(), &p);
      return;
    }
  }
  std::vector<BandPair> flat;
  flat.reserve(tab.size());
  for (auto& e : tab) flat.push_back(e.second);
  DevMemP d = upload_vec(flat);
  const BandPair* dp = d->as<BandPair>();
  if (table_out && one_key) *table_out = d;
  std::unique_ptr<Runtime::Scope> prof(prof_name ? new Runtime::Scope(&rt, prof_name, prof_bytes) : nullptr);
  for (size_t i0 = 0; i0 < tab.size();) {
    size_t i1 = i0;
    int max_ns = 0;
    while (i1 < tab.size() && tab[i1].first == tab[i0].first) max_ns = std::max(max_ns, tab[i1++].second.NS);
    const BandLaunchKey& k = tab[i0].first;
    if (backward)
      launch_band_backward(dp + i0, int(i1 - i0), k.npl, k.C, max_ns, k.unit != 0, k.gradg != 0, k.vec != 0, rt.stream());
    else
      launch_band_forward(dp + i0, int(i1 - i0), k.npl, k.C, max_ns, k.unit != 0, k.vec != 0, rt.stream());
    i0 = i1;
  }
}
bool band_shape_ok(const Structure& cs, Structure& fs, bool chain_first) {
  if (cs.kind != KIND_LINEAR || cs.C < band_min_labels() || cs.C > band_max_labels() || cs.M < 0 || cs.M > (1 << 20)) return false;
  std::shared_ptr<BandInfo> b = band_info(fs, chain_first);
  return b->ok && b->max_label < cs.C;
}
bool band_ok(const LazyProduct& lp, std::shared_ptr<BandInfo>* out) {
  if (!band_shape_ok(*lp.chain.s, *lp.fixed.s, lp.chain_side == 1)) return false;
  if (out) *out = band_info(*lp.fixed.s, lp.chain_side == 1);
  return true;
}
static bool tie_ranks(Structure& fs, BandInfo& bi, bool use_ilabel);
void band_prepare(const std::vector<Graph*>& fixed, const std::vector<uint8_t>& chain_first, bool want_ranks) {
  std::vector<size_t> todo;
  std::unordered_set<Structure*> seen;
  for (size_t i = 0; i < fixed.size(); ++i) {
    Structure* st = fixed[i]->s.get();
    const std::shared_ptr<BandInfo>& b = st->band[chain_first[i] ? 0 : 1];
    if ((!b || (want_ranks && b->ok && b->rank_state == 0)) && seen.insert(st).second) todo.push_back(i);
  }
  auto body = [&](size_t q) {
    Graph& g = *fixed[todo[q]];
    std::shared_ptr<BandInfo> b = band_info(*g.s, chain_first[todo[q]] != 0);
    (void)g.w->is_all_zero();
    if (want_ranks && b && b->ok) (void)tie_ranks(*g.s, *b, chain_first[todo[q]] != 0);
  };
  if (todo.size() >= 64) gtn::detail::runIndexed(todo.size(), body, 32, false);
  else for (size_t q = 0; q < todo.size(); ++q) body(q);
}

struct BandSdOp : OpRecord {
  std::vector<BandPair> pairs;
  std::vector<Graph> chains, fixed;
  std::vector<std::shared_ptr<BandInfo>> infos;
  std::vector<uint8_t> unit;
  DevMemP arena;

  using Key = BandLaunchKey;
  static int band_vec(const BandPair& p) { return band_vec_ok(p); }
  static void launch(std::vector<std::pair<Key, BandPair>>& tab, bool backward, const char* prof_name = nullptr, double prof_bytes = 0.0) {
    band_launch(tab, backward, prof_name, prof_bytes);
  }

  void backward(std::vector<Member>& ms) override {
    Runtime& rt = Runtime::get();
    size_t eb = 0, fb = 0;
    std::vector<size_t> eo(ms.size(), 0), fo(ms.size(), 0);
    std::vector<float*> dest(ms.size(), nullptr);
    std::vector<DevMemP> dest_mem(ms.size());
    for (size_t k = 0; k < ms.size(); ++k) {
      const int i = ms[k].idx;
      if (chains[i].calc_grad()) {
        GradState& cg = *chains[i].g;
        if (cg.grad_dest && !chains[i].is_grad_available()) {
          dest[k] = cg.grad_dest;
          dest_mem[k] = cg.grad_dest_mem;
          cg.grad_dest = nullptr;
        } else {
          eo[k] = eb;
          eb = align_up(eb + 4 * size_t(pairs[i].T) * size_t(pairs[i].C), 256);
        }
      }
      if (fixed[i].calc_grad()) {
        fo[k] = fb;
        fb = align_up(fb + 4 * size_t(fixed[i].s->A), 256);
      }
    }
    DevMemP gem = rt.alloc(eb ? eb : 1);
    DevMemP gfx = rt.alloc_zero(fb ? fb : 1);
    ChainGradPlan local;
    ChainGradPlan& plan = t_chain_plan ? *t_chain_plan : local;
    plan.keep.push_back(gem);
    plan.keep.push_back(gfx);
    plan.keep.push_back(arena);
    for (size_t k = 0; k < ms.size(); ++k) {
      plan.keep.push_back(infos[ms[k].idx]->dev_mem);
      plan.keep.push_back(chains[ms[k].idx].w->dev_mem);
      plan.keep.push_back(fixed[ms[k].idx].w->dev_mem);
    }
    for (size_t k = 0; k < ms.size(); ++k) {
      const int i = ms[k].idx;
      BandPair p = pairs[i];
      p.delta = through_delta(ms[k].out);
      p.delta_norm = nullptr;
      p.grad_em = chains[i].calc_grad() ? (dest[k] ? dest[k] : gem->as<float>(eo[k])) : nullptr;
      p.grad_fixed = fixed[i].calc_grad() ? gfx->as<float>(fo[k]) : nullptr;
      plan.band.push_back({p.C, band_npl(p.N), int(unit[i]), p.grad_fixed ? 1 : 0, band_vec(p), p, chains[i].w.get()});
      if (p.grad_em) plan.sink.add(chains[i], dest[k] ? dest_mem[k] : gem, p.grad_em);
      if (p.grad_fixed) plan.sink.add(fixed[i], gfx, p.grad_fixed);
      ms[k].out.g->inputs[0].g->grad_propagated = true;
      plan.bytes += 4.0 * p.T * p.C * (p.grad_em ? 2 : 1) + 4.0 * double(p.T + 1) * p.NS +
                    (p.grad_fixed ? 4.0 * double(fixed[i].s->A) : 0.0);
    }
    if (!t_chain_plan) {
      t_chain_plan = &local;
      flush_chain_plan();
      t_chain_plan = nullptr;
    }
  }
  bool joins_chain_plan() const override { return true; }
};

void flush_chain_plan() {
  ChainGradPlan* plan = t_chain_plan;
  if (!plan || plan->empty()) return;
    std::vector<std::pair<BandSdOp::Key, BandPair>> tab;
  tab.reserve(plan->band.size());
  for (auto& b : plan->band) {
    auto it = b.p.grad_em ? plan->lin.find(b.chain_w) : plan->lin.end();
    if (it != plan->lin.end() && !it->second.fused) {
      b.p.delta_norm = it->second.delta;
      b.p.rowlse = const_cast<float*>(it->second.rowlse);
      it->second.fused = true;
    } else {
      b.p.delta_norm = nullptr;
    }
    tab.push_back({BandSdOp::Key{b.C, b.npl, b.unit, b.gradg, b.vec}, b.p});
  }
  if (!tab.empty()) {
    BandSdOp::launch(tab, true, "band_forward_score_grad", plan->bytes);
  }
  plan->sink.flush();
  std::vector<Member> rest;
  std::vector<Graph> rest_in;
  for (auto& kv : plan->lin)
    if (!kv.second.fused) {
      rest.push_back(kv.second.m);
      rest_in.push_back(kv.second.chain);
    }
  if (!rest.empty()) {
    linear_sd_backward_now(rest, rest_in);
  }
  plan->band.clear();
  plan->lin.clear();
  plan->keep.clear();
  plan->bytes = 0;
}

std::vector<Graph> band_forward_score(std::vector<Graph>& gs) {
  GraphSlabScope slab_scope(gs.size());
  Runtime& rt = Runtime::get();
  auto op = std::make_shared<BandSdOp>();
  op->seq = next_seq();
  const size_t n = gs.size();
  std::vector<BandInfo*> bis;
  std::vector<Structure*> ss;
  std::vector<Weights*> ws;
  op->unit.resize(n);
  {
    std::vector<Graph*> fx(n);
    std::vector<uint8_t> cf(n);
    for (size_t i = 0; i < n; ++i) {
      fx[i] = &gs[i].s->lazy->fixed;
      cf[i] = gs[i].s->lazy->chain_side == 1;
    }
    band_prepare(fx, cf);
  }
  op->chains.reserve(n);
  op->fixed.reserve(n);
  op->infos.reserve(n);
  for (size_t i = 0; i < n; ++i) {
    LazyProduct& lp = *gs[i].s->lazy;
    std::shared_ptr<BandInfo> b;
    band_ok(lp, &b);
    op->chains.push_back(lp.chain);
    op->fixed.push_back(lp.fixed);
    op->infos.push_back(b);
    bis.push_back(b.get());
    ss.push_back(lp.fixed.s.get());
    const bool zero = lp.fixed.w->is_all_zero();
    op->unit[i] = zero && b->unit_shape;
    if (!zero) ws.push_back(lp.fixed.w.get());
    ws.push_back(lp.chain.w.get());
  }
  ensure_band_device_batch(bis, ss);
  ensure_weights_device_batch(ws);
  size_t bytes = align_up(8 * n, 256);
  std::vector<size_t> ao(n), oo(n), lo(n);
  for (size_t i = 0; i < n; ++i) {
    const int T = op->chains[i].s->M, N = int(op->fixed[i].s->N);
    const int ns = band_row_stride(N, band_npl(N));
    lo[i] = bytes;
    bytes = align_up(bytes + 4 * size_t(T > 0 ? T : 1), 256);
    oo[i] = bytes;
    bytes = align_up(bytes + 8 * (4 * size_t(T) + 16), 256);
    ao[i] = bytes;
    bytes = align_up(bytes + 4 * size_t(T + 1) * size_t(ns), 256);
  }
  op->arena = rt.alloc(bytes);
  op->pairs.resize(n);
  std::vector<std::pair<BandSdOp::Key, BandPair>> tab;
  tab.reserve(n);
  double abytes = 0;
  for (size_t i = 0; i < n; ++i) {
    BandPair& p = op->pairs[i];
    p = BandPair{};
    const BandInfo& b = *op->infos[i];
    p.nodes = b.dev;
    p.nflags = b.dev_flags;
    p.snode = b.dev_snode;
    p.slab = b.dev_slab;
    p.n_lab = int(b.snode.size());
    p.w = op->fixed[i].w->is_all_zero() ? nullptr : op->fixed[i].w->dev;
    p.em = op->chains[i].w->dev;
    p.N = int(op->fixed[i].s->N);
    p.T = op->chains[i].s->M;
    p.C = op->chains[i].s->C;
    p.NS = band_row_stride(p.N, band_npl(p.N));
    p.alpha = op->arena->as<float>(ao[i]);
    p.aoff = op->arena->as<double>(oo[i]);
    p.score = op->arena->as<float>(4 * i);
    if (!op->chains[i].w->valid_norm_cache()) {
      p.norm = op->arena->as<float>(4 * (n + i));
      p.rowlse = op->arena->as<float>(lo[i]);
    }
    p.hot = b.hot;
    p.lgrn = band_forward_lgrn(p.C);
    tab.push_back({BandSdOp::Key{p.C, band_npl(p.N), int(op->unit[i]), 0, BandSdOp::band_vec(p)}, p});
    abytes += 4.0 * p.T * p.C + 4.0 * double(p.T + 1) * p.NS;
  }
  {
    BandSdOp::launch(tab, false, "band_forward_score", abytes);
  }
  for (size_t i = 0; i < n; ++i) {
    const BandPair& p = op->pairs[i];
    if (!p.norm) continue;
    auto nc = std::make_shared<NormCache>();
    nc->version = op->chains[i].w->version;
    nc->mem = op->arena;
    nc->norm = p.norm;
    nc->rowlse = p.rowlse;
    op->chains[i].w->norm_cache = std::move(nc);
  }
  std::vector<Graph> outs;
  outs.reserve(n);
  for (size_t i = 0; i < n; ++i) {
    Graph out = make_output(op, int(i), {gs[i]});
    init_scalar_result(out);
    set_dev_weights(out, op->arena, op->pairs[i].score, 1);
    outs.push_back(std::move(out));
  }
  return outs;
}

struct BandViterbiScoreOp : OpRecord {
  struct Saved {
    DevMemP mem;
    const int *arc = nullptr, *lab = nullptr;
    int len = -1, C = 0, chain_first = 0;
  };
  std::vector<Saved> saved;
  void backward(std::vector<Member>& ms) override {
    Runtime& rt = Runtime::get();
    GradSink sink;
    for (auto& m : ms) {
      const Saved& sv = saved[m.idx];
      Graph& comp = m.out.g->inputs[0];
      comp.g->grad_propagated = true;
      if (sv.len <= 0 || comp.g->inputs.size() != 2) continue;
      Graph& chain = comp.g->inputs[sv.chain_first ? 0 : 1];
      Graph& fixed = comp.g->inputs[sv.chain_first ? 1 : 0];
      size_t bytes = 0;
      const size_t oc = bytes;
      if (chain.calc_grad()) bytes = align_up(bytes + 4 * size_t(chain.num_arcs()), 256);
      const size_t of = bytes;
      if (fixed.calc_grad()) bytes = align_up(bytes + 4 * size_t(fixed.num_arcs()), 256);
      if (!bytes) continue;
      DevMemP gm = rt.alloc_zero(bytes);
      LazyPathGrad a{};
      a.delta = through_delta(m.out);
      a.delta_stride = 0;
      a.path_arc = sv.arc;
      a.il = a.ol = sv.lab;
      a.len = sv.len;
      a.C = sv.C;
      a.chain_first = sv.chain_first;
      a.grad_chain = chain.calc_grad() ? gm->as<float>(oc) : nullptr;
      a.grad_fixed = fixed.calc_grad() ? gm->as<float>(of) : nullptr;
      launch_lazy_path_grad(a, rt.stream());
      if (a.grad_chain) sink.add(chain, gm, a.grad_chain);
      if (a.grad_fixed) sink.add(fixed, gm, a.grad_fixed);
    }
    sink.flush();
  }
};

static bool layer_order(const Structure& s, int start, bool last_touch, std::vector<int>& rank) {
  const int N = int(s.N);
  std::vector<int> layer{start}, next;
  std::vector<long long> key(size_t(N), -1);
  bool fixed = false;
  for (int it = 0; it < 4 * N + 8 && !fixed; ++it) {
    std::fill(key.begin(), key.end(), -1);
    for (size_t i = 0; i < layer.size(); ++i) {
      const int l = layer[i];
      for (int k = s.out_off[size_t(l)]; k < s.out_off[size_t(l) + 1]; ++k) {
        const int d = s.dst[size_t(s.out_list[size_t(k)])];
        const long long kk = (long long)(i) * 8 + (k - s.out_off[size_t(l)]);
        long long& slot = key[size_t(d)];
        slot = slot < 0 ? kk : (last_touch ? std::max(slot, kk) : std::min(slot, kk));
      }
// ... 377 lines not shown
```

Measured before the change: 932,900 losses/s.

## Fuse CTC target building into band forward and fold scalar step into backward

Defers the ctc_targets kernel so the band forward kernel builds target node labels and skip flags in LDS itself, removing a separate launch and a global round trip. It also records the scalar axpby and seed-gradient step lazily and folds it into the patched band backward kernel prologue, removing two small launches per step. The cost is considerable bookkeeping: a global fold state under a mutex, flush points scattered across the API, and risk of ordering bugs if a flush is missed.

```diff
diff --git a/gtn_amd/csrc/band.hip b/gtn_amd/csrc/band.hip
--- a/gtn_amd/csrc/band.hip
+++ b/gtn_amd/csrc/band.hip
@@ -332,50 +332,7 @@
   return wave_max(mx);
 }
 
-template <int NPL, bool UNIT, int K, bool VEC>
-__global__ __launch_bounds__(WG) void band_forward_kernel(const BandPair* __restrict__ pairs, int NSmax) {
-#define GTNX_BAND_PAIR pairs[blockIdx.x]
-#include "band_forward_body.inc"
-#undef GTNX_BAND_PAIR
-}
-template <int NPL, bool UNIT, int K, bool VEC>
-__global__ __launch_bounds__(WG) void band_forward_one_kernel(BandPair one, int NSmax) {
-#define GTNX_BAND_PAIR one
-#include "band_forward_body.inc"
-#undef GTNX_BAND_PAIR
-}
-
-__device__ __forceinline__ BandPair band_patched(BandPair P, const BandPatch& pt) {
-  if (pt.on) {
-    const int b = P.bidx;
-    P.delta = pt.delta + b;
-    P.delta_norm = pt.delta_norm ? pt.delta_norm + b : nullptr;
-    P.rowlse = pt.rowlse ? pt.rowlse + int64_t(b) * pt.M : nullptr;
-    P.norm = nullptr;
-    P.em_copy = nullptr;
-    P.grad_em = pt.grad_em ? pt.grad_em + int64_t(b) * pt.A : nullptr;
-    P.grad_fixed = pt.grad_fixed ? pt.grad_fixed + P.goff : nullptr;
-  }
-  return P;
-}
-template <int NPL, bool UNIT, bool GRADG, int K, bool VEC, bool BIG>
-__global__ __launch_bounds__(WGB, BIG ? 3 : 6) void band_backward_kernel(const BandPair* __restrict__ pairs, int NSmax, BandPatch patch) {
-#define GTNX_BAND_PAIR band_patched(pairs[blockIdx.x], patch)
-#include "band_backward_body.inc"
-#undef GTNX_BAND_PAIR
-}
-template <int NPL, bool UNIT, bool GRADG, int K, bool VEC, bool BIG>
-__global__ __launch_bounds__(WGB, BIG ? 3 : 6) void band_backward_one_kernel(BandPair one, int NSmax) {
-#define GTNX_BAND_PAIR one
-#include "band_backward_body.inc"
-#undef GTNX_BAND_PAIR
-}
-
-
-__global__ __launch_bounds__(512) void ctc_targets_kernel(const CtcTargetArgs* __restrict__ args, int blank) {
-  const CtcTargetArgs a = args[blockIdx.x];
-  __shared__ __attribute__((aligned(16))) int tl[256 + 4];
-  __shared__ __attribute__((aligned(16))) int tk[256 + 4];
+__device__ __forceinline__ void ctc_target_build(const CtcTargetArgs a, int blank, int* tl, int* tk, int* nl, int* nk) {
   const int N = a.N, U = (N - 1) >> 1, m = threadIdx.x;
   if (m < 260) {
     const int v = m < U ? a.labels[m] : 0x7fffffff;
@@ -411,6 +368,96 @@
   a.snode[rank] = m;
   a.slab[rank] = my;
   if (m == N - 1 && a.n_arcs) a.n_arcs[0] = base + 1 + (m > 0 ? 1 : 0) + skip;
+  if (nl) {
+    nl[m] = my;
+    nk[m] = skip;
+  }
+}
+template <int NPL>
+__device__ __forceinline__ void built_nodes(int N, int m0, const int* lab, const int* skip, NodeRegs<NPL>& g) {
+#pragma unroll
+  for (int j = 0; j < NPL; ++j) {
+    const int m = m0 + j;
+    const bool in = m < N;
+    g.lab[j] = in ? lab[j] : 0;
+    g.start[j] = in && m == 0;
+    g.accept[j] = in && m + 2 >= N;
+    g.has_in[j] = in;
+    g.wi[0][j] = in ? 0.0f : NEGF;
+    g.wi[1][j] = in && m > 0 ? 0.0f : NEGF;
+    g.wi[2][j] = in && skip[j] ? 0.0f : NEGF;
+#pragma unroll
+    for (int k = 0; k < 3; ++k) {
+      g.wo[k][j] = NEGF;
+      g.ao[k][j] = -1;
+    }
+  }
+}
+
+template <int NPL, bool UNIT, int K, bool VEC>
+__global__ __launch_bounds__(WG) void band_forward_kernel(const BandPair* __restrict__ pairs, int NSmax, BandTargets targets) {
+#define GTNX_BAND_PAIR pairs[blockIdx.x]
+#define GTNX_BAND_TARGETS targets
+#include "band_forward_body.inc"
+#undef GTNX_BAND_TARGETS
+#undef GTNX_BAND_PAIR
+}
+template <int NPL, bool UNIT, int K, bool VEC>
+__global__ __launch_bounds__(WG) void band_forward_one_kernel(BandPair one, int NSmax) {
+#define GTNX_BAND_PAIR one
+#include "band_forward_body.inc"
+#undef GTNX_BAND_PAIR
+}
+
+__device__ __forceinline__ BandPair band_patched(BandPair P, const BandPatch& pt) {
+  if (pt.on) {
+    const int b = P.bidx;
+    P.delta = pt.delta + b;
+    P.delta_norm = pt.delta_norm ? pt.delta_norm + b : nullptr;
+    P.rowlse = pt.rowlse ? pt.rowlse + int64_t(b) * pt.M : nullptr;
+    P.norm = nullptr;
+    P.em_copy = nullptr;
+    P.grad_em = pt.grad_em ? pt.grad_em + int64_t(b) * pt.A : nullptr;
+    P.grad_fixed = pt.grad_fixed ? pt.grad_fixed + P.goff : nullptr;
+  }
+  return P;
+}
+__device__ __forceinline__ void band_fold_apply(const BandFold& f, int b, float& ds, float& dn) {
+  float v = f.sa * f.a[b];
+  if (f.b) v += f.sb * f.b[b];
+  float v0 = f.s0, v1 = f.s1;
+  if (f.g0 && f.acc0) v0 = f.g0[b] + f.s0;
+  if (f.g1 && f.acc1) v1 = f.g1[b] + f.s1;
+  __syncthreads();
+  if (threadIdx.x == 0) {
+    f.out[b] = v;
+    f.root[b] = 1.0f;
+    if (f.g0) f.g0[b] = v0;
+    if (f.g1) f.g1[b] = v1;
+  }
+  ds = uniform(f.ds_src ? v1 : v0);
+  if (f.dn_src >= 0) dn = uniform(f.dn_src ? v1 : v0);
+}
+template <int NPL, bool UNIT, bool GRADG, int K, bool VEC, bool BIG>
+__global__ __launch_bounds__(WGB, BIG ? 3 : 6) void band_backward_kernel(const BandPair* __restrict__ pairs, int NSmax, BandPatch patch) {
+#define GTNX_BAND_PAIR band_patched(pairs[blockIdx.x], patch)
+#define GTNX_BAND_FOLD patch.fold
+#include "band_backward_body.inc"
+#undef GTNX_BAND_FOLD
+#undef GTNX_BAND_PAIR
+}
+template <int NPL, bool UNIT, bool GRADG, int K, bool VEC, bool BIG>
+__global__ __launch_bounds__(WGB, BIG ? 3 : 6) void band_backward_one_kernel(BandPair one, int NSmax) {
+#define GTNX_BAND_PAIR one
+#include "band_backward_body.inc"
+#undef GTNX_BAND_PAIR
+}
+
+
+__global__ __launch_bounds__(512) void ctc_targets_kernel(const CtcTargetArgs* __restrict__ args, int blank) {
+  __shared__ __attribute__((aligned(16))) int tl[256 + 4];
+  __shared__ __attribute__((aligned(16))) int tk[256 + 4];
+  ctc_target_build(args[blockIdx.x], blank, tl, tk, nullptr, nullptr);
 }
 
 __global__ __launch_bounds__(512) void band_viterbi_kernel(const BandDecode* __restrict__ pairs) {
@@ -810,7 +857,7 @@
 }
 
 template <int NPL, int K, bool VEC>
-void launch_fwd2(const BandPair* d, const BandPair* one, int n, int ns, size_t lds, bool unit, hipStream_t st) {
+void launch_fwd2(const BandPair* d, const BandPair* one, int n, int ns, size_t lds, bool unit, hipStream_t st, const BandTargets& tg) {
   static std::atomic<uint64_t> done{0};
   if (gtnx_first_on_device first{done}) {
     big_lds(band_forward_kernel<NPL, true, K, VEC>);
@@ -827,13 +874,14 @@
       return;
     }
   }
-  if (unit) hipLaunchKernelGGL((band_forward_kernel<NPL, true, K, VEC>), dim3(n), dim3(WG), lds, st, d, ns);
-  else hipLaunchKernelGGL((band_forward_kernel<NPL, false, K, VEC>), dim3(n), dim3(WG), lds, st, d, ns);
+  if (unit) hipLaunchKernelGGL((band_forward_kernel<NPL, true, K, VEC>), dim3(n), dim3(WG), lds, st, d, ns, tg);
+  else hipLaunchKernelGGL((band_forward_kernel<NPL, false, K, VEC>), dim3(n), dim3(WG), lds, st, d, ns, tg);
 }
 template <int NPL, int K>
-void launch_fwd(const BandPair* d, const BandPair* one, int n, int ns, size_t lds, bool unit, bool vec, hipStream_t st) {
-  if (vec) launch_fwd2<NPL, K, true>(d, one, n, ns, lds, unit, st);
-  else launch_fwd2<NPL, K, false>(d, one, n, ns, lds, unit, st);
+void launch_fwd(const BandPair* d, const BandPair* one, int n, int ns, size_t lds, bool unit, bool vec, hipStream_t st,
+                const BandTargets& tg) {
+  if (vec) launch_fwd2<NPL, K, true>(d, one, n, ns, lds, unit, st, tg);
+  else launch_fwd2<NPL, K, false>(d, one, n, ns, lds, unit, st, tg);
 }
 template <int NPL, int K, bool VEC, bool BIG>
 void launch_bwd3(const BandPair* d, const BandPair* one, int n, int ns, size_t lds, bool unit, bool gradg, hipStream_t st,
@@ -923,19 +971,25 @@
   return !(K * C > 1024 || K * max_NS > 1024);
 }
 void launch_band_forward(const BandPair* d_pairs, int n, int npl, int C, int max_NS, bool unit, bool vec, hipStream_t st,
-                         const BandPair* one) {
+                         const BandPair* one, const BandTargets* targets) {
   if (n <= 0) return;
   if (one && (n != 1 || !band_one_ok(npl, C, max_NS, vec, false))) throw std::logic_error("band.hip: not a single-pair launch");
   const int K = band_block_rows(C, 0, false);
-  const size_t lds = 4 * size_t(band_lds(C, K, max_NS, false).total) + 64;
+  size_t lds = 4 * size_t(band_lds(C, K, max_NS, false).total) + 64;
+  BandTargets tg{};
+  if (targets && targets->args) {
+    if (one || !unit) throw std::logic_error("band.hip: targets are built by a table launch over unit weights");
+    tg = *targets;
+    lds = std::max(lds, 4 * size_t(BAND_TARGETS_LDS_INTS) + 64);
+  }
   if (npl == 1) {
-    if (K == 8) launch_fwd<1, 8>(d_pairs, one, n, max_NS, lds, unit, vec, st);
-    else if (K == 4) launch_fwd<1, 4>(d_pairs, one, n, max_NS, lds, unit, vec, st);
-    else launch_fwd<1, 2>(d_pairs, one, n, max_NS, lds, unit, vec, st);
+    if (K == 8) launch_fwd<1, 8>(d_pairs, one, n, max_NS, lds, unit, vec, st, tg);
+    else if (K == 4) launch_fwd<1, 4>(d_pairs, one, n, max_NS, lds, unit, vec, st, tg);
+    else launch_fwd<1, 2>(d_pairs, one, n, max_NS, lds, unit, vec, st, tg);
   } else {
-    if (K == 8) launch_fwd<2, 8>(d_pairs, one, n, max_NS, lds, unit, vec, st);
-    else if (K == 4) launch_fwd<2, 4>(d_pairs, one, n, max_NS, lds, unit, vec, st);
-    else launch_fwd<2, 2>(d_pairs, one, n, max_NS, lds, unit, vec, st);
+    if (K == 8) launch_fwd<2, 8>(d_pairs, one, n, max_NS, lds, unit, vec, st, tg);
+    else if (K == 4) launch_fwd<2, 4>(d_pairs, one, n, max_NS, lds, unit, vec, st, tg);
+    else launch_fwd<2, 2>(d_pairs, one, n, max_NS, lds, unit, vec, st, tg);
   }
 }
 
diff --git a/gtn_amd/csrc/band_backward_body.inc b/gtn_amd/csrc/band_backward_body.inc
--- a/gtn_amd/csrc/band_backward_body.inc
+++ b/gtn_amd/csrc/band_backward_body.inc
@@ -19,11 +19,19 @@
   const GTNX_G double* ao = P.aoff;
   const double z2 = uniform(ao[0]);
   const bool dead = !(z2 > double(DEADF));
+#ifdef GTNX_BAND_FOLD
+  float ds = 0.0f, dn_k = 0.0f;
+  const bool dn_folded = GTNX_BAND_FOLD.on && GTNX_BAND_FOLD.dn_src >= 0;
+  if (GTNX_BAND_FOLD.on) band_fold_apply(GTNX_BAND_FOLD, P.bidx, ds, dn_k);
+  else ds = uniform(P.delta[0]);
+  if (!dn_folded) dn_k = P.delta_norm ? uniform(P.delta_norm[0]) : 0.0f;
+#else
   const float ds = uniform(P.delta[0]);
+  const float dn_k = P.delta_norm ? uniform(P.delta_norm[0]) : 0.0f;
+#endif
   const bool want_em = P.grad_em != nullptr;
   GTNX_TM_INIT(128);
   constexpr bool SPLIT = !BIG && K >= 2 && GTNX_BWD_SPLIT;
-  const float dn_k = P.delta_norm ? uniform(P.delta_norm[0]) : 0.0f;
   float* const rnorm_k = lser + NBG * K;
   auto rows_of_k = [&](int c) { return c < nblocks ? min(K, T - c * K) : 0; };
   auto ring_start = [](int c, int M) { return ((c % M) + M) % M; };
diff --git a/gtn_amd/csrc/band_forward_body.inc b/gtn_amd/csrc/band_forward_body.inc
--- a/gtn_amd/csrc/band_forward_body.inc
+++ b/gtn_amd/csrc/band_forward_body.inc
@@ -17,12 +17,32 @@
   const int nblocks = (T + K - 1) / K;
   const int nticks = nblocks + 3;
   GTNX_TM_INIT(0);
+#ifdef GTNX_BAND_TARGETS
+  const bool built = GTNX_BAND_TARGETS.args != nullptr;
+  int pre_lab[NPL], pre_skip[NPL];
+  if (built) {
+    int* scr = reinterpret_cast<int*>(lds);
+    ctc_target_build(GTNX_BAND_TARGETS.args[P.bidx], GTNX_BAND_TARGETS.blank, scr, scr + 260, scr + 520, scr + 520 + 512);
+    __syncthreads();
+#pragma unroll
+    for (int j = 0; j < NPL; ++j) {
+      const int m = int(threadIdx.x) * NPL + j;
+      pre_lab[j] = m < P.N ? scr[520 + m] : 0;
+      pre_skip[j] = m < P.N ? scr[520 + 512 + m] : 0;
+    }
+    __syncthreads();
+  }
+#endif
 
   if (sweeper) {
     __builtin_amdgcn_s_setprio(1);
     const int w = wv;
     const int m0 = threadIdx.x * NPL;
     NodeRegs<NPL> g;
+#ifdef GTNX_BAND_TARGETS
+    if (built) built_nodes<NPL>(P.N, m0, pre_lab, pre_skip, g);
+    else
+#endif
     load_nodes<NPL, false>(P, m0, g);
     const bool writer = m0 < NS;
     float a[NPL];
diff --git a/gtn_amd/csrc/batch.cpp b/gtn_amd/csrc/batch.cpp
--- a/gtn_amd/csrc/batch.cpp
+++ b/gtn_amd/csrc/batch.cpp
@@ -2,6 +2,7 @@
 
 #include <algorithm>
 #include <atomic>
+#include <mutex>
 #include <unordered_map>
 #include <unordered_set>
 
@@ -75,6 +76,53 @@
   launch_vec_axpby(b.g_dev, t.ptr, nullptr, size_t(b.g_off[size_t(b.n)]), 1.0f, 0.0f, 1, Runtime::get().stream());
 }
 
+}
+
+struct StepFold {
+  const float* a = nullptr;
+  const float* b = nullptr;
+  float* out = nullptr;
+  float sa = 0, sb = 0;
+  size_t n = 0;
+  bool seed = false;
+  float* root = nullptr;
+  float* g[2] = {nullptr, nullptr};
+  float sc[2] = {0, 0};
+  int acc[2] = {0, 0};
+};
+
+namespace {
+std::mutex g_fold_mu;
+Batch* g_fold = nullptr;
+
+bool fold_enabled() {
+  static const bool off = std::getenv("GTNX_NO_STEP_FOLD") != nullptr;
+  return !off;
+}
+void fold_run(const StepFold& f) {
+  hipStream_t st = Runtime::get().stream();
+  launch_vec_axpby(f.out, f.a, f.b, f.n, f.sa, f.sb, 0, st);
+  if (f.seed) launch_scalar_seed(f.root, f.g[0], f.sc[0], f.acc[0], f.g[1], f.sc[1], f.acc[1], f.n, st);
+}
+std::shared_ptr<StepFold> fold_take() {
+  std::lock_guard<std::mutex> lk(g_fold_mu);
+  if (!g_fold) return nullptr;
+  std::shared_ptr<StepFold> f = std::move(g_fold->fold);
+  g_fold->fold.reset();
+  g_fold = nullptr;
+  return f;
+}
+StepFold* fold_of(Batch& x) {
+  std::lock_guard<std::mutex> lk(g_fold_mu);
+  return g_fold == &x ? x.fold.get() : nullptr;
+}
+}
+
+void batch_fold_flush() {
+  if (std::shared_ptr<StepFold> f = fold_take()) fold_run(*f);
+}
+
+namespace {
 struct BScalarOp : BatchOp {
   ScalarKind kind;
   void backward(Batch& out) override {
@@ -110,6 +158,7 @@
   void run(Batch& out) {
     Batch& e = *inputs[0];
     Runtime& rt = Runtime::get();
+    batch_fold_flush();
     if (e.w_pend) e.w_pend->settle();
     const bool have = e.g_dev != nullptr;
     if (!have) alloc_grad(e, false);
@@ -146,6 +195,18 @@
     Batch& ch = *prod.chain;
     Runtime& rt = Runtime::get();
     const float* delta = out.g_dev;
+    static const bool no_patch = std::getenv("GTNX_NO_BAND_PATCH") != nullptr;
+    std::shared_ptr<StepFold> fold;
+    {
+      std::unique_lock<std::mutex> lk(g_fold_mu);
+      StepFold* f = g_fold ? g_fold->fold.get() : nullptr;
+      bool ok = f && f->seed && f->n == size_t(prod.n) && prod.n > 1 && fwd_table && !no_patch && !through_acc &&
+                !t_batch_retain && (f->a == out.v_dev || f->b == out.v_dev) && (delta == f->g[0] || delta == f->g[1]);
+      for (int b = 0; b < prod.n && ok; ++b) ok = pairs[size_t(b)].bidx == b;
+      lk.unlock();
+      if (ok) fold = fold_take();
+      else batch_fold_flush();
+    }
     if (through_acc || t_batch_retain) {
       const size_t n = size_t(prod.n);
       if (!through_acc) through_acc = rt.alloc_zero(sizeof(float) * (n ? n : 1));
@@ -183,7 +244,10 @@
       bytes += 4.0 * p.T * p.C * (p.grad_em ? 2 : 1) + 4.0 * double(p.T + 1) * p.NS +
                (p.grad_fixed ? 4.0 * double(fx.elem_size(b)) : 0.0);
     }
-    static const bool no_patch = std::getenv("GTNX_NO_BAND_PATCH") != nullptr;
+    if (fold && !one_key) {
+      fold_run(*fold);
+      fold.reset();
+    }
     if (fwd_table && one_key && prod.n > 1 && !no_patch) {
       BandPatch pt{};
       pt.on = 1;
@@ -194,6 +258,16 @@
       pt.grad_em = ge.ptr;
       pt.grad_fixed = gf.ptr;
       pt.A = int64_t(A);
+      if (fold) {
+        BandFold& fd = pt.fold;
+        fd.on = 1;
+        fd.a = fold->a, fd.b = fold->b, fd.out = fold->out, fd.sa = fold->sa, fd.sb = fold->sb;
+        fd.root = fold->root;
+        fd.g0 = fold->g[0], fd.s0 = fold->sc[0], fd.acc0 = fold->acc[0];
+        fd.g1 = fold->g[1], fd.s1 = fold->sc[1], fd.acc1 = fold->acc[1];
+        fd.ds_src = delta == fold->g[0] ? 0 : 1;
+        fd.dn_src = !pt.delta_norm ? -1 : (pt.delta_norm == fold->g[0] ? 0 : (pt.delta_norm == fold->g[1] ? 1 : -1));
+      }
       band_launch_patched(fwd_table, prod.n, tab.front().first, max_ns, pt, "band_forward_score_grad", bytes);
     } else {
       band_launch(tab, true, "band_forward_score_grad", bytes);
@@ -257,6 +331,19 @@
 }
 
 Batch::~Batch() {
+  if (fold) {
+    std::shared_ptr<StepFold> f;
+    {
+      std::lock_guard<std::mutex> lk(g_fold_mu);
+      if (g_fold == this) g_fold = nullptr, f = std::move(fold);
+    }
+    if (f && (!v_mem || f->seed) && Runtime::initialized()) {
+      try {
+        fold_run(*f);
+      } catch (...) {
+      }
+    }
+  }
   if (host_ev) (void)hipEventDestroy(static_cast<hipEvent_t>(host_ev));
   if (give_back && !origins.empty()) {
     for (const Origin& o : origins) {
@@ -384,8 +471,17 @@
     a.pad = 0;
   }
   rt.h2d_pinned(b->rec_mem->ptr, pin->ptr, lab_bytes + arg_bytes);
-  launch_ctc_targets(reinterpret_cast<const CtcTargetArgs*>(b->rec_mem->as<char>(lab_bytes)), n, blank, rt.stream());
+  b->tgt_args_off = lab_bytes;
+  b->tgt_pending = true;
+  if (!fold_enabled() || n < 2) batch_targets_settle(*b);
   return b;
+}
+
+void batch_targets_settle(Batch& x) {
+  if (!x.tgt_pending) return;
+  x.tgt_pending = false;
+  launch_ctc_targets(reinterpret_cast<const CtcTargetArgs*>(x.rec_mem->as<char>(x.tgt_args_off)), x.n, x.blank,
+                     Runtime::get().stream());
 }
 
 
@@ -605,6 +701,7 @@
 }
 
 void batch_materialise(Batch& x) {
+  batch_fold_flush();
   if (x.materialised) return;
   if (x.leaf) {
     x.materialised = true;
@@ -833,7 +930,13 @@
       tab.push_back({BandLaunchKey{C, band_npl(q.N), fx.fal ? 0 : 1, 0, band_vec_ok(q)}, q});
       abytes += 4.0 * T * C + 4.0 * double(T + 1) * p.NS + (fuse_copy ? 4.0 * T * C : 0.0);
     }
-    band_launch(tab, false, "band_forward_score", abytes, fuse_copy ? nullptr : &op->fwd_table);
+    BandTargets tg{};
+    if (fx.tgt_pending && !fx.fal && n > 1) {
+      tg.args = reinterpret_cast<const CtcTargetArgs*>(fx.rec_mem->as<char>(fx.tgt_args_off));
+      tg.blank = fx.blank;
+      fx.tgt_pending = false;
+    }
+    band_launch(tab, false, "band_forward_score", abytes, fuse_copy ? nullptr : &op->fwd_table, tg.args ? &tg : nullptr);
     if (fuse_copy) pend->done.store(true, std::memory_order_release);
     if (want_norm) {
       ch.nc_mem = op->arena;
@@ -915,6 +1018,7 @@
 BatchP batch_scalar(ScalarKind k, const BatchP& a0, const BatchP& b0, void* items_dev) {
   BatchP a = a0, b = b0;
   const bool binary = k != SK_NEGATE;
+  batch_fold_flush();
   if (binary && a->n == b->n) {
     const bool an = a->kind == Batch::SCALAR && !a->materialised, bn = b->kind == Batch::SCALAR && !b->materialised;
     if (an && !bn && b->kind == Batch::GRAPHS) {
@@ -937,8 +1041,16 @@
       r->v_mem = rt.alloc(sizeof(float) * size_t(a->n ? a->n : 1));
       r->v_dev = r->v_mem->as<float>();
     }
-    launch_vec_axpby(r->v_dev, a->v_dev, binary ? b->v_dev : nullptr, size_t(a->n), k == SK_NEGATE ? -1.0f : 1.0f,
-                     k == SK_SUBTRACT ? -1.0f : 1.0f, 0, rt.stream());
+    const float sa = k == SK_NEGATE ? -1.0f : 1.0f, sb = k == SK_SUBTRACT ? -1.0f : 1.0f;
+    if (binary && a->n > 1 && fold_enabled() && a.get() != b.get()) {
+      auto f = std::make_shared<StepFold>();
+      f->a = a->v_dev, f->b = b->v_dev, f->out = r->v_dev, f->sa = sa, f->sb = sb, f->n = size_t(a->n);
+      std::lock_guard<std::mutex> lk(g_fold_mu);
+      r->fold = f;
+      g_fold = r.get();
+      return r;
+    }
+    launch_vec_axpby(r->v_dev, a->v_dev, binary ? b->v_dev : nullptr, size_t(a->n), sa, sb, 0, rt.stream());
     return r;
   }
   batch_materialise(*a);
@@ -953,6 +1065,7 @@
   GTNX_HOST_T("batch.backward");
   if (root->tape_cleared)
     throw_invalid("[autograd::backward] Cannot Backward twice without retaining the graph.");
+  if (retain || !fold_of(*root)) batch_fold_flush();
   if (root->materialised || !root->op || root->kind != Batch::SCALAR) {
     batch_materialise(*root);
     op_backward(root->graphs, nullptr, retain);
@@ -994,12 +1107,25 @@
         if (!in.g_dev) alloc_grad(in, false);
         g[i] = in.g_dev;
       }
-      launch_scalar_seed(root->g_dev, g[0], sc[0], acc[0], g[1], sc[1], acc[1], size_t(root->n), rt.stream());
+      bool recorded = false;
+      {
+        std::lock_guard<std::mutex> lk(g_fold_mu);
+        if (g_fold == root.get() && root->fold && !retain) {
+          StepFold& f = *root->fold;
+          f.seed = true;
+          f.root = root->g_dev;
+          for (int i = 0; i < 2; ++i) f.g[i] = g[i], f.sc[i] = sc[i], f.acc[i] = acc[i];
+          recorded = true;
+        }
+      }
+      if (!recorded) launch_scalar_seed(root->g_dev, g[0], sc[0], acc[0], g[1], sc[1], acc[1], size_t(root->n), rt.stream());
       root_done = true;
     } else {
+      batch_fold_flush();
       launch_fill_f32(root->g_dev, 1.0f, size_t(root->n), rt.stream());
     }
   } else {
+    batch_fold_flush();
     DevMemP ones = rt.alloc(sizeof(float) * size_t(root->n ? root->n : 1));
     launch_fill_f32(ones->as<float>(), 1.0f, size_t(root->n), rt.stream());
     launch_vec_axpby(root->g_dev, ones->as<float>(), nullptr, size_t(root->n), 1.0f, 0.0f, 1, rt.stream());
@@ -1021,10 +1147,12 @@
         from_graphs.push_back(b);
         continue;
       }
+      if (!dynamic_cast<BFsBandOp*>(b->op.get()) && !dynamic_cast<BFsLinearOp*>(b->op.get())) batch_fold_flush();
       b->op->backward(*b);
     }
     for (auto& kv : plan.lin)
       if (!plan.fused.count(kv.first)) static_cast<BFsLinearOp*>(kv.second->op.get())->run(*kv.second);
+    batch_fold_flush();
   } catch (...) {
     t_plan = nullptr;
     throw;
@@ -1045,6 +1173,7 @@
 }
 
 void batch_items_device(const BatchP& x, void* dev_out) {
+  batch_fold_flush();
   if (x->kind == Batch::SCALAR && !x->materialised) {
     if (static_cast<const void*>(x->v_dev) == dev_out) return;
     Runtime::get().d2d(dev_out, x->v_dev, sizeof(float) * size_t(x->n));
@@ -1054,6 +1183,7 @@
   items_device(x->graphs, dev_out);
 }
 float batch_item_host(const BatchP& x, int i) {
+  batch_fold_flush();
   if (i < 0 || i >= x->n) throw_range("[gtnx_batch_get] element index out of range");
   if (!x->host_vals_valid) {
     x->host_vals.resize(size_t(x->n));
@@ -1071,6 +1201,7 @@
   return x->host_vals[size_t(i)];
 }
 void batch_prefetch_items(const BatchP& x) {
+  batch_fold_flush();
   if (!x || x->kind != Batch::SCALAR || x->materialised || x->host_vals_valid || x->host_ev || x->n <= 0 || !x->v_dev) return;
   Runtime& rt = Runtime::get();
   hipEvent_t ev;
@@ -1084,6 +1215,7 @@
   x->host_ev = ev;
 }
 void batch_items_host(const BatchP& x, float* out) {
+  batch_fold_flush();
   if (x->kind == Batch::SCALAR && !x->materialised) {
     Runtime::get().d2h_sync(out, x->v_dev, sizeof(float) * size_t(x->n));
     return;
diff --git a/gtn_amd/csrc/batch.h b/gtn_amd/csrc/batch.h
--- a/gtn_amd/csrc/batch.h
+++ b/gtn_amd/csrc/batch.h
@@ -42,6 +42,8 @@
   int max_label = -1, max_nodes = 0;
   DevMemP rec_mem;
   std::vector<size_t> rec_off;
+  bool tgt_pending = false;
+  size_t tgt_args_off = 0;
   bool fal = false;
   Graph trans;
   int trans_labels = 0;
@@ -57,6 +59,8 @@
   bool chain_first = false, intersect = false;
   DevMemP v_mem;
   float* v_dev = nullptr;
+
+  std::shared_ptr<struct StepFold> fold;
 
   std::shared_ptr<BatchOp> op;
   bool tape_cleared = false;
@@ -89,5 +93,7 @@
 BatchP batch_ctc_targets_from_graphs(const std::vector<Graph>& gs);
 BatchP batch_linear_from_graphs(const std::vector<Graph>& gs);
 void batch_materialise(Batch& x);
+void batch_fold_flush();
+void batch_targets_settle(Batch& x);
 
 }
diff --git a/gtn_amd/csrc/capi.cpp b/gtn_amd/csrc/capi.cpp
--- a/gtn_amd/csrc/capi.cpp
+++ b/gtn_amd/csrc/capi.cpp
@@ -163,11 +163,15 @@
   });
 }
 GTNX_API gtnx_status_t gtnx_set_stream(void* s) {
-  return guard([&] { Runtime::get().set_stream(static_cast<hipStream_t>(s)); });
+  return guard([&] {
+    batch_fold_flush();
+    Runtime::get().set_stream(static_cast<hipStream_t>(s));
+  });
 }
 GTNX_API gtnx_status_t gtnx_synchronize(void) {
   return guard([&] {
     if (Runtime::initialized()) {
+      batch_fold_flush();
       Runtime::get().sync();
       deferred_resolve_all();
     }
diff --git a/gtn_amd/csrc/kernels.h b/gtn_amd/csrc/kernels.h
--- a/gtn_amd/csrc/kernels.h
+++ b/gtn_amd/csrc/kernels.h
@@ -379,6 +379,18 @@
   int bidx;
   int64_t goff;
 };
+struct BandFold {
+  int on;
+  int acc0, acc1;
+  int ds_src, dn_src;
+  float sa, sb, s0, s1;
+  const GTNX_G float* a;
+  const GTNX_G float* b;
+  GTNX_G float* out;
+  GTNX_G float* root;
+  GTNX_G float* g0;
+  GTNX_G float* g1;
+};
 struct BandPatch {
   int on;
   int M;
@@ -388,6 +400,7 @@
   GTNX_G float* grad_em;
   GTNX_G float* grad_fixed;
   int64_t A;
+  BandFold fold;
 };
 struct BandDecode {
   const GTNX_G BandNode* nodes;
@@ -465,6 +478,11 @@
   int N, pad;
 };
 void launch_ctc_targets(const CtcTargetArgs* d_args, int n, int blank, hipStream_t st);
+struct BandTargets {
+  const CtcTargetArgs* args;
+  int blank, pad;
+};
+constexpr int BAND_TARGETS_LDS_INTS = 2 * 260 + 2 * 512;
 struct AsgFalArgs {
   const GTNX_G int* labels;
   const GTNX_G float* trans_w;
@@ -487,7 +505,7 @@
 int band_forward_lgrn(int C);
 bool band_one_ok(int npl, int C, int max_NS, bool vec, bool backward);
 void launch_band_forward(const BandPair* d_pairs, int n, int npl, int C, int max_NS, bool unit, bool vec, hipStream_t st,
-                         const BandPair* one = nullptr);
+                         const BandPair* one = nullptr, const BandTargets* targets = nullptr);
 void launch_band_backward(const BandPair* d_pairs, int n, int npl, int C, int max_NS, bool unit, bool gradg, bool vec,
                           hipStream_t st, const BandPair* one = nullptr, const BandPatch* patch = nullptr);
 void launch_lazy_dense_prep(const LazyGroup& g, float* E, float* cmax, hipStream_t st);
diff --git a/gtn_amd/csrc/ops.h b/gtn_amd/csrc/ops.h
--- a/gtn_amd/csrc/ops.h
+++ b/gtn_amd/csrc/ops.h
@@ -42,7 +42,7 @@
 };
 int band_vec_ok(const BandPair& p);
 void band_launch(std::vector<std::pair<BandLaunchKey, BandPair>>& tab, bool backward, const char* prof_name = nullptr,
-                 double prof_bytes = 0.0, DevMemP* table_out = nullptr);
+                 double prof_bytes = 0.0, DevMemP* table_out = nullptr, const BandTargets* targets = nullptr);
 void band_launch_patched(const DevMemP& table, int n, const BandLaunchKey& key, int max_ns, const BandPatch& patch,
                          const char* prof_name, double prof_bytes);
 
diff --git a/gtn_amd/csrc/ops_band.cpp b/gtn_amd/csrc/ops_band.cpp
--- a/gtn_amd/csrc/ops_band.cpp
+++ b/gtn_amd/csrc/ops_band.cpp
@@ -1,6 +1,7 @@
 #include "ops_internal.h"
 
 #include <memory>
+#include <stdexcept>
 
 namespace gtnx {
 
@@ -13,10 +14,11 @@
                        &patch);
 }
 void band_launch(std::vector<std::pair<BandLaunchKey, BandPair>>& tab, bool backward, const char* prof_name, double prof_bytes,
-                 DevMemP* table_out) {
+                 DevMemP* table_out, const BandTargets* targets) {
   Runtime& rt = Runtime::get();
   if (table_out) table_out->reset();
   if (tab.empty()) return;
+  if (targets && (backward || tab.size() == 1)) throw std::logic_error("band_launch: targets ride with a forward table launch");
   bool one_key = true;
   for (size_t i = 1; i < tab.size() && one_key; ++i) one_key = tab[i].first == tab[0].first;
   if (!one_key) std::stable_sort(tab.begin(), tab.end(), [](const auto& x, const auto& y) { return x.first < y.first; });
@@ -45,7 +47,7 @@
     if (backward)
       launch_band_backward(dp + i0, int(i1 - i0), k.npl, k.C, max_ns, k.unit != 0, k.gradg != 0, k.vec != 0, rt.stream());
     else
-      launch_band_forward(dp + i0, int(i1 - i0), k.npl, k.C, max_ns, k.unit != 0, k.vec != 0, rt.stream());
+      launch_band_forward(dp + i0, int(i1 - i0), k.npl, k.C, max_ns, k.unit != 0, k.vec != 0, rt.stream(), nullptr, targets);
     i0 = i1;
   }
 }
```

After: 941,000 losses/s (median of 6 runs). About the same (+0.9%).
